# EryiXie/PlaneRecNet

Hardware: AMD Instinct MI355X
Metric: img/s fwd+bwd @480×640 ResNet101-DCN, 1/2/4/8 MI355X + roofline % (higher is better)
Workload: dtype f32 (tensors and accumulation fp32; plain GEMMs and the tap-walked 4x4/s2, 1x1/s2 and sub-pixel convolutions >= 300 tiles: 2xfp16-piece split MFMA, fp32 accumulate; fp32-only rate in fp32_only_run)

## Files before the change

include/prn.h:

```cpp
#ifndef PRN_H
#define PRN_H
#include <stdint.h>
#ifdef __cplusplus
extern "C" {
#endif

#define PRN_BN_SPLITS 32

int prn_version(void);
const char* prn_last_error(void);

enum { PRN_IN_ZERO = 0, PRN_IN_REFLECT = 1, PRN_IN_UP2_REFLECT = 2, PRN_IN_DILATED = 3, PRN_IN_UP2_PHASE = 4,
       PRN_IN_EMBED1 = 5  };
enum { PRN_EPI_NONE = 0, PRN_EPI_RELU = 1, PRN_EPI_SIGMOID = 2 };

enum { PRN_SPLIT_OFF = 0, PRN_SPLIT_PLAN = 1, PRN_SPLIT_ALWAYS = 2 };
enum { PRN_PIECES_BF16 = 0, PRN_PIECES_F16 = 16 };
typedef struct prn_gemm_opts {
  int32_t split_mode;
  int32_t split_kind;
  int32_t split_products;
  int32_t split_min_tiles;
  float split_min_gflop;
  int32_t wgrad_wgs;
// ... 161 lines not shown
                    const float* beta, float* dx, float* dres, float* dgamma, float* dbeta, double* ws,
                    int B, int C, int HW, int relu, int frozen, void* stream);

int prn_bn_train_fwd_partials(const float* parts, int nparts, int64_t part_stride, float* x_out, float* stats, const float* gamma, const float* beta,
                              const float* residual, float* y, float* running_mean, float* running_var, int B, int C, int HW, float eps, float momentum,
                              int relu, void* stream);
int prn_bn_bwd_partials(const float* dparts, int nparts, int64_t part_stride, const float* x, const float* y, const float* stats, const float* gamma,
                        const float* beta, float* dx, float* dres, float* dgamma, float* dbeta, int B, int C, int HW, int relu, int frozen, void* stream);
int prn_bn_train_fwd_winograd(const float* parts, int nparts, int64_t part_stride, float* x_out, float* stats, const float* gamma, const float* beta,
                              const float* residual, float* y, float* running_mean, float* running_var, float* V, int B, int C, int H, int W, float eps,
                              float momentum, int relu, void* stream);
int prn_bn_bwd_winograd(const float* dparts, int nparts, int64_t part_stride, const float* x, const float* y, const float* stats, const float* gamma,
                        const float* beta, float* dx, float* dres, float* dgamma, float* dbeta, float* V, int B, int C, int H, int W, int relu, int frozen,
                        void* stream);

int prn_gn_relu_fwd(const float* x, const float* gamma, const float* beta, float* y, float* stats ,
                    int B, int C, int HW, int G, float eps, void* stream);
int prn_gn_relu_bwd(const float* dy, const float* x, const float* beta, const float* stats, const float* gamma,
                    float* dx, float* dgamma_part , float* dbeta_part ,
                    int B, int C, int HW, int G, void* stream);
int prn_gn_relu_fwd_ragged(const float* x, const float* gamma, const float* beta, float* y, float* stats,
                           int B, int C, int nseg, const int* hw, int G, float eps, void* stream);
int prn_gn_relu_bwd_ragged(const float* dy, const float* x, const float* beta, const float* stats, const float* gamma,
                           float* dx, float* dgamma_part, float* dbeta_part, int B, int C, int nseg, const int* hw, int G,
                           void* stream);

int prn_sum_rows(const float* in, float* out, int nb, int R, int N, void* stream);

int prn_debug_skip_launches(int mask);

int prn_resize_bilinear_fwd(const float* x, float* y, int BC, int H, int W, int Ho, int Wo, void* stream);
int prn_resize_bilinear_bwd(const float* dy, float* dx, int BC, int H, int W, int Ho, int Wo, void* stream);
int prn_resize_bilinear_add_fwd(const float* x, const float* addend, float* y, int BC, int H, int W, int Ho, int Wo, void* stream);
int prn_resize_bilinear_bwd_add(const float* dy, const float* addend, float* dx, int BC, int H, int W, int Ho, int Wo, void* stream);
int prn_maxpool3s2_fwd(const float* x, float* y, unsigned char* arg, int BC, int H, int W, int Ho, int Wo, void* stream);
int prn_maxpool3s2_bwd(const unsigned char* arg, const float* dy, float* dx, int BC, int H, int W, int Ho, int Wo, void* stream);

int64_t prn_plane_prior_ws_bytes(int B, int E, int h, int w, int NK, int F, const prn_gemm_opts* opts);
int prn_plane_prior_fwd(const float* seg, const float* kernels, const float* w1, const float* b1, float* pooled, float* out, void* ws, int B, int E,
                        int h, int w, int NK, int F, const prn_gemm_opts* opts, void* stream);
int prn_plane_prior_fwd_phase(const float* seg, const float* kernels, const float* w1, const float* b1, float* pooled, float* out, void* ws, int B, int E,
                        int h, int w, int NK, int F, const prn_gemm_opts* opts, void* stream, int phase);
int64_t prn_plane_prior_wgrad_ws_bytes(int B, int h, int w, int NK, int F, const prn_gemm_opts* opts);
int prn_plane_prior_wgrad(const float* pooled, const float* d_out, float* dw1, void* ws, int B, int h, int w, int NK, int F, const prn_gemm_opts* opts,
                          void* stream);
int64_t prn_fpn_level_ws_bytes(int B, int C, int H, int W, int F, int relu, int has_prev, int have_u, const prn_gemm_opts* opts);
int prn_fpn_level_fwd(const float* x, const float* w_lat, const float* b_lat, const float* prev, int Hp, int Wp, const float* w_out, const float* u_out,
                      const float* b_out, float* lateral, float* p_out, void* ws, int B, int C, int H, int W, int F, int relu, const prn_gemm_opts* opts,
                      void* stream);

enum { PRN_BLK_WINOGRAD = 1,
       PRN_BLK_HANDOVER = 2,
       PRN_BLK_KEEP_V = 4,
       PRN_BLK_SCATTER_ACC = 8 };
enum { PRN_BLK_CONV2_DIRECT = 0, PRN_BLK_CONV2_WINOGRAD = 1, PRN_BLK_CONV2_DCN = 2 };
typedef struct prn_bottleneck_desc {
  int32_t B, C, H, W;
  int32_t planes;
  int32_t stride;
  int32_t dcn;
  int32_t downsample;
  int32_t flags;
  float eps[4], momentum[4];
  float max_offset;
  int32_t reserved;
  prn_gemm_opts opts;
} prn_bottleneck_desc;
typedef struct prn_bottleneck_params {
  const float *w1, *w2, *w3, *wd;
  const float *b2;
  const void *w1_img, *w3_img, *wd_img;
  const float* u2; const void* u2_img;
  const float *w1_t, *w2_t, *w3_t, *wd_t;
  const void *w1_t_img, *w3_t_img, *wd_t_img;
  const float* ut2; const void* ut2_img;
  const float *w27, *b27, *w27_t;
  const float* w2_cols_t; const void* w2_cols_t_img;
  const float *gamma[4], *beta[4];
  float *running_mean[4], *running_var[4];
} prn_bottleneck_params;
enum { PRN_BLK_SAVE_BYTES = 0, PRN_BLK_GSAVE_BYTES, PRN_BLK_FWD_WS_BYTES, PRN_BLK_BWD_WS_BYTES, PRN_BLK_HO, PRN_BLK_WO, PRN_BLK_CONV2_PATH, PRN_BLK_KEEPS_V,
       PRN_BLK_OFF_A1, PRN_BLK_OFF_V, PRN_BLK_OFF_A2, PRN_BLK_OFF_OM, PRN_BLK_OFF_TABLE,
       PRN_BLK_OFF_D1, PRN_BLK_OFF_D2, PRN_BLK_OFF_D3, PRN_BLK_OFF_DD, PRN_BLK_OFF_DOM,
       PRN_BLK_BN_GRAD_FLOATS,
       PRN_BLK_HANDOVERS,
       PRN_BLK_NEEDS_W1_IMG, PRN_BLK_NEEDS_W3_IMG, PRN_BLK_NEEDS_WD_IMG, PRN_BLK_NEEDS_W1T_IMG, PRN_BLK_NEEDS_W3T_IMG, PRN_BLK_NEEDS_WDT_IMG, PRN_BLK_NEEDS_U_IMG,
       PRN_BLK_NEEDS_COLT_IMG, PRN_BLK_INFO_COUNT };
int64_t prn_bottleneck_plan_bytes(void);
int64_t prn_bottleneck_params_bytes(void);
int prn_bottleneck_plan(const prn_bottleneck_desc* d, void* plan);
int prn_bottleneck_plan_info(const void* plan, int64_t* out, int n);
int prn_bottleneck_train_fwd(const void* plan, const prn_bottleneck_params* p, const float* x, float* y, void* save, void* ws, void* stream);
int prn_bottleneck_train_bwd(const void* plan, const prn_bottleneck_params* p, const float* x, const float* y, const float* dy, float* dx, int dx_accumulate,
                             const void* save, void* gsave, float* bn_grads, void* ws, void* stream);

int prn_frame_to_input(const unsigned char* src, int Hs, int Ws, int Hr, int Wr, int Hp, int Wp, const float* mean_bgr, const float* std_bgr, int mode,
                       float* dst, float* frame_bgr, void* stream);

int prn_mask_loss_ws_floats(int P);
int prn_mask_loss_fwd(const float* logits, const unsigned char* labels, const float* adj, const int64_t* img, const float* gsum, const float* npos,
                      float* out2, float* coef, float* ws, int P, int HW, int B, float w_ins, float w_lav, void* stream);
int prn_mask_loss_bwd(const float* logits, const unsigned char* labels, const float* adj, const int64_t* img, const float* coef, const float* g_ins,
                      const float* g_lav, float* dlogits, int P, int HW, void* stream);

int prn_lava_gt_weights(const float* gt, float* out, int B, int H, int W, float depth_resolution, void* stream);

int prn_vnl_triplets(const float* pred, const float* gt, const int* gid, const int64_t* seg, const unsigned char* seg_is_plane, const double* seg_normal,
// ... 123 lines not shown
```

planerecnet_amd/blocks.py:

```python
import ctypes
import os
import sys

import torch

from . import _lib, ops, profiling
from ._lib import lib, check

ENABLED = os.environ.get("PRN_BLOCKS", "1") == "1"
HANDOVER = os.environ.get("PRN_BLOCK_HANDOVER", "1") == "1"
SCATTER_ACCUMULATE = os.environ.get("PRN_SCATTER_ACC", "1") == "1"
STATS = {"fwd": 0, "bwd": 0, "resolved": 0, "vouched": 0, "scatter_acc": 0}

BLK_WINOGRAD, BLK_HANDOVER, BLK_KEEP_V, BLK_SCATTER_ACC = 1, 2, 4, 8
CONV2_DIRECT, CONV2_WINOGRAD, CONV2_DCN = 0, 1, 2
(I_SAVE, I_GSAVE, I_FWD_WS, I_BWD_WS, I_HO, I_WO, I_CONV2, I_KEEPS_V, I_A1, I_V, I_A2, I_OM, I_TABLE, I_D1, I_D2, I_D3, I_DD, I_DOM, I_BN_FLOATS, I_HANDOVERS,
 I_W1_IMG, I_W3_IMG, I_WD_IMG, I_W1T_IMG, I_W3T_IMG, I_WDT_IMG, I_U_IMG, I_COLT_IMG, INFO_COUNT) = range(29)

_SCRATCH = {}
_F32 = torch.float32
_empty = torch.empty


def scratch(nbytes, dev):
    key = (dev.index, ops._raw_stream(dev.index))
    t = _SCRATCH.get(key)
    if t is None or t.numel() * 4 < nbytes:
        t = _SCRATCH[key] = torch.empty((int(nbytes * 1.25) + 1023) // 4, device=dev, dtype=torch.float32)
    return t


class _Ref:
    __slots__ = ("ptr", "shape", "device")

    def __init__(self, ptr, shape, device):
        self.ptr, self.shape, self.device = ptr, shape, device

    def data_ptr(self):
        return self.ptr

    def numel(self):
        n = 1
        for s in self.shape:
            n *= s
        return n


class _State:
    __slots__ = ("plan", "plan_ref", "info", "params", "params_ref", "convw", "wver", "epoch", "batched", "keep", "hb", "bn_sizes", "out_shape", "Ho", "Wo", "conv2",
                 "dims", "wino_wgrad", "g_keys", "max_offset", "ps", "bns", "stat_bufs", "save_n", "gsave_n", "bn_n", "fwd_ws", "bwd_ws", "stride", "dcn", "ds",
                 "shapes")


def _flags():
    f = BLK_SCATTER_ACC if SCATTER_ACCUMULATE else 0
    if ops.WINOGRAD:
        f |= BLK_WINOGRAD
    if ops.WINOGRAD and ops.WINOGRAD_WGRAD:
        f |= BLK_KEEP_V
    if HANDOVER:
        f |= BLK_HANDOVER
    return f


def supported(blk):
    from .dcn import DeformableConv2d
    c2 = blk.conv2
    if blk.downsample is not None:
        dc = blk.downsample[0]
        if dc.kernel_size != (1, 1) or dc.stride[0] != blk.stride or dc.bias is not None:
            return False
    elif blk.stride != 1 or blk.conv1.weight.shape[1] != blk.conv3.weight.shape[0]:
        return False
    if isinstance(c2, DeformableConv2d):
        if c2.stride != blk.stride:
            return False
    elif c2.bias is not None or c2.kernel_size != (3, 3) or c2.padding != (1, 1) or c2.stride[0] != blk.stride:
        return False
    bns = [blk.bn1, blk.bn2, blk.bn3] + ([blk.downsample[1]] if blk.downsample is not None else [])
    return (blk.stride in (1, 2) and ops.WINOGRAD_MIN_TILES == 128 and blk.conv1.bias is None and blk.conv3.bias is None and blk.conv1.kernel_size == (1, 1)
            and blk.conv3.kernel_size == (1, 1) and all(isinstance(m, torch.nn.BatchNorm2d) and m.affine and m.track_running_stats and m.momentum is not None for m in bns))


def _param_list(blk):
    from .dcn import DeformableConv2d
    c2 = blk.conv2
    ps = [blk.conv1.weight, blk.bn1.weight, blk.bn1.bias]
    if isinstance(c2, DeformableConv2d):
        ps += [c2.offset_conv.weight, c2.modulator_conv.weight, c2.offset_conv.bias, c2.modulator_conv.bias, c2.regular_conv.weight, c2.regular_conv.bias]
    else:
        ps += [c2.weight]
    ps += [blk.bn2.weight, blk.bn2.bias, blk.conv3.weight, blk.bn3.weight, blk.bn3.bias]
    if blk.downsample is not None:
        ps += [blk.downsample[0].weight, blk.downsample[1].weight, blk.downsample[1].bias]
    return tuple(ps)


def _state(blk, x, key):
    from .dcn import DeformableConv2d
    oe = ops._opts_entry()
    B, C, H, W = x.shape
    dcn = isinstance(blk.conv2, DeformableConv2d)
    bns = (blk.bn1, blk.bn2, blk.bn3) + ((blk.downsample[1],) if blk.downsample is not None else ())
    eps = [float(m.eps) for m in bns] + [0.0] * (4 - len(bns))
    mom = [float(m.momentum) for m in bns] + [0.0] * (4 - len(bns))
    P = blk.conv1.weight.shape[0]
    d = _lib.BottleneckDesc(B, C, H, W, P, blk.stride, int(dcn), int(blk.downsample is not None), key[2], (ctypes.c_float * 4)(*eps), (ctypes.c_float * 4)(*mom),
                            max(H, W) / 4.0 if dcn else 0.0, 0, oe[0])
    st = _State()
    st.plan = ctypes.create_string_buffer(int(lib.prn_bottleneck_plan_bytes()) + 64)
    st.plan_ref = (ctypes.addressof(st.plan) + 63) & ~63
    check(lib.prn_bottleneck_plan(ctypes.byref(d), st.plan_ref), "prn_bottleneck_plan")
    info = (ctypes.c_int64 * INFO_COUNT)()
    check(lib.prn_bottleneck_plan_info(st.plan_ref, info, INFO_COUNT), "prn_bottleneck_plan_info")
# ... 276 lines not shown
```

planerecnet_amd/csrc/prn_bottleneck.hip:

```cpp
#include "prn_common.h"
#include <string.h>

namespace {

constexpr int32_t PLAN_MAGIC = 0x424c4b36;
constexpr int64_t WINOGRAD_MIN_TILES = 128;

inline int64_t up256(int64_t v) { return (v + 255) & ~255LL; }

struct Plan {
  int32_t magic, pad_;
  prn_bottleneck_desc d;
  int32_t Ho, Wo, P4, conv2_path;
  int32_t small1, small2;
  int32_t lazy1, parts1;
  int32_t v1, lazy2, keep_v;
  int32_t lazy3g, parts3g;
  int32_t v2g, lazy2g;
  int32_t pad2_;
  int64_t parts1_off, parts3g_off;
  prn_conv_desc c1, c2, c3, cd, c27, g1, g2, g3, gd, g27;
  prn_dcn_desc dcn;
  int64_t s_c1, s_a1, s_v, s_c2, s_a2, s_c3, s_cd, s_om, s_table, s_stats[4], save_bytes;
  int64_t q_d3, q_dd, q_d2, q_d1, q_dom, q_bn, gsave_bytes;
  int64_t f_c1, f_bn, f_v, f_yt, f_gemm, f_c2, f_c27, f_dcn, f_c3, f_cd, f_res, fwd_ws_bytes;
  int64_t b_bn, b_dres, b_g3, b_g3ws, b_v, b_yt, b_gemm, b_g2, b_g2ws, b_dcn, b_dx1, b_g27ws, b_g1ws, b_gdtmp, b_gdws, bwd_ws_bytes;
};

prn_conv_desc conv_desc(int B, int C, int H, int W, int M, int K, int stride, int pad, int Ho, int Wo, int mode, int dil, int ystride, int yH, int yW,
                        const prn_gemm_opts& o) {
  prn_conv_desc d;
  d.B = B; d.C = C; d.H = H; d.W = W; d.M = M; d.KH = d.KW = K; d.stride = stride; d.pad = pad; d.Ho = Ho; d.Wo = Wo;
  d.in_mode = mode; d.dil = dil; d.epilogue = PRN_EPI_NONE; d.ystride = ystride; d.yH = yH; d.yW = yW; d.reserved = 0;
  d.opts = o;
  return d;
}

bool winograd_ok(const prn_bottleneck_desc& d, int B, int C, int H, int W, int M) {
  return (d.flags & PRN_BLK_WINOGRAD) && (W % 4) == 0 && H >= 8 && C >= 64 && M >= 64 && (int64_t)B * ((H + 3) / 4) * (W / 4) >= WINOGRAD_MIN_TILES;
}

int make_plan(const prn_bottleneck_desc* dp, Plan& L) {
  PRN_REQUIRE(dp != nullptr, "prn_bottleneck_plan: null descriptor");
  const prn_bottleneck_desc& d = *dp;
  PRN_REQUIRE(d.B > 0 && d.C > 0 && d.H > 0 && d.W > 0 && d.planes > 0, "prn_bottleneck_plan: empty dimension");
  PRN_REQUIRE(d.stride == 1 || d.stride == 2, "prn_bottleneck_plan: stride %d (1 or 2)", d.stride);
  PRN_REQUIRE(d.downsample || (d.stride == 1 && d.C == 4 * d.planes), "prn_bottleneck_plan: without a downsample branch the block must keep its shape (C = 4 * planes, stride 1)");
  PRN_REQUIRE(!d.dcn || d.max_offset > 0.f, "prn_bottleneck_plan: the deformable variant needs max_offset (max(h, w) / 4)");
  memset(&L, 0, sizeof(L));
  L.magic = PLAN_MAGIC;
  L.d = d;
  const int B = d.B, C = d.C, H = d.H, W = d.W, P = d.planes, s = d.stride, Q = 4 * d.planes;
  const int Ho = (H + 2 - 3) / s + 1, Wo = (W + 2 - 3) / s + 1;
  L.Ho = Ho; L.Wo = Wo;
  const prn_gemm_opts& o = d.opts;
  const bool ho = (d.flags & PRN_BLK_HANDOVER) != 0;
  L.small1 = prn_bn_kernel_kind(B, H * W);
  L.small2 = prn_bn_kernel_kind(B, Ho * Wo);
  L.c1 = conv_desc(B, C, H, W, P, 1, 1, 0, H, W, PRN_IN_ZERO, 1, 0, 0, 0, o);
  L.c3 = conv_desc(B, P, Ho, Wo, Q, 1, 1, 0, Ho, Wo, PRN_IN_ZERO, 1, 0, 0, 0, o);
  if (d.downsample) L.cd = conv_desc(B, C, H, W, Q, 1, s, 0, Ho, Wo, PRN_IN_ZERO, 1, 0, 0, 0, o);
  const bool wino = !d.dcn && s == 1 && winograd_ok(d, B, P, H, W, P);
  L.conv2_path = d.dcn ? PRN_BLK_CONV2_DCN : (wino ? PRN_BLK_CONV2_WINOGRAD : PRN_BLK_CONV2_DIRECT);
  if (d.dcn) {
    L.c27 = conv_desc(B, P, H, W, 27, 3, s, 1, Ho, Wo, PRN_IN_ZERO, 1, 0, 0, 0, o);
    prn_dcn_desc& q = L.dcn;
    q.B = B; q.C = P; q.H = H; q.W = W; q.M = P; q.stride = s; q.pad = 1; q.Ho = Ho; q.Wo = Wo; q.raw = 1; q.max_offset = d.max_offset; q.epilogue = PRN_EPI_NONE;
    q.opts = o;
  } else if (!wino) {
    L.c2 = conv_desc(B, P, H, W, P, 3, s, 1, Ho, Wo, PRN_IN_ZERO, 1, 0, 0, 0, o);
  }
  if (wino) L.P4 = (int)prn_winograd_tiles(B, H, W);
  L.g3 = conv_desc(B, Q, Ho, Wo, P, 1, 1, 0, Ho, Wo, PRN_IN_ZERO, 1, 0, 0, 0, o);
  L.g1 = conv_desc(B, P, H, W, C, 1, 1, 0, H, W, PRN_IN_ZERO, 1, 0, 0, 0, o);
  if (!d.dcn && !wino)
    L.g2 = s == 1 ? conv_desc(B, P, Ho, Wo, P, 3, 1, 1, H, W, PRN_IN_ZERO, 1, 0, 0, 0, o) : conv_desc(B, P, Ho, Wo, P, 3, 1, 1, H, W, PRN_IN_DILATED, 2, 0, 0, 0, o);
  if (d.dcn)
    L.g27 = s == 1 ? conv_desc(B, 27, Ho, Wo, P, 3, 1, 1, H, W, PRN_IN_ZERO, 1, 0, 0, 0, o) : conv_desc(B, 27, Ho, Wo, P, 3, 1, 1, H, W, PRN_IN_DILATED, 2, 0, 0, 0, o);
  if (d.downsample)
    L.gd = s == 1 ? conv_desc(B, Q, Ho, Wo, C, 1, 1, 0, H, W, PRN_IN_ZERO, 1, 0, 0, 0, o) : conv_desc(B, Q, Ho, Wo, C, 1, 1, 0, Ho, Wo, PRN_IN_ZERO, 1, 2, H, W, o);
  int64_t off = 0;
  const int p1 = prn_conv2d_fwd_partials(&L.c1, &off);
  if (p1 < 0) return 2;
  L.lazy1 = ho && L.small1 && p1 > 1 && (((int64_t)B * P * H * W) & 3) == 0;
  L.parts1 = L.lazy1 ? p1 : 0; L.parts1_off = L.lazy1 ? off : 0;
  L.v1 = ho && wino && L.small1;
  L.lazy2 = ho && wino && L.small2 && L.P4 <= 768;
  L.keep_v = wino && (d.flags & PRN_BLK_KEEP_V) && 4LL * 36 * P * L.P4 <= (128LL << 20);
  const int p3 = prn_conv2d_fwd_partials(&L.g3, &off);
  if (p3 < 0) return 2;
  L.lazy3g = ho && L.small2 && p3 > 1 && (((int64_t)B * P * Ho * Wo) & 3) == 0;
  L.parts3g = L.lazy3g ? p3 : 0; L.parts3g_off = L.lazy3g ? off : 0;
  L.v2g = ho && wino && L.small2;
  L.lazy2g = ho && wino && L.small1 && L.P4 <= 768;
  const int64_t n1 = (int64_t)B * P * H * W * 4, n2 = (int64_t)B * P * Ho * Wo * 4, n3 = (int64_t)B * Q * Ho * Wo * 4, nx = (int64_t)B * C * H * W * 4;
  const int64_t nv = wino ? 4LL * 36 * P * L.P4 : 0, nom = (int64_t)B * 27 * Ho * Wo * 4;
  const int Cmax = Q > C ? Q : C;
  const int64_t bnws = 2LL * Cmax * PRN_BN_SPLITS * 8;
#define PRN_WS(expr_, name_) const int64_t name_ = (expr_); if (name_ < 0) return 2
  PRN_WS(prn_conv2d_fwd_ws_bytes(&L.c1), w_c1);
  PRN_WS(prn_conv2d_fwd_ws_bytes(&L.c3), w_c3);
  PRN_WS(d.downsample ? prn_conv2d_fwd_ws_bytes(&L.cd) : 0, w_cd);
  PRN_WS(L.conv2_path == PRN_BLK_CONV2_DIRECT ? prn_conv2d_fwd_ws_bytes(&L.c2) : 0, w_c2);
  PRN_WS(d.dcn ? prn_conv2d_fwd_ws_bytes(&L.c27) : 0, w_c27);
  PRN_WS(d.dcn ? prn_dcnv2_fwd_ws_bytes(&L.dcn) : 0, w_dcnf);
  PRN_WS(d.dcn ? prn_dcnv2_table_bytes(&L.dcn) : 0, n_table);
  PRN_WS(d.dcn ? prn_dcnv2_bwd_ws_bytes(&L.dcn) : 0, w_dcnb);
  PRN_WS(wino ? prn_gemm_batched_ws_bytes(P, P, L.P4, 36, &o) : 0, w_gemm);
  PRN_WS(prn_conv2d_fwd_ws_bytes(&L.g3), w_g3);
  PRN_WS(prn_conv2d_fwd_ws_bytes(&L.g1), w_g1);
  PRN_WS(L.conv2_path == PRN_BLK_CONV2_DIRECT ? prn_conv2d_fwd_ws_bytes(&L.g2) : 0, w_g2);
  PRN_WS(d.dcn ? prn_conv2d_fwd_ws_bytes(&L.g27) : 0, w_g27);
  PRN_WS(d.downsample ? prn_conv2d_fwd_ws_bytes(&L.gd) : 0, w_gd);
#undef PRN_WS
  int64_t at = 0;
  auto put = [&at](int64_t& slot, int64_t bytes) { slot = at; at += up256(bytes); };
  put(L.s_c1, n1); put(L.s_a1, n1);
  put(L.s_v, L.keep_v ? nv : 0);
  put(L.s_c2, n2); put(L.s_a2, n2); put(L.s_c3, n3);
  put(L.s_cd, d.downsample ? n3 : 0);
  put(L.s_om, d.dcn ? nom : 0); put(L.s_table, n_table);
  put(L.s_stats[0], 8LL * P); put(L.s_stats[1], 8LL * P); put(L.s_stats[2], 8LL * Q); put(L.s_stats[3], d.downsample ? 8LL * Q : 0);
  L.save_bytes = at;
  at = 0;
  put(L.q_d3, n3); put(L.q_dd, d.downsample ? n3 : 0); put(L.q_d2, n2); put(L.q_d1, n1); put(L.q_dom, d.dcn ? nom : 0);
  L.q_bn = 2 * P + 2 * P + 2 * Q + (d.downsample ? 2 * Q : 0);
  L.gsave_bytes = at;
  at = 0;
  put(L.f_c1, w_c1); put(L.f_bn, bnws);
  put(L.f_v, (wino && !L.keep_v) ? nv : 0); put(L.f_yt, nv); put(L.f_gemm, w_gemm);
  put(L.f_c2, w_c2); put(L.f_c27, w_c27); put(L.f_dcn, w_dcnf); put(L.f_c3, w_c3); put(L.f_cd, w_cd);
  put(L.f_res, d.downsample ? n3 : 0);
  L.fwd_ws_bytes = at;
  at = 0;
  put(L.b_bn, bnws); put(L.b_dres, n3);
  put(L.b_g3, n2); put(L.b_g3ws, w_g3);
  put(L.b_v, nv); put(L.b_yt, nv); put(L.b_gemm, w_gemm);
  put(L.b_g2, n1); put(L.b_g2ws, w_g2);
  put(L.b_dcn, w_dcnb); put(L.b_dx1, d.dcn ? n1 : 0); put(L.b_g27ws, w_g27);
  put(L.b_g1ws, w_g1);
  put(L.b_gdtmp, d.downsample ? nx : 0); put(L.b_gdws, w_gd);
  L.bwd_ws_bytes = at;
  return 0;
}

const Plan* plan_of(const void* plan, const char* who) {
  const Plan* L = (const Plan*)plan;
  if (L == nullptr || L->magic != PLAN_MAGIC) { prn_set_error("%s: not a plan filled by prn_bottleneck_plan", who); return nullptr; }
  return L;
}

inline float* f32(void* base, int64_t off) { return (float*)((char*)base + off); }
inline void* raw(void* base, int64_t off, int64_t used = 1) { return used ? (void*)((char*)base + off) : nullptr; }

#define PRN_TRY(call_) do { if (int e_ = (call_)) return e_; } while (0)

}

extern "C" int64_t prn_bottleneck_plan_bytes(void) { return (int64_t)sizeof(Plan); }
extern "C" int64_t prn_bottleneck_params_bytes(void) { return (int64_t)sizeof(prn_bottleneck_params); }

extern "C" int prn_bottleneck_plan(const prn_bottleneck_desc* d, void* plan) {
  PRN_REQUIRE(plan != nullptr, "prn_bottleneck_plan: null plan buffer (prn_bottleneck_plan_bytes() bytes, caller-owned)");
  Plan L;
  if (int e = make_plan(d, L)) { memset(plan, 0, sizeof(int32_t)); return e; }
  memcpy(plan, &L, sizeof(L));
  return 0;
}

extern "C" int prn_bottleneck_plan_info(const void* plan, int64_t* out, int n) {
  const Plan* L = plan_of(plan, "prn_bottleneck_plan_info");
  if (!L) return 2;
  PRN_REQUIRE(out != nullptr && n >= PRN_BLK_INFO_COUNT, "prn_bottleneck_plan_info: out must hold PRN_BLK_INFO_COUNT (%d) values", PRN_BLK_INFO_COUNT);
  out[PRN_BLK_SAVE_BYTES] = L->save_bytes; out[PRN_BLK_GSAVE_BYTES] = L->gsave_bytes;
  out[PRN_BLK_FWD_WS_BYTES] = L->fwd_ws_bytes; out[PRN_BLK_BWD_WS_BYTES] = L->bwd_ws_bytes;
  out[PRN_BLK_HO] = L->Ho; out[PRN_BLK_WO] = L->Wo; out[PRN_BLK_CONV2_PATH] = L->conv2_path; out[PRN_BLK_KEEPS_V] = L->keep_v;
  out[PRN_BLK_OFF_A1] = L->s_a1; out[PRN_BLK_OFF_V] = L->s_v; out[PRN_BLK_OFF_A2] = L->s_a2; out[PRN_BLK_OFF_OM] = L->s_om; out[PRN_BLK_OFF_TABLE] = L->s_table;
  out[PRN_BLK_OFF_D1] = L->q_d1; out[PRN_BLK_OFF_D2] = L->q_d2; out[PRN_BLK_OFF_D3] = L->q_d3; out[PRN_BLK_OFF_DD] = L->q_dd; out[PRN_BLK_OFF_DOM] = L->q_dom;
  out[PRN_BLK_BN_GRAD_FLOATS] = L->q_bn;
  out[PRN_BLK_HANDOVERS] = L->lazy1 | (L->v1 << 1) | (L->lazy2 << 2) | (L->lazy3g << 3) | (L->v2g << 4) | (L->lazy2g << 5);
  out[PRN_BLK_NEEDS_W1_IMG] = prn_conv2d_kernel_kind(&L->c1) >= 2; out[PRN_BLK_NEEDS_W3_IMG] = prn_conv2d_kernel_kind(&L->c3) >= 2;
  out[PRN_BLK_NEEDS_WD_IMG] = (L->d.downsample && L->d.stride == 1 && prn_conv2d_kernel_kind(&L->cd) >= 2) ? 1 : 0;
  out[PRN_BLK_NEEDS_W1T_IMG] = prn_conv2d_kernel_kind(&L->g1) >= 2; out[PRN_BLK_NEEDS_W3T_IMG] = prn_conv2d_kernel_kind(&L->g3) >= 2;
  out[PRN_BLK_NEEDS_WDT_IMG] = (L->d.downsample && L->d.stride == 1 && prn_conv2d_kernel_kind(&L->gd) >= 2) ? 1 : 0;
  out[PRN_BLK_NEEDS_U_IMG] = (L->conv2_path == PRN_BLK_CONV2_WINOGRAD && prn_gemm_pipe(L->d.planes, L->d.planes, 1, L->P4, 36, &L->d.opts) >= 1) ? 1 : 0;
  out[PRN_BLK_NEEDS_COLT_IMG] = (L->d.dcn && prn_gemm_pipe(9 * L->d.planes, L->d.planes, L->d.B, L->Ho * L->Wo, 1, &L->d.opts) >= 1) ? 1 : 0;
  return 0;
}

extern "C" int prn_bottleneck_train_fwd(const void* plan, const prn_bottleneck_params* p, const float* x, float* y, void* save, void* ws, void* stream) {
  const Plan* Lp = plan_of(plan, "prn_bottleneck_train_fwd");
  if (!Lp) return 2;
  const Plan& L = *Lp;
  const prn_bottleneck_desc& d = L.d;
  PRN_REQUIRE(p && x && y && save && (ws || L.fwd_ws_bytes == 0), "prn_bottleneck_train_fwd: null tensor / buffer");
  PRN_REQUIRE(p->w1 && p->w3 && (p->w2 || L.conv2_path == PRN_BLK_CONV2_WINOGRAD) && (p->u2 || L.conv2_path != PRN_BLK_CONV2_WINOGRAD) && (!d.downsample || p->wd),
              "prn_bottleneck_train_fwd: a weight operand the plan reads is null");
  PRN_REQUIRE(!d.dcn || (p->w27 && p->b27), "prn_bottleneck_train_fwd: the deformable variant needs the merged offset | modulator weights");
  for (int i = 0; i < (d.downsample ? 4 : 3); ++i)
    PRN_REQUIRE(p->gamma[i] && p->beta[i] && p->running_mean[i] && p->running_var[i], "prn_bottleneck_train_fwd: null BatchNorm parameter (layer %d)", i);
  PRN_REQUIRE(((reinterpret_cast<uintptr_t>(save) | reinterpret_cast<uintptr_t>(ws)) & 255) == 0, "prn_bottleneck_train_fwd: save / ws must be 256-byte aligned");
  const int B = d.B, H = d.H, W = d.W, P = d.planes, Q = 4 * P, Ho = L.Ho, Wo = L.Wo;
  float* c1 = f32(save, L.s_c1); float* a1 = f32(save, L.s_a1); float* c2 = f32(save, L.s_c2); float* a2 = f32(save, L.s_a2); float* c3 = f32(save, L.s_c3);
  float* st1 = f32(save, L.s_stats[0]); float* st2 = f32(save, L.s_stats[1]); float* st3 = f32(save, L.s_stats[2]); float* std_ = f32(save, L.s_stats[3]);
  double* bnws = (double*)raw(ws, L.f_bn);
  const int64_t n1 = (int64_t)B * P * H * W;
  const prn_gemm_opts* o = &d.opts;
  PRN_TRY(prn_conv2d_fwd_counted(&L.c1, x, p->w1, p->w1_img, nullptr, nullptr, c1, raw(ws, L.f_c1, L.f_bn - L.f_c1), nullptr, stream, L.lazy1 ? 1 : 0));
  float* V = L.conv2_path == PRN_BLK_CONV2_WINOGRAD ? (L.keep_v ? f32(save, L.s_v) : f32(ws, L.f_v)) : nullptr;
  const float* in1 = L.lazy1 ? f32(ws, L.f_c1 + L.parts1_off) : c1;
  if (L.v1)
    PRN_TRY(prn_bn_train_fwd_winograd(in1, L.lazy1 ? L.parts1 : 1, L.lazy1 ? n1 : 0, L.lazy1 ? c1 : nullptr, st1, p->gamma[0], p->beta[0], nullptr, a1, p->running_mean[0],
                                      p->running_var[0], V, B, P, H, W, d.eps[0], d.momentum[0], 1, stream));
  else if (L.lazy1)
    PRN_TRY(prn_bn_train_fwd_partials(in1, L.parts1, n1, c1, st1, p->gamma[0], p->beta[0], nullptr, a1, p->running_mean[0], p->running_var[0], B, P, H * W, d.eps[0],
                                      d.momentum[0], 1, stream));
  else
    PRN_TRY(prn_bn_train_fwd(c1, st1, p->gamma[0], p->beta[0], nullptr, a1, p->running_mean[0], p->running_var[0], L.small1 ? nullptr : bnws, B, P, H * W, d.eps[0],
                             d.momentum[0], 1, stream));
  float* Yt = f32(ws, L.f_yt);
  if (L.conv2_path == PRN_BLK_CONV2_WINOGRAD) {
    if (!L.v1) PRN_TRY(prn_winograd_input(a1, V, B, P, H, W, PRN_IN_ZERO, stream));
    PRN_TRY(prn_gemm_batched(P, P, L.P4, 36, p->u2, p->u2_img, V, Yt, raw(ws, L.f_gemm, L.f_c2 - L.f_gemm), o, stream));
    if (!L.lazy2) PRN_TRY(prn_winograd_output(Yt, nullptr, nullptr, c2, B, P, H, W, PRN_EPI_NONE, stream));
  } else if (L.conv2_path == PRN_BLK_CONV2_DCN) {
    float* om = f32(save, L.s_om);
    void* table = raw(save, L.s_table);
    PRN_TRY(prn_conv2d_fwd_counted(&L.c27, a1, p->w27, nullptr, p->b27, nullptr, om, raw(ws, L.f_c27, L.f_dcn - L.f_c27), nullptr, stream, 0));
    PRN_TRY(prn_dcnv2_table(&L.dcn, om, nullptr, table, stream));
    PRN_TRY(prn_dcnv2_fwd(&L.dcn, a1, table, p->w2, p->b2, c2, raw(ws, L.f_dcn, L.f_c3 - L.f_dcn), stream));
  } else {
    PRN_TRY(prn_conv2d_fwd_counted(&L.c2, a1, p->w2, nullptr, nullptr, nullptr, c2, raw(ws, L.f_c2, L.f_c27 - L.f_c2), nullptr, stream, 0));
  }
  if (L.conv2_path == PRN_BLK_CONV2_WINOGRAD && L.lazy2)
    PRN_TRY(prn_winograd_output_bn_fwd(Yt, c2, st2, p->gamma[1], p->beta[1], a2, p->running_mean[1], p->running_var[1], B, P, Ho, Wo, d.eps[1], d.momentum[1], 1, stream));
  else
    PRN_TRY(prn_bn_train_fwd(c2, st2, p->gamma[1], p->beta[1], nullptr, a2, p->running_mean[1], p->running_var[1], L.small2 ? nullptr : bnws, B, P, Ho * Wo, d.eps[1],
                             d.momentum[1], 1, stream));
  PRN_TRY(prn_conv2d_fwd_counted(&L.c3, a2, p->w3, p->w3_img, nullptr, nullptr, c3, raw(ws, L.f_c3, L.f_cd - L.f_c3), nullptr, stream, 0));
  const float* res = x;
  if (d.downsample) {
    float* cd = f32(save, L.s_cd);
    float* rd = f32(ws, L.f_res);
    PRN_TRY(prn_conv2d_fwd_counted(&L.cd, x, p->wd, d.stride == 1 ? p->wd_img : nullptr, nullptr, nullptr, cd, raw(ws, L.f_cd, L.f_res - L.f_cd), nullptr, stream, 0));
    PRN_TRY(prn_bn_train_fwd(cd, std_, p->gamma[3], p->beta[3], nullptr, rd, p->running_mean[3], p->running_var[3], L.small2 ? nullptr : bnws, B, Q, Ho * Wo, d.eps[3],
                             d.momentum[3], 0, stream));
    res = rd;
  }
  return prn_bn_train_fwd(c3, st3, p->gamma[2], p->beta[2], res, y, p->running_mean[2], p->running_var[2], L.small2 ? nullptr : bnws, B, Q, Ho * Wo, d.eps[2], d.momentum[2],
                          1, stream);
}

extern "C" int prn_bottleneck_train_bwd(const void* plan, const prn_bottleneck_params* p, const float* x, const float* y, const float* dy, float* dx,
                                        int dx_accumulate, const void* save_, void* gsave, float* bn_grads, void* ws, void* stream) {
  const Plan* Lp = plan_of(plan, "prn_bottleneck_train_bwd");
  if (!Lp) return 2;
  const Plan& L = *Lp;
  const prn_bottleneck_desc& d = L.d;
  PRN_REQUIRE(p && x && y && dy && dx && save_ && gsave && bn_grads && ws, "prn_bottleneck_train_bwd: null tensor / buffer");
  PRN_REQUIRE(p->w1_t && p->w3_t && (!d.downsample || p->wd_t), "prn_bottleneck_train_bwd: an input-gradient weight layout the plan reads is null");
  PRN_REQUIRE(L.conv2_path != PRN_BLK_CONV2_WINOGRAD || p->ut2, "prn_bottleneck_train_bwd: conv2's Winograd-domain input-gradient operand is null");
  PRN_REQUIRE(L.conv2_path != PRN_BLK_CONV2_DIRECT || p->w2_t, "prn_bottleneck_train_bwd: conv2's input-gradient layout is null");
  PRN_REQUIRE(!d.dcn || (p->w27_t && p->w2_cols_t), "prn_bottleneck_train_bwd: the deformable variant needs the input-gradient layouts of both convolutions");
  PRN_REQUIRE(!dx_accumulate || (d.downsample && d.stride == 2 && (d.flags & PRN_BLK_SCATTER_ACC)),
              "prn_bottleneck_train_bwd: dx_accumulate only for stride-2 downsample blocks planned with PRN_BLK_SCATTER_ACC");
  PRN_REQUIRE(((reinterpret_cast<uintptr_t>(save_) | reinterpret_cast<uintptr_t>(gsave) | reinterpret_cast<uintptr_t>(ws)) & 255) == 0,
              "prn_bottleneck_train_bwd: save / gsave / ws must be 256-byte aligned");
  void* save = const_cast<void*>(save_);
  const int B = d.B, C = d.C, H = d.H, W = d.W, P = d.planes, Q = 4 * P, Ho = L.Ho, Wo = L.Wo;
  const float* c1 = f32(save, L.s_c1); const float* a1 = f32(save, L.s_a1); const float* c2 = f32(save, L.s_c2); const float* c3 = f32(save, L.s_c3);
  const float* st1 = f32(save, L.s_stats[0]); const float* st2 = f32(save, L.s_stats[1]); const float* st3 = f32(save, L.s_stats[2]); const float* std_ = f32(save, L.s_stats[3]);
  float* d3 = f32(gsave, L.q_d3); float* d2 = f32(gsave, L.q_d2); float* d1 = f32(gsave, L.q_d1);
  float* dg1 = bn_grads; float* db1 = dg1 + P; float* dg2 = db1 + P; float* db2 = dg2 + P; float* dg3 = db2 + P; float* db3 = dg3 + Q; float* dgd = db3 + Q; float* dbd = dgd + Q;
  double* bnws = (double*)raw(ws, L.b_bn);
  float* dres = f32(ws, L.b_dres);
  const prn_gemm_opts* o = &d.opts;
  hipStream_t st = (hipStream_t)stream;
  PRN_TRY(prn_bn_bwd(dy, c3, y, st3, p->gamma[2], p->beta[2], d3, dres, dg3, db3, L.small2 ? nullptr : bnws, B, Q, Ho * Wo, 1, 0, stream));
  const float* addx = dres;
  if (d.downsample) {
    float* dd = f32(gsave, L.q_dd);
    PRN_TRY(prn_bn_bwd(dres, f32(save, L.s_cd), nullptr, std_, p->gamma[3], p->beta[3], dd, nullptr, dgd, dbd, L.small2 ? nullptr : bnws, B, Q, Ho * Wo, 0, 0, stream));
    void* gws = raw(ws, L.b_gdws, L.bwd_ws_bytes - L.b_gdws);
    if (d.stride == 1) {
      float* tmp = f32(ws, L.b_gdtmp);
      PRN_TRY(prn_conv2d_fwd_counted(&L.gd, dd, p->wd_t, p->wd_t_img, nullptr, nullptr, tmp, gws, nullptr, stream, 0));
      addx = tmp;
    } else if (dx_accumulate) {
      PRN_TRY(prn_conv2d_fwd_counted(&L.gd, dd, p->wd_t, nullptr, nullptr, dx, dx, gws, nullptr, stream, 0));
      addx = dx;
    } else {
      float* tmp = f32(ws, L.b_gdtmp);
      const hipError_t e = hipMemsetAsync(tmp, 0, (size_t)B * C * H * W * 4, st);
      PRN_REQUIRE(e == hipSuccess, "prn_bottleneck_train_bwd: clearing the strided input gradient failed: %s", hipGetErrorString(e));
      PRN_TRY(prn_conv2d_fwd_counted(&L.gd, dd, p->wd_t, nullptr, nullptr, nullptr, tmp, gws, nullptr, stream, 0));
      addx = tmp;
    }
  }
  float* g3 = f32(ws, L.b_g3);
  PRN_TRY(prn_conv2d_fwd_counted(&L.g3, d3, p->w3_t, p->w3_t_img, nullptr, nullptr, g3, raw(ws, L.b_g3ws, L.b_v - L.b_g3ws), nullptr, stream, L.lazy3g ? 1 : 0));
  const float* in2 = L.lazy3g ? f32(ws, L.b_g3ws + L.parts3g_off) : g3;
  const int64_t n2 = (int64_t)B * P * Ho * Wo;
  float* Vg = f32(ws, L.b_v);
  if (L.v2g)
    PRN_TRY(prn_bn_bwd_winograd(in2, L.lazy3g ? L.parts3g : 1, L.lazy3g ? n2 : 0, c2, nullptr, st2, p->gamma[1], p->beta[1], d2, nullptr, dg2, db2, Vg, B, P, Ho, Wo, 1, 0, stream));
  else if (L.lazy3g)
    PRN_TRY(prn_bn_bwd_partials(in2, L.parts3g, n2, c2, nullptr, st2, p->gamma[1], p->beta[1], d2, nullptr, dg2, db2, B, P, Ho * Wo, 1, 0, stream));
  else
    PRN_TRY(prn_bn_bwd(g3, c2, nullptr, st2, p->gamma[1], p->beta[1], d2, nullptr, dg2, db2, L.small2 ? nullptr : bnws, B, P, Ho * Wo, 1, 0, stream));
  float* g2 = f32(ws, L.b_g2);
  float* Ytg = f32(ws, L.b_yt);
  if (L.conv2_path == PRN_BLK_CONV2_WINOGRAD) {
    if (!L.v2g) PRN_TRY(prn_winograd_input(d2, Vg, B, P, H, W, PRN_IN_ZERO, stream));
    PRN_TRY(prn_gemm_batched(P, P, L.P4, 36, p->ut2, p->ut2_img, Vg, Ytg, raw(ws, L.b_gemm, L.b_g2 - L.b_gemm), o, stream));
    if (!L.lazy2g) PRN_TRY(prn_winograd_output(Ytg, nullptr, nullptr, g2, B, P, H, W, PRN_EPI_NONE, stream));
  } else if (L.conv2_path == PRN_BLK_CONV2_DCN) {
    const float* om = f32(save, L.s_om);
    float* dom = f32(gsave, L.q_dom);
    float* dx1 = f32(ws, L.b_dx1);
    void* cws = raw(ws, L.b_dcn);
    PRN_TRY(prn_dcnv2_bwd_input(&L.dcn, d2, p->w2_cols_t, p->w2_cols_t_img, om, nullptr, dx1, cws, stream));
    PRN_TRY(prn_dcnv2_bwd_offset_mask(&L.dcn, a1, om, nullptr, dom, nullptr, cws, stream));
    PRN_TRY(prn_conv2d_fwd_counted(&L.g27, dom, p->w27_t, nullptr, nullptr, dx1, g2, raw(ws, L.b_g27ws, L.b_g1ws - L.b_g27ws), nullptr, stream, 0));
  } else {
    PRN_TRY(prn_conv2d_fwd_counted(&L.g2, d2, p->w2_t, nullptr, nullptr, nullptr, g2, raw(ws, L.b_g2ws, L.b_dcn - L.b_g2ws), nullptr, stream, 0));
  }
  if (L.conv2_path == PRN_BLK_CONV2_WINOGRAD && L.lazy2g)
    PRN_TRY(prn_winograd_output_bn_bwd(Ytg, c1, st1, p->gamma[0], p->beta[0], d1, dg1, db1, B, P, H, W, 1, stream));
  else
    PRN_TRY(prn_bn_bwd(g2, c1, nullptr, st1, p->gamma[0], p->beta[0], d1, nullptr, dg1, db1, L.small1 ? nullptr : bnws, B, P, H * W, 1, 0, stream));
  return prn_conv2d_fwd_counted(&L.g1, d1, p->w1_t, p->w1_t_img, nullptr, addx, dx, raw(ws, L.b_g1ws, L.b_gdtmp - L.b_g1ws), nullptr, stream, 0);
}
```

planerecnet_amd/csrc/prn_common.h:

```cpp
#pragma once
#include <hip/hip_runtime.h>
#include <stdint.h>
#include <stdio.h>
#include "../../include/prn.h"

#define PRN_WAVE 64

void prn_set_error(const char* fmt, ...);

#include <stdlib.h>
static inline int prn_env_int(const char* name, int dflt) {
  const char* e = getenv(name);
  return e ? atoi(e) : dflt;
}
struct prn_env4 { int v[4]; };
static inline prn_env4 prn_env_ints(const char* name) {
  prn_env4 r = {{0, 0, 0, 0}};
  if (const char* e = getenv(name)) sscanf(e, "%d,%d,%d,%d", &r.v[0], &r.v[1], &r.v[2], &r.v[3]);
  return r;
}

extern int prn_skip_mask;
#define PRN_SKIPPED(bit) (__builtin_expect(prn_skip_mask & (bit), 0))
#define PRN_REPS(bit) (__builtin_expect(prn_skip_mask & ((bit) | ((bit) << 8)), 0) ? ((prn_skip_mask & (bit)) ? 0 : 2) : 1)
// ... 37 lines not shown
  const int64_t T_ = (int64_t)gridDim.x * 256, i0_ = (int64_t)blockIdx.x * 256 + threadIdx.x; \
  float v_[PRN_EPT]; \
  _Pragma("unroll") for (int k_ = 0; k_ < PRN_EPT; ++k_) { \
    const int64_t i = (i0_ + k_ * T_ < (total_)) ? i0_ + k_ * T_ : (total_) - 1;
#define PRN_EPT_END(total_, out_) \
  } \
  _Pragma("unroll") for (int k_ = 0; k_ < PRN_EPT; ++k_) if (i0_ + k_ * T_ < (total_)) (out_)[i0_ + k_ * T_] = v_[k_];


__device__ __forceinline__ float wave_sum(float v) {
#pragma unroll
  for (int o = 32; o > 0; o >>= 1) v += __shfl_xor(v, o, 64);
  return v;
}
__device__ __forceinline__ double wave_sum_d(double v) {
#pragma unroll
  for (int o = 32; o > 0; o >>= 1) v += __shfl_xor(v, o, 64);
  return v;
}
__device__ __forceinline__ int wave_sum_i(int v) {
#pragma unroll
  for (int o = 32; o > 0; o >>= 1) v += __shfl_xor(v, o, 64);
  return v;
}

__device__ __forceinline__ void block_sum2(double& a, double& b, double* sm) {
  a = wave_sum_d(a);
  b = wave_sum_d(b);
  const int w = threadIdx.x >> 6, nw = blockDim.x >> 6;
  __syncthreads();
  if ((threadIdx.x & 63) == 0) { sm[w] = a; sm[nw + w] = b; }
  __syncthreads();
  double ra = 0.0, rb = 0.0;
  for (int i = 0; i < nw; ++i) { ra += sm[i]; rb += sm[nw + i]; }
  a = ra; b = rb;
}

__device__ __forceinline__ void bt6(const float* v, float* o) {
  o[0] = 4.f * v[0] - 5.f * v[2] + v[4];
  o[1] = -4.f * (v[1] + v[2]) + v[3] + v[4];
  o[2] = 4.f * (v[1] - v[2]) - v[3] + v[4];
  o[3] = -2.f * v[1] - v[2] + 2.f * v[3] + v[4];
  o[4] = 2.f * v[1] - v[2] - 2.f * v[3] + v[4];
  o[5] = 4.f * v[1] - 5.f * v[3] + v[5];
}
__device__ __forceinline__ void at6(const float* m, float* o) {
  const float s12 = m[1] + m[2], d12 = m[1] - m[2], s34 = m[3] + m[4], d34 = m[3] - m[4];
  o[0] = m[0] + s12 + s34;
  o[1] = d12 + 2.f * d34;
  o[2] = s12 + 4.f * s34;
  o[3] = d12 + 8.f * d34 + m[5];
}

static inline int cdiv(int64_t a, int64_t b) { return (int)((a + b - 1) / b); }
__host__ __device__ inline size_t prn_align256(size_t v) { return (v + 255) & ~(size_t)255; }

int prn_launch_reduce_epilogue(const float* ws, const float* bias, const float* addend, float* y, int64_t total, int M, int HoWo, int splits,
                               int epi, hipStream_t st);
int prn_launch_reduce_splits(const float* ws, float* out, int64_t n, int splits, hipStream_t st);
int prn_quantise_splits(int64_t tiles, int splits);
int prn_gemm_batched_epi(int M, int C, int P, int nb, const float* U, const void* u_images, const float* V, float* Y, void* ws, const prn_gemm_opts* opts, int epi,
                         void* stream);

int prn_split_gemm_plan(int M, int K, int B, int HW, int nz, const prn_gemm_opts* opts);
int64_t prn_split_gemm_image_bytes(int M, int K, int nz);
int64_t prn_split_gemm_partial_bytes(int M, int B, int HW, int nz, int splits);
int prn_split_gemm(const float* w, const void* w_images, const float* x, const float* bias, const float* addend, float* y, void* images_ws, float* partial, int M,
                   int K, int B, int HW, int nz, int64_t zw, int64_t zx, int64_t zy, int epi, int splits, const prn_gemm_opts* opts, hipStream_t st, int phase);
int prn_split_conv_taps(const float* w, const float* x, const float* bias, const float* addend, float* y, void* images_ws, float* partial, int M, int C, int B, int XH,
                        int XW, int Ho, int Wo, int KH, int KW, int stride, int pad, int epi, int splits, const prn_gemm_opts* o, hipStream_t st, int phase);
int prn_split_conv_up2(const float* wp, const float* x, const float* bias, float* y, void* images_ws, int M, int C, int B, int H, int W, int epi, const prn_gemm_opts* o,
                       hipStream_t st);
static inline prn_gemm_opts prn_opts_or_zero(const prn_gemm_opts* o) {
  prn_gemm_opts z;
  if (o) return *o;
  z.split_mode = 0; z.split_kind = 0; z.split_products = 0; z.split_min_tiles = 0; z.split_min_gflop = 0.f; z.wgrad_wgs = 0; z.wgrad_target = 0; z.wgrad_split = 0;
  return z;
}

int prn_wgrad16_plan(int M, int C, int64_t N, int HW, int nz, const prn_gemm_opts* opts);
int prn_wgrad16_launch(const float* dy, const float* x, const float* const* gdy, const float* const* gx, int ngroup, float* out, int M, int C, int B, int HW, int nz,
                       int64_t zdy, int64_t zx, int splits, const prn_gemm_opts* opts, hipStream_t st);
```

planerecnet_amd/csrc/prn_conv.hip:

```cpp
#include <stddef.h>
#include <stdlib.h>
#include <type_traits>
#include "prn_common.h"

typedef float f32x16 __attribute__((ext_vector_type(16)));

namespace {

constexpr int MAX_SEG = 6;
struct Seg {
  int nseg;
  int n0[MAX_SEG + 1];
  int H[MAX_SEG], W[MAX_SEG];
  int x0[MAX_SEG], y0[MAX_SEG];
};
__device__ __forceinline__ int seg_find(const Seg& g, int n) {
  int s = 0;
#pragma unroll
  for (int t = 1; t < MAX_SEG; ++t)
    if (t < g.nseg && n >= g.n0[t]) s = t;
  return s;
}
template <class Args>
__device__ __forceinline__ int seg_read(size_t member_offset, int s) {
// ... 839 lines not shown
#pragma unroll
  for (int t = 0; t < 9; ++t) {
    const int o = tap_offset<PRN_IN_ZERO>(oh - pad + t / 3, ow - pad + t % 3, true, H, W);
    v[t] = o >= 0 ? xb[o] : 0.f;
  }
  for (int m = 0; m < M; ++m) {
    float r = 0.f;
#pragma unroll
    for (int t = 0; t < 9; ++t) r += w[(size_t)m * 9 + t] * v[t];
    const size_t idx = ((size_t)b * M + m) * HoWo + p;
    if (bias) r += bias[m];
    if (addend) r += addend[idx];
    if (epi == PRN_EPI_RELU) r = fmaxf(r, 0.f);
    else if (epi == PRN_EPI_SIGMOID) r = 1.f / (1.f + __expf(-r));
    y[idx] = r;
  }
}

template <int MODE>
__global__ __launch_bounds__(256) void conv3x3_small_m_wgrad_kernel(const float* __restrict__ x, const float* __restrict__ dy, float* __restrict__ out,
                                                                    int B, int C, int H, int W, int M, int pad) {
  const int c = blockIdx.x % C, m = blockIdx.x / C, sp = blockIdx.y, S = gridDim.y;
  const int HW = H * W;
  const int64_t N = (int64_t)B * HW, beg = N * sp / S, end = N * (sp + 1) / S;
  float acc[9];
#pragma unroll
  for (int t = 0; t < 9; ++t) acc[t] = 0.f;
  for (int64_t n = beg + threadIdx.x; n < end; n += 256) {
    const int b = (int)(n / HW), p = (int)(n - (int64_t)b * HW), oh = p / W, ow = p - oh * W;
    const float g = dy[((size_t)b * M + m) * HW + p];
    const float* xc = x + ((size_t)b * C + c) * HW;
#pragma unroll
    for (int t = 0; t < 9; ++t) {
      const int o = tap_offset<MODE>(oh - pad + t / 3, ow - pad + t % 3, true, H, W);
      acc[t] += g * (o >= 0 ? xc[o] : 0.f);
    }
  }
  __shared__ float sm[4][9];
#pragma unroll
  for (int t = 0; t < 9; ++t) {
    float v = acc[t];
    for (int o = 32; o > 0; o >>= 1) v += __shfl_down(v, o);
    if ((threadIdx.x & 63) == 0) sm[threadIdx.x >> 6][t] = v;
  }
  __syncthreads();
  if (threadIdx.x < 9) {
    const int t = threadIdx.x;
    out[((size_t)sp * M + m) * C * 9 + (size_t)c * 9 + t] = (sm[0][t] + sm[1][t]) + (sm[2][t] + sm[3][t]);
  }
}

__global__ __launch_bounds__(256) void reduce_epilogue_kernel(const float* __restrict__ ws, const float* __restrict__ bias,
                                                               const float* __restrict__ addend, float* __restrict__ y, int64_t total,
                                                               int M, int HoWo, int splits, int epi) {
  const int64_t i = ((int64_t)blockIdx.x * 256 + threadIdx.x) * 4;
  if (i >= total) return;
  if (i + 3 < total && (HoWo & 3) == 0) {
    float4 v = *reinterpret_cast<const float4*>(ws + i);
    for (int s = 1; s < splits; ++s) {
      const float4 t = *reinterpret_cast<const float4*>(ws + (size_t)s * total + i);
      v.x += t.x; v.y += t.y; v.z += t.z; v.w += t.w;
    }
    const int m = (int)((i / HoWo) % M);
    if (bias) { const float bm = bias[m]; v.x += bm; v.y += bm; v.z += bm; v.w += bm; }
    if (addend) { const float4 t = *reinterpret_cast<const float4*>(addend + i); v.x += t.x; v.y += t.y; v.z += t.z; v.w += t.w; }
    if (epi == PRN_EPI_RELU) { v.x = fmaxf(v.x, 0.f); v.y = fmaxf(v.y, 0.f); v.z = fmaxf(v.z, 0.f); v.w = fmaxf(v.w, 0.f); }
    else if (epi == PRN_EPI_SIGMOID) { v.x = 1.f / (1.f + __expf(-v.x)); v.y = 1.f / (1.f + __expf(-v.y)); v.z = 1.f / (1.f + __expf(-v.z)); v.w = 1.f / (1.f + __expf(-v.w)); }
    *reinterpret_cast<float4*>(y + i) = v;
  } else {
    for (int64_t q = i; q < total && q < i + 4; ++q) {
      float v = ws[q];
      for (int s = 1; s < splits; ++s) v += ws[(size_t)s * total + q];
      if (bias) v += bias[(q / HoWo) % M];
      if (addend) v += addend[q];
      if (epi == PRN_EPI_RELU) v = fmaxf(v, 0.f);
      else if (epi == PRN_EPI_SIGMOID) v = 1.f / (1.f + __expf(-v));
      y[q] = v;
    }
  }
}

__global__ __launch_bounds__(256) void reduce_tail_kernel(const float* __restrict__ ws, const float* __restrict__ bias, const float* __restrict__ addend,
                                                          float* __restrict__ y, int64_t total, int M, int HoWo, int n_start, int ntail4, int splits,
                                                          int epi) {
  const int64_t t = (int64_t)blockIdx.x * 256 + threadIdx.x;
  if (t >= (int64_t)M * ntail4) return;
  const int m = (int)(t / ntail4), q = (int)(t - (int64_t)m * ntail4);
  const int n = n_start + q * 4, b = n / HoWo, p = n - b * HoWo;
  const int64_t i = ((int64_t)b * M + m) * HoWo + p;
  float4 v = *reinterpret_cast<const float4*>(ws + i);
  for (int s = 1; s < splits; ++s) {
    const float4 u = *reinterpret_cast<const float4*>(ws + (size_t)s * total + i);
    v.x += u.x; v.y += u.y; v.z += u.z; v.w += u.w;
  }
  if (bias) { const float bm = bias[m]; v.x += bm; v.y += bm; v.z += bm; v.w += bm; }
  if (addend) { const float4 u = *reinterpret_cast<const float4*>(addend + i); v.x += u.x; v.y += u.y; v.z += u.z; v.w += u.w; }
  if (epi == PRN_EPI_RELU) { v.x = fmaxf(v.x, 0.f); v.y = fmaxf(v.y, 0.f); v.z = fmaxf(v.z, 0.f); v.w = fmaxf(v.w, 0.f); }
  else if (epi == PRN_EPI_SIGMOID) { v.x = 1.f / (1.f + __expf(-v.x)); v.y = 1.f / (1.f + __expf(-v.y)); v.z = 1.f / (1.f + __expf(-v.z)); v.w = 1.f / (1.f + __expf(-v.w)); }
  *reinterpret_cast<float4*>(y + i) = v;
}

__global__ __launch_bounds__(256) void reduce_splits_kernel(const float* __restrict__ ws, float* __restrict__ out, int64_t n, int splits) {
  __shared__ float sm[4][64];
  const int e = threadIdx.x & 63, g = threadIdx.x >> 6;
  const int64_t i = (int64_t)blockIdx.x * 64 + e;
  float acc = 0.f;
  if (i < n) {
    float a0 = 0.f, a1 = 0.f, a2 = 0.f, a3 = 0.f;
    int k = g;
    for (; k + 12 < splits; k += 16) {
      a0 += ws[(size_t)k * n + i];
      a1 += ws[(size_t)(k + 4) * n + i];
      a2 += ws[(size_t)(k + 8) * n + i];
      a3 += ws[(size_t)(k + 12) * n + i];
    }
    for (; k < splits; k += 4) a0 += ws[(size_t)k * n + i];
    acc = (a0 + a1) + (a2 + a3);
  }
// ... 371 lines not shown
int direct_wgrad_splits(const prn_conv_desc* d) {
  int s = 2048 / (d->C * d->M);
  return s < 1 ? 1 : (s > 64 ? 64 : s);
}

struct Geo { int gH, gW, phases; bool nosplit; };
Geo geo_of(const prn_conv_desc* d) {
  Geo g;
  g.phases = d->in_mode == PRN_IN_UP2_PHASE ? 4 : 1;
  g.gH = g.phases == 4 ? d->H : d->Ho;
  g.gW = g.phases == 4 ? d->W : d->Wo;
  g.nosplit = g.phases == 4 || d->ystride == 2;
  return g;
}

int tail_of(const prn_conv_desc* d, const Geo& g, const FwdPlan& p, int* pieces) {
  *pieces = 0;
  if (g.phases != 1 || g.nosplit || d->ystride > 1) return 0;
  const int64_t N = (int64_t)d->B * g.gH * g.gW;
  const int tilesM = cdiv(d->M, 32 * p.wm * p.tm);
  return plan_tail(p, (int64_t)tilesM * cdiv(N, 32 * p.wn * p.tn), tilesM, d->C * d->KH * d->KW, N, g.gH * g.gW, pieces);
}

int split_plan_of(const prn_conv_desc* d) {
  if (!(d->KH == 1 && d->in_mode == PRN_IN_ZERO && d->stride == 1 && d->pad == 0 && d->ystride <= 1 && d->Ho == d->H && d->Wo == d->W)) return 0;
  return prn_split_gemm_plan(d->M, d->C, d->B, d->H * d->W, 1, &d->opts);
}
int wgrad16_plan_of(const prn_conv_desc* d, int G) {
  if (!(d->KH == 1 && d->in_mode == PRN_IN_ZERO && d->stride == 1 && d->pad == 0 && d->ystride <= 1 && d->Ho == d->H && d->Wo == d->W)) return 0;
  return prn_wgrad16_plan(d->M, d->C, (int64_t)d->B * d->H * d->W, d->H * d->W, G, &d->opts);
}
int taps_plan_of(const prn_conv_desc* d) {
  static const int on = prn_env_int("PRN_SPLIT_TAPS", 1);
  const bool shape = (d->KH == 4 && d->stride == 2) || (d->KH == 1 && d->stride == 2 && d->pad == 0);
  if (!on || !(shape && d->in_mode == PRN_IN_ZERO && d->ystride <= 1 && (d->C & 31) == 0 && d->opts.split_kind == PRN_PIECES_F16)) return 0;
  return prn_split_gemm_plan(d->M, d->C * d->KH * d->KW, d->B, d->Ho * d->Wo, 1, &d->opts);
}
int up2_plan_of(const prn_conv_desc* d) {
  static const int on = prn_env_int("PRN_SPLIT_UP2", 1);
  if (!on || !(d->KH == 2 && d->in_mode == PRN_IN_UP2_PHASE && (d->C & 31) == 0 && (d->W & 3) == 0 && d->opts.split_kind == PRN_PIECES_F16 && d->ystride <= 1)) return 0;
  if (!(d->epilogue == PRN_EPI_NONE || d->epilogue == PRN_EPI_RELU)) return 0;
  return prn_split_gemm_plan(d->M, d->C * 4, d->B, d->H * d->W, 4, &d->opts) == 1 ? 1 : 0;
}
int64_t taps_ws_bytes(const prn_conv_desc* d, int splits) {
  return ((prn_split_gemm_image_bytes(d->M, d->C * d->KH * d->KW, 1) + 255) & ~255LL) + prn_split_gemm_partial_bytes(d->M, d->B, d->Ho * d->Wo, 1, splits);
}
int64_t split_ws_bytes(const prn_conv_desc* d, int splits) {
  return ((prn_split_gemm_image_bytes(d->M, d->C, 1) + 255) & ~255LL) + prn_split_gemm_partial_bytes(d->M, d->B, d->H * d->W, 1, splits);
}

}

int prn_launch_reduce_epilogue(const float* ws, const float* bias, const float* addend, float* y, int64_t total, int M, int HoWo, int splits,
                               int epi, hipStream_t st) {
  hipLaunchKernelGGL(reduce_epilogue_kernel, dim3(cdiv(total, 1024)), dim3(256), 0, st, ws, bias, addend, y, total, M, HoWo, splits, epi);
  PRN_CHECK_LAUNCH("reduce_epilogue");
  return 0;
}
int prn_launch_reduce_splits(const float* ws, float* out, int64_t n, int splits, hipStream_t st) {
  for (int r = PRN_REPS(4); r > 0; --r) hipLaunchKernelGGL(reduce_splits_kernel, dim3(cdiv(n, 64)), dim3(256), 0, st, ws, out, n, splits);
  PRN_CHECK_LAUNCH("reduce_splits");
  return 0;
}
int prn_quantise_splits(int64_t tiles, int splits) { return quantise_splits(tiles, splits); }

extern "C" int64_t prn_conv2d_fwd_ws_bytes(const prn_conv_desc* d) {
  if (check_desc(d, "prn_conv2d_fwd_ws_bytes")) return -1;
  if (direct_small_m(d) || direct_one_c(d)) return 0;
  if (const int ss = split_plan_of(d)) return split_ws_bytes(d, ss);
  if (const int st = taps_plan_of(d)) return taps_ws_bytes(d, st);
  if (up2_plan_of(d)) return (prn_split_gemm_image_bytes(d->M, d->C * 4, 4) + 255) & ~255LL;
  const Geo g = geo_of(d);
  const FwdPlan p = plan_fwd(d->M, (int64_t)d->B * g.gH * g.gW, d->C * d->KH * d->KW, narrow_available(d->KH, d->in_mode), g.phases, g.nosplit,
                             wide_ks(d->KH, d->in_mode));
  if (p.splits > 1) return (int64_t)p.splits * d->B * d->M * d->Ho * d->Wo * 4;
  int pieces = 0;
  tail_of(d, g, p, &pieces);
  return pieces > 1 ? (int64_t)pieces * d->B * d->M * d->Ho * d->Wo * 4 : 0;
}

extern "C" int prn_conv2d_fwd(const prn_conv_desc* d, const float* x, const float* w, const float* bias,
                              const float* addend, float* y, void* ws, void* stream) {
  return prn_conv2d_fwd_phase(d, x, w, bias, addend, y, ws, stream, 0);
}

namespace {
int fill_seg(Seg& sg, const prn_ragged* rg, const prn_conv_desc* d, int align, const char* who) {
  sg.nseg = 0;
  if (rg == nullptr) return 0;
  PRN_REQUIRE(rg->nseg >= 1 && rg->nseg <= MAX_SEG, "%s: 1..%d segments", who, MAX_SEG);
  PRN_REQUIRE(d->in_mode == PRN_IN_ZERO && d->stride == 1 && (d->KH == 1 || d->KH == 3) && d->pad == (d->KH - 1) / 2 && d->ystride <= 1,
              "%s: ragged batches take stride-1 'same' 1x1 / 3x3 convolutions with zero padding", who);
  int64_t n = 0, xo = 0, yo = 0;
  for (int s = 0; s < rg->nseg; ++s) {
    const int H = rg->H[s], W = rg->W[s];
    PRN_REQUIRE(H > 0 && W > 0, "%s: empty segment", who);
    PRN_REQUIRE(n % align == 0, "%s: segment %d starts at pixel %lld, not a multiple of %d", who, s, (long long)n, align);
    sg.n0[s] = (int)n; sg.H[s] = H; sg.W[s] = W; sg.x0[s] = (int)xo; sg.y0[s] = (int)yo;
    n += (int64_t)d->B * H * W;
    xo += (int64_t)d->B * d->C * H * W;
    yo += (int64_t)d->B * d->M * H * W;
  }
  PRN_REQUIRE(n % align == 0 && n < (1LL << 31) && xo < (1LL << 29) && yo < (1LL << 29), "%s: ragged batch too large or unaligned", who);
  for (int s = rg->nseg; s <= MAX_SEG; ++s) sg.n0[s] = (int)n;
  sg.nseg = rg->nseg;
  return 0;
}
int64_t seg_pixels(const prn_ragged* rg, int B) {
  int64_t n = 0;
  for (int s = 0; s < rg->nseg; ++s) n += (int64_t)B * rg->H[s] * rg->W[s];
  return n;
}
int conv_fwd_impl(const prn_conv_desc* d, const prn_ragged* rg, const float* x, const float* w, const float* bias, const float* addend, float* y,
                  void* ws, void* stream, int phase, unsigned* counters = nullptr, const void* w_images = nullptr);
int conv_wgrad_impl(const prn_conv_desc* d, const prn_ragged* rg, const float* x, const float* dy, float* dw, void* ws, void* stream, int phase);
}

extern "C" int prn_conv2d_kernel_kind(const prn_conv_desc* d) {
  if (check_desc(d, "prn_conv2d_kernel_kind")) return -1;
  if (direct_small_m(d) || direct_one_c(d)) return 1;
  int ss = split_plan_of(d);
  if (ss == 0) ss = taps_plan_of(d);
  if (ss == 0) ss = up2_plan_of(d);
  return ss == 0 ? 0 : (ss == 1 ? 2 : 3);
}

extern "C" int prn_conv2d_fwd_partials(const prn_conv_desc* d, int64_t* offset_bytes) {
  if (check_desc(d, "prn_conv2d_fwd_partials")) return -1;
  PRN_REQUIRE(offset_bytes != nullptr, "prn_conv2d_fwd_partials: null offset");
  *offset_bytes = 0;
  if (direct_small_m(d) || direct_one_c(d)) return 0;
  if (const int ss = split_plan_of(d)) {
    *offset_bytes = (prn_split_gemm_image_bytes(d->M, d->C, 1) + 255) & ~255LL;
    return ss > 1 ? ss : 0;
  }
  if (taps_plan_of(d) || up2_plan_of(d)) return 0;
  const Geo g = geo_of(d);
  const FwdPlan p = plan_fwd(d->M, (int64_t)d->B * g.gH * g.gW, d->C * d->KH * d->KW, narrow_available(d->KH, d->in_mode), g.phases, g.nosplit,
                             wide_ks(d->KH, d->in_mode));
  return p.splits > 1 ? p.splits : 0;
}

extern "C" int prn_conv2d_fwd_phase(const prn_conv_desc* d, const float* x, const float* w, const float* bias,
                                    const float* addend, float* y, void* ws, void* stream, int phase) {
  return conv_fwd_impl(d, nullptr, x, w, bias, addend, y, ws, stream, phase);
}

extern "C" int prn_conv2d_fwd_counted(const prn_conv_desc* d, const float* x, const float* w, const void* w_images, const float* bias, const float* addend,
                                      float* y, void* ws, unsigned* counters, void* stream, int phase) {
  return conv_fwd_impl(d, nullptr, x, w, bias, addend, y, ws, stream, phase, counters, w_images);
}

extern "C" int prn_conv2d_fwd_ragged(const prn_conv_desc* d, const prn_ragged* rg, const float* x, const float* w, const float* bias,
                                     const float* addend, float* y, void* stream) {
  PRN_REQUIRE(rg != nullptr, "prn_conv2d_fwd_ragged: null segment list");
  return conv_fwd_impl(d, rg, x, w, bias, addend, y, nullptr, stream, 0);
}

namespace {
int conv_fwd_impl(const prn_conv_desc* d0, const prn_ragged* rg, const float* x, const float* w, const float* bias, const float* addend, float* y,
                  void* ws, void* stream, int phase, unsigned* counters, const void* w_images) {
  prn_conv_desc dd;
  const prn_conv_desc* d = d0;
  if (rg && d0) {
    dd = *d0; dd.H = dd.Ho = rg->H[0]; dd.W = dd.Wo = rg->W[0]; d = &dd;
  }
  if (int e = check_desc(d, "prn_conv2d_fwd")) return e;
  PRN_REQUIRE(x && w && y, "prn_conv2d_fwd: null tensor");
  if (rg == nullptr && (direct_small_m(d) || direct_one_c(d))) {
    if (phase == 2) return 0;
    hipStream_t sd = (hipStream_t)stream;
    if (direct_small_m(d)) {
      const dim3 grid(cdiv((int64_t)d->B * d->H * d->W, 256)), block(256);
#define PRN_SMALL_M(MODE_, MM_) hipLaunchKernelGGL((conv3x3_small_m_kernel<MODE_, MM_>), grid, block, 0, sd, x, w, bias, addend, y, d->B, d->C, d->H, d->W, \
                                                   d->pad, d->epilogue)
      if (d->in_mode == PRN_IN_ZERO) { if (d->M == 1) PRN_SMALL_M(PRN_IN_ZERO, 1); else PRN_SMALL_M(PRN_IN_ZERO, 2); }
      else { if (d->M == 1) PRN_SMALL_M(PRN_IN_REFLECT, 1); else PRN_SMALL_M(PRN_IN_REFLECT, 2); }
#undef PRN_SMALL_M
    } else {
      hipLaunchKernelGGL(conv3x3_one_c_kernel, dim3(cdiv((int64_t)d->B * d->Ho * d->Wo, 256)), dim3(256), 0, sd, x, w, bias, addend, y, d->B, d->H, d->W,
                         d->M, d->pad, d->Ho, d->Wo, d->epilogue);
    }
    PRN_CHECK_LAUNCH("prn_conv2d_fwd/direct");
    return 0;
  }
  if (rg == nullptr && ws != nullptr) {
    if (const int ss = split_plan_of(d)) {
      const int64_t ib = (prn_split_gemm_image_bytes(d->M, d->C, 1) + 255) & ~255LL;
      return prn_split_gemm(w, w_images, x, bias, addend, y, ws, (float*)((char*)ws + ib), d->M, d->C, d->B, d->H * d->W, 1, 0, 0, 0, d->epilogue, ss, &d->opts,
                            (hipStream_t)stream, phase);
    }
    if (up2_plan_of(d) && addend == nullptr && (reinterpret_cast<uintptr_t>(y) & 15) == 0) {
      if (phase == 2) return 0;
      return prn_split_conv_up2(w, x, bias, y, ws, d->M, d->C, d->B, d->H, d->W, d->epilogue, &d->opts, (hipStream_t)stream);
    }
    if (const int st = taps_plan_of(d)) {
      const int64_t ib = (prn_split_gemm_image_bytes(d->M, d->C * d->KH * d->KW, 1) + 255) & ~255LL;
      return prn_split_conv_taps(w, x, bias, addend, y, ws, (float*)((char*)ws + ib), d->M, d->C, d->B, d->H, d->W, d->Ho, d->Wo, d->KH, d->KW, d->stride, d->pad, d->epilogue,
                                 st, &d->opts, (hipStream_t)stream, phase);
    }
  }
  ConvArgs a;
  a.x = x; a.w = w; a.bias = bias; a.addend = addend; a.y = y; a.ws = (float*)ws;
  a.B = d->B; a.C = d->C; a.H = d->H; a.W = d->W; a.M = d->M; a.stride = d->stride; a.pad = d->pad;
  const Geo g = geo_of(d);
  a.Ho = g.gH; a.Wo = g.gW; a.epi = d->epilogue;
  a.K = d->C * d->KH * d->KW; a.N = d->B * g.gH * g.gW; a.HoWo = g.gH * g.gW; a.HW = d->H * d->W;
  a.xbytes = d->B * d->C * d->H * d->W * 4; a.wbytes = d->M * a.K * 4;
  a.ystride = 1; a.yW = g.gW; a.yHW = a.HoWo;
  a.zx = a.zw = a.zy = 0;
  if (g.phases == 4) { a.ystride = 2; a.yW = d->Wo; a.yHW = d->Ho * d->Wo; }
  else if (d->ystride == 2) { a.ystride = 2; a.yW = d->yW; a.yHW = d->yH * d->yW; }
  if (rg) a.N = (int)seg_pixels(rg, d->B);
  FwdPlan p = plan_fwd(a.M, a.N, a.K, narrow_available(d->KH, d->in_mode), g.phases, g.nosplit || rg != nullptr, wide_ks(d->KH, d->in_mode));
  if (rg) {
    int bn = 32 * p.wn * p.tn;
    bool ok = true;
    int64_t n = 0;
    for (int sI = 0; sI < rg->nseg; ++sI) { ok = ok && n % bn == 0; n += (int64_t)d->B * rg->H[sI] * rg->W[sI]; }
    if (!(ok && n % bn == 0) && !(p.tm == 1 && p.tn == 1 && p.wm == 2)) { p.tm = 1; p.tn = 1; p.wm = 2; p.wn = 2; }
    if (int e = fill_seg(a.seg, rg, d, 32 * p.wn * p.tn, "prn_conv2d_fwd_ragged")) return e;
  } else {
    a.seg.nseg = 0;
  }
  PRN_REQUIRE(p.splits == 1 || ws != nullptr, "prn_conv2d_fwd: workspace required (%d K-splits, see prn_conv2d_fwd_ws_bytes)", p.splits);
  hipStream_t st = (hipStream_t)stream;
  const int mode = d->in_mode;
  int tail_pieces = 0;
  const int tail_tiles = (rg == nullptr && ws != nullptr) ? tail_of(d, g, p, &tail_pieces) : 0;
  if (phase == 2) goto reduce_only;
  if (d->KH == 1) {
    PRN_REQUIRE(mode == PRN_IN_ZERO || mode == PRN_IN_DILATED, "prn_conv2d_fwd: 1x1 kernels take zero or dilated input mode");
    if (mode == PRN_IN_ZERO) launch_fwd<1, PRN_IN_ZERO>(a, p, st, 1, tail_tiles, tail_pieces, counters); else launch_fwd<1, PRN_IN_DILATED>(a, p, st, 1, 0, 0, counters);
  } else if (d->KH == 2) {
    launch_fwd<2, PRN_IN_UP2_PHASE>(a, p, st, 4);
  } else if (d->KH == 3) {
    if (mode == PRN_IN_ZERO) launch_fwd<3, PRN_IN_ZERO>(a, p, st, 1, tail_tiles, tail_pieces, counters);
    else if (mode == PRN_IN_REFLECT) launch_fwd<3, PRN_IN_REFLECT>(a, p, st, 1, tail_tiles, tail_pieces, counters);
    else if (mode == PRN_IN_UP2_REFLECT) launch_fwd<3, PRN_IN_UP2_REFLECT>(a, p, st, 1, 0, 0, counters);
    else launch_fwd<3, PRN_IN_DILATED>(a, p, st, 1, 0, 0, counters);
  } else if (d->KH == 4) {
    launch_fwd<4, PRN_IN_ZERO>(a, p, st, 1, 0, 0, counters);
  } else {
    if (mode == PRN_IN_ZERO) launch_fwd<7, PRN_IN_ZERO>(a, p, st, 1, 0, 0, counters); else launch_fwd<7, PRN_IN_DILATED>(a, p, st, 1, 0, 0, counters);
  }
  PRN_CHECK_LAUNCH("prn_conv2d_fwd");
  if (phase == 1) return 0;
reduce_only:
  {
    const bool tail_launch = tail_pieces > 1 && (mode == PRN_IN_ZERO || mode == PRN_IN_REFLECT) && (d->KH == 1 || d->KH == 3);
    if (fused_reduce_ok(a, p, g.phases, tail_launch ? tail_pieces : 0, counters)) return 0;
  }
  if (p.splits > 1) {
    const int64_t total = (int64_t)a.B * a.M * a.HoWo;
    hipLaunchKernelGGL(reduce_epilogue_kernel, dim3(cdiv(total, 1024)), dim3(256), 0, st, (const float*)ws, bias, addend, y, total, a.M, a.HoWo,
                       p.splits, a.epi);
    PRN_CHECK_LAUNCH("prn_conv2d_fwd/reduce");
  } else if (tail_pieces > 1 && (mode == PRN_IN_ZERO || mode == PRN_IN_REFLECT) && (d->KH == 1 || d->KH == 3)) {
    const int64_t total = (int64_t)a.B * a.M * a.HoWo;
    const int bn = 32 * p.wn * p.tn, tilesM = cdiv(a.M, 32 * p.wm * p.tm);
    const int n_start = (int)(((int64_t)tilesM * cdiv(a.N, bn) - tail_tiles) / tilesM) * bn;
    const int ntail4 = (a.N - n_start) / 4;
    hipLaunchKernelGGL(reduce_tail_kernel, dim3(cdiv((int64_t)a.M * ntail4, 256)), dim3(256), 0, st, (const float*)ws, bias, addend, y, total, a.M, a.HoWo,
                       n_start, ntail4, tail_pieces, a.epi);
    PRN_CHECK_LAUNCH("prn_conv2d_fwd/tail reduce");
  }
  return 0;
}
}

extern "C" int64_t prn_conv2d_wgrad_ws_bytes(const prn_conv_desc* d) {
  if (check_desc(d, "prn_conv2d_wgrad_ws_bytes")) return -1;
  const int K = d->C * d->KH * d->KW;
  if (direct_small_m(d)) return (int64_t)direct_wgrad_splits(d) * d->M * K * 4;
  if (const int s16 = wgrad16_plan_of(d, 1)) return s16 > 1 ? (int64_t)s16 * d->M * K * 4 : 0;
  const Geo g = geo_of(d);
  WgPlan p = plan_wgrad(d->opts, d->M, K, (int64_t)d->B * g.gH * g.gW, g.phases);
  return p.splits > 1 ? (int64_t)p.splits * g.phases * d->M * K * 4 : 0;
}

extern "C" int prn_conv2d_wgrad_kernel_kind(const prn_conv_desc* d, int G) {
  if (check_desc(d, "prn_conv2d_wgrad_kernel_kind")) return -1;
  if (direct_small_m(d)) return 1;
  return wgrad16_plan_of(d, G < 1 ? 1 : G) ? 2 : 0;
}
extern "C" int prn_conv2d_wgrad(const prn_conv_desc* d, const float* x, const float* dy, float* dw, void* ws, void* stream) {
  return prn_conv2d_wgrad_phase(d, x, dy, dw, ws, stream, 0);
}

extern "C" int prn_conv2d_wgrad_phase(const prn_conv_desc* d, const float* x, const float* dy, float* dw, void* ws, void* stream, int phase) {
  return conv_wgrad_impl(d, nullptr, x, dy, dw, ws, stream, phase);
}

extern "C" int64_t prn_conv2d_wgrad_grouped_ws_bytes(const prn_conv_desc* d, int G) {
  if (check_desc(d, "prn_conv2d_wgrad_grouped_ws_bytes")) return -1;
  if (G < 1 || G > PRN_WGRAD_GROUP_MAX || geo_of(d).phases != 1 || direct_small_m(d)) { prn_set_error("prn_conv2d_wgrad_grouped_ws_bytes: unsupported group"); return -1; }
  const int K = d->C * d->KH * d->KW;
  if (const int s16 = wgrad16_plan_of(d, G)) return s16 > 1 ? (int64_t)s16 * G * d->M * K * 4 : 0;
  const WgPlan p = plan_wgrad(d->opts, d->M, K, (int64_t)d->B * d->Ho * d->Wo, G);
  return p.splits > 1 ? (int64_t)p.splits * G * d->M * K * 4 : 0;
}

extern "C" int prn_conv2d_wgrad_grouped(const prn_conv_desc* d, int G, const float* const* x, const float* const* dy, float* dw, void* ws, void* stream) {
  if (int e = check_desc(d, "prn_conv2d_wgrad_grouped")) return e;
  PRN_REQUIRE(G >= 1 && G <= PRN_WGRAD_GROUP_MAX, "prn_conv2d_wgrad_grouped: 1 <= G <= %d", PRN_WGRAD_GROUP_MAX);
  PRN_REQUIRE(x && dy && dw, "prn_conv2d_wgrad_grouped: null argument");
  const Geo g = geo_of(d);
  PRN_REQUIRE(g.phases == 1 && !direct_small_m(d) && d->in_mode != PRN_IN_DILATED && d->KH != 4 && d->KH != 2 && d->ystride <= 1,
              "prn_conv2d_wgrad_grouped: dense 1x1 / 3x3 / 7x7 weight gradients only");
// ... 266 lines not shown
```

planerecnet_amd/csrc/prn_gemm_split.hip:

```cpp
#include "prn_common.h"
#include <stdlib.h>

namespace {

typedef __attribute__((ext_vector_type(8))) __bf16 bf16x8_t;
typedef __attribute__((ext_vector_type(16))) float f32x16_t;
typedef int i32x4_t __attribute__((ext_vector_type(4)));
typedef float f32x4_t __attribute__((ext_vector_type(4)));

constexpr int BM = 128, BK = 32;
constexpr int IMG_U4 = 1536;

__device__ __forceinline__ void split2(float x0, float x1, unsigned& h, unsigned& m, unsigned& l) {
  const unsigned u0 = __float_as_uint(x0), u1 = __float_as_uint(x1);
  const float r0 = x0 - __uint_as_float(u0 & 0xffff0000u), r1 = x1 - __uint_as_float(u1 & 0xffff0000u);
  const unsigned v0 = __float_as_uint(r0), v1 = __float_as_uint(r1);
  const float s0 = r0 - __uint_as_float(v0 & 0xffff0000u), s1 = r1 - __uint_as_float(v1 & 0xffff0000u);
  h = __builtin_amdgcn_perm(u1, u0, 0x07060302u);
  m = __builtin_amdgcn_perm(v1, v0, 0x07060302u);
  l = __builtin_amdgcn_perm(__float_as_uint(s1), __float_as_uint(s0), 0x07060302u);
}

__global__ void split_prepare_kernel(const float* __restrict__ w, uint4* __restrict__ img, int M, int K, long long zw, int mtiles, int kslices, long long total) {
  const long long i = (long long)blockIdx.x * 256 + threadIdx.x;
// ... 177 lines not shown

__global__ void split16_prepare_kernel(const float* __restrict__ w, uint4* __restrict__ img, const int* __restrict__ ex, int M, int K, long long zw, int mtiles, int kslices,
                                       long long total, int taps = 1) {
  const long long i = (long long)blockIdx.x * 256 + threadIdx.x;
  if (i >= total) return;
  const int g = i % 4; const int r = (i / 4) % 128; const long long t = i / 512;
  const int ks = t % kslices; const long long zm = t / kslices; const int mt = zm % mtiles; const long long z = zm / mtiles;
  const int m = mt * 128 + r, k0 = ks * 32 + g * 8;
  const int sh = 14 - ex[z * (mtiles * 128) + m];
  float v[8];
  const int C = K / taps;
#pragma unroll
  for (int j = 0; j < 8; ++j) {
    const int kp = k0 + j;
    const int ksrc = taps > 1 ? (kp % C) * taps + kp / C : kp;
    v[j] = (m < M && kp < K) ? ldexpf(w[z * zw + (long long)m * K + ksrc], sh) : 0.f;
  }
  uint4 h, l;
  split2_f16(v[0], v[1], h.x, l.x); split2_f16(v[2], v[3], h.y, l.y); split2_f16(v[4], v[5], h.z, l.z); split2_f16(v[6], v[7], h.w, l.w);
  uint4* o = img + t * IMG16_U4;
  o[g * 128 + r] = h; o[(4 + g) * 128 + r] = l;
}

#ifdef PRN_S16_TIMING
__device__ long long prn_s16_dbg[8192 * 6];
#define S16_T(slot_) do { if (t == 0 && blockIdx.x + gridDim.x * blockIdx.y < 8192) prn_s16_dbg[(blockIdx.x + gridDim.x * blockIdx.y) * 6 + (slot_)] = (long long)wall_clock64(); } while (0)
__device__ long long prn_s16_it[64 * 4 * 4];
#define S16_IT(slot_) do { if (t == 0 && (blockIdx.x == 0 || blockIdx.x == gridDim.x / 2) && blockIdx.y == 0 && ks - ks0 < 64) { \
    if ((slot_) == 2) asm volatile("s_waitcnt vmcnt(0)" ::: "memory"); \
    prn_s16_it[((blockIdx.x ? 1 : 0) * 64 + (ks - ks0)) * 4 + (slot_)] = (long long)wall_clock64(); } } while (0)
extern "C" int prn_debug_s16_iter(long long* host, int n) { return (int)hipMemcpyFromSymbol(host, HIP_SYMBOL(prn_s16_it), sizeof(long long) * (size_t)n); }
extern "C" int prn_debug_s16_timing(long long* host, int n) { return (int)hipMemcpyFromSymbol(host, HIP_SYMBOL(prn_s16_dbg), sizeof(long long) * (size_t)n); }
#else
#define S16_T(slot_) do { } while (0)
#define S16_IT(slot_) do { } while (0)
#endif

__device__ __forceinline__ void store4_policy(float* p, float4 v, int pol) {
  const f32x4_t q = {v.x, v.y, v.z, v.w};
  if (pol == 0) *reinterpret_cast<float4*>(p) = v;
  else if (pol == 1) asm volatile("global_store_dwordx4 %0, %1, off sc1" ::"v"(p), "v"(q) : "memory");
  else if (pol == 2) asm volatile("global_store_dwordx4 %0, %1, off nt" ::"v"(p), "v"(q) : "memory");
  else if (pol == 3) asm volatile("global_store_dwordx4 %0, %1, off sc0 sc1" ::"v"(p), "v"(q) : "memory");
  else asm volatile("global_store_dwordx4 %0, %1, off sc1 nt" ::"v"(p), "v"(q) : "memory");
}

struct Split16Args {
  const uint4* img; const int* ex; const float* x; const float* bias; const float* addend; float* y; float* partial;
  int M, K, B, HW, epi, mtiles, kslices, ptiles, total, splits;
  int wide;
  int store_policy;
  long long zx, zy, slice;
  int C, XH, XW, Wo, KW, stride, pad;
};

template <int NP, int TAPS = 0>
__global__ __launch_bounds__(256) __attribute__((amdgpu_waves_per_eu(3, 3))) void split16_gemm_kernel(const Split16Args a) {
  __shared__ uint4 lds[2 * IMG16_U4];
  const int t = threadIdx.x, lane = t & 63, wave = __builtin_amdgcn_readfirstlane(t >> 6);
  const int id = prn_xcd_remap(blockIdx.x, a.total);
  const int mt = id % a.mtiles; const int rest = id / a.mtiles;
  const int pt = rest % a.ptiles; const int zb = rest / a.ptiles; const int b = zb % a.B, z = zb / a.B;
  const int sp = blockIdx.y;
  const int ks0 = (int)((long long)a.kslices * sp / a.splits), ks1 = (int)((long long)a.kslices * (sp + 1) / a.splits);
  const int HW = a.HW, M = a.M;
  const int r = lane & 31, gs = lane >> 5;
  S16_T(0);
#ifdef PRN_S16_TIMING
  if (t == 0 && blockIdx.x + gridDim.x * blockIdx.y < 8192) {
    unsigned hw, xcc; asm volatile("s_getreg_b32 %0, hwreg(HW_REG_HW_ID)" : "=s"(hw)); asm volatile("s_getreg_b32 %0, hwreg(HW_REG_XCC_ID)" : "=s"(xcc));
    prn_s16_dbg[(blockIdx.x + gridDim.x * blockIdx.y) * 6 + 4] = ((long long)(xcc & 15) << 32) | hw;
  }
#endif
  const int px = pt * 128 + wave * 32 + r;
  const int pxc = px < HW ? px : HW - 1;
  const int XHW = TAPS ? a.XH * a.XW : HW;
  const int XK = TAPS ? a.C : a.K;
  const float* xb = a.x + (long long)z * a.zx + (long long)b * XK * XHW;
  const __amdgpu_buffer_rsrc_t xrs = __builtin_amdgcn_make_buffer_rsrc(const_cast<float*>(xb), 0, XK * XHW * 4, 0x00020000);
  const int xoff = (pxc + gs * 8 * HW) * 4;
  int choff[16];
#pragma unroll
  for (int j = 0; j < 16; ++j) choff[j] = __builtin_amdgcn_readfirstlane(min(((j >> 3) * 16 + (j & 7)) * XHW * 4, XK * XHW * 4));
  const int t_oi = TAPS ? pxc / a.Wo : 0, t_oj = TAPS ? pxc - t_oi * a.Wo : 0;
  const int t_iy0 = t_oi * a.stride - a.pad, t_ix0 = t_oj * a.stride - a.pad;
  auto tap_vo = [&](int ks_) -> int {
    const int k0 = ks_ * BK, tp = __builtin_amdgcn_readfirstlane(k0 / a.C), c0 = __builtin_amdgcn_readfirstlane(k0 - tp * a.C);
    const int ty = __builtin_amdgcn_readfirstlane(tp / a.KW), tx = __builtin_amdgcn_readfirstlane(tp - ty * a.KW);
    int iy = t_iy0 + ty, ix = t_ix0 + tx;
    bool ok = (unsigned)iy < (unsigned)a.XH && (unsigned)ix < (unsigned)a.XW && k0 < a.K;
    if (TAPS == 2) {
      iy = min(max(t_oi + (z >> 1) - 1 + ty, 0), a.XH - 1); ix = min(max(t_oj + (z & 1) - 1 + tx, 0), a.XW - 1);
      ok = k0 < a.K;
    }
    return ok ? (iy * a.XW + ix + (c0 + gs * 8) * XHW) * 4 : (int)0x80000000u;
  };
  const uint4* ag = a.img + ((long long)(z * a.mtiles + mt) * a.kslices) * IMG16_U4;
  const i32x4_t adesc = make_desc(ag, (unsigned)a.kslices * IMG16_U4 * 16u);
  const unsigned lds0 = (unsigned)(unsigned long long)(void*)lds;
  float rn[16];
  f16x8_t bp[2][2];
  int erun = -1000, de = 0;
  const unsigned podd = (unsigned)__builtin_popcount((unsigned)px) & 1u;
  const unsigned sflip16 = podd ? 0x80008000u : 0u, sflip32 = podd ? 0x80000000u : 0u;
#define S16_DMA(ks_, st_) do { \
    _Pragma("unroll") for (int i = 0; i < 4; ++i) \
// ... 73 lines not shown
    __builtin_amdgcn_sched_barrier(0);
    S16_STEP(1);
    S16_IT(1);
    S16_IT(2);
    if (more) S16_PIECES(); else de = 0;
    __builtin_amdgcn_sched_barrier(0);
    S16_LOADB(ks + 2);
    S16_IT(3);
  }
#undef S16_DMA
#undef S16_LOADB
#undef S16_PIECES
#undef S16_STEP
  S16_T(2);
  const bool cok = px < HW;
  const int* exm = a.ex + (long long)z * a.mtiles * 128 + mt * 128;
  float* yb = a.y + (long long)z * a.zy + (long long)b * M * HW;
  const float* ab = a.addend ? a.addend + (long long)z * a.zy + (long long)b * M * HW : nullptr;
  float* pb = a.splits > 1 ? a.partial + (long long)sp * a.slice + ((long long)z * a.B + b) * (long long)M * HW : nullptr;
  if (a.wide) {
    __syncthreads();
    float* cw = reinterpret_cast<float*>(lds) + wave * (32 * 36);
    int* exl = reinterpret_cast<int*>(lds) + 4 * (32 * 36);
    if (t < 128) exl[t] = exm[t];
    __syncthreads();
    const int crow = lane >> 3, ccol = (lane & 7) * 4;
    const int px4 = pt * 128 + wave * 32 + ccol;
    const bool pok = px4 < HW;
    const bool fin = a.splits == 1;
#pragma unroll
    for (int i = 0; i < 4; ++i) {
#pragma unroll
      for (int e = 0; e < 16; ++e) {
        const int ro = (e >> 2) * 8 + (e & 3) + gs * 4;
        cw[ro * 36 + r] = __uint_as_float(__float_as_uint(ldexpf(acc[i][e], erun + exl[i * 32 + ro] - 28)) ^ sflip32);
      }
      __builtin_amdgcn_wave_barrier();
#pragma unroll
      for (int q = 0; q < 4; ++q) {
        const int rl = crow + 8 * q, row = mt * BM + i * 32 + rl;
        float4 v = *reinterpret_cast<const float4*>(&cw[rl * 36 + ccol]);
        if (!pok || row >= M) continue;
        const long long idx = (long long)row * HW + px4;
        if (TAPS == 2) {
          if (a.bias) { const float bm = a.bias[row]; v.x += bm; v.y += bm; v.z += bm; v.w += bm; }
          if (a.epi == PRN_EPI_RELU) { v.x = fmaxf(v.x, 0.f); v.y = fmaxf(v.y, 0.f); v.z = fmaxf(v.z, 0.f); v.w = fmaxf(v.w, 0.f); }
          const int oi4 = px4 / a.Wo, oj4 = px4 - oi4 * a.Wo;
          float* yp = a.y + (((long long)b * M + row) * (2 * a.XH) + 2 * oi4 + (z >> 1)) * (2 * a.XW) + 2 * oj4 + (z & 1);
          yp[0] = v.x; yp[2] = v.y; yp[4] = v.z; yp[6] = v.w;
          continue;
        }
        if (fin) {
          if (a.bias) { const float bm = a.bias[row]; v.x += bm; v.y += bm; v.z += bm; v.w += bm; }
          if (ab) { const float4 t4 = *reinterpret_cast<const float4*>(ab + idx); v.x += t4.x; v.y += t4.y; v.z += t4.z; v.w += t4.w; }
          if (a.epi == PRN_EPI_RELU) { v.x = fmaxf(v.x, 0.f); v.y = fmaxf(v.y, 0.f); v.z = fmaxf(v.z, 0.f); v.w = fmaxf(v.w, 0.f); }
          else if (a.epi == PRN_EPI_SIGMOID) { v.x = 1.f / (1.f + expf(-v.x)); v.y = 1.f / (1.f + expf(-v.y)); v.z = 1.f / (1.f + expf(-v.z)); v.w = 1.f / (1.f + expf(-v.w)); }
          store4_policy(yb + idx, v, a.store_policy);
        } else {
          store4_policy(pb + idx, v, a.store_policy);
        }
      }
      __builtin_amdgcn_wave_barrier();
    }
#ifdef PRN_S16_TIMING
    asm volatile("s_waitcnt vmcnt(0)" ::: "memory");
#endif
    S16_T(3);
    return;
  }
  if (a.splits > 1) {
#pragma unroll
    for (int i = 0; i < 4; ++i)
#pragma unroll
      for (int e = 0; e < 16; ++e) {
        const int rl = i * 32 + gs * 4 + (e >> 2) * 8 + (e & 3), row = mt * BM + rl;
        if (cok && row < M) pb[(long long)row * HW + px] = __uint_as_float(__float_as_uint(ldexpf(acc[i][e], erun + exm[rl] - 28)) ^ sflip32);
      }
    return;
  }
#pragma unroll
  for (int i = 0; i < 4; ++i) {
    const int rl0 = i * 32 + gs * 4, rbase = mt * BM + rl0;
    float bv[16], av[16]; int ev[16];
#pragma unroll
    for (int e = 0; e < 16; ++e) {
      const int ro = (e >> 2) * 8 + (e & 3), row = rbase + ro; const int rc = row < M ? row : M - 1;
      bv[e] = a.bias ? a.bias[rc] : 0.f; av[e] = ab ? ab[(long long)rc * HW + pxc] : 0.f; ev[e] = exm[rl0 + ro];
    }
#pragma unroll
    for (int e = 0; e < 16; ++e) {
      const int row = rbase + (e >> 2) * 8 + (e & 3);
      float v = __uint_as_float(__float_as_uint(ldexpf(acc[i][e], erun + ev[e] - 28)) ^ sflip32) + bv[e] + av[e];
      if (a.epi == PRN_EPI_RELU) v = fmaxf(v, 0.f);
      else if (a.epi == PRN_EPI_SIGMOID) v = 1.f / (1.f + expf(-v));
      if (cok && row < M) yb[(long long)row * HW + px] = v;
    }
  }
}

struct PrepItem { const float* src; uint4* dst; int M, K, nz, pad; long long zw; long long first; };
__global__ void split_prepare_batched_kernel(const PrepItem* __restrict__ items, int n) {
  int lo = 0, hi = n - 1;
  const long long blk = blockIdx.x;
  while (lo < hi) { const int mid = (lo + hi + 1) >> 1; if (items[mid].first <= blk) lo = mid; else hi = mid - 1; }
  const PrepItem it = items[lo];
  const int mtiles = (it.M + 127) / 128, kslices = (it.K + 31) / 32;
  const long long total = (long long)it.nz * mtiles * kslices * 512;
  const long long i = (blk - it.first) * 256 + threadIdx.x;
  if (i >= total) return;
  const int g = i % 4; const int r = (i / 4) % 128; const long long t = i / 512;
  const int ks = t % kslices; const long long zm = t / kslices; const int mt = zm % mtiles; const long long z = zm / mtiles;
  const int m = mt * 128 + r, k0 = ks * 32 + g * 8;
  float v[8];
#pragma unroll
  for (int j = 0; j < 8; ++j) v[j] = (m < it.M && k0 + j < it.K) ? it.src[z * (long long)it.M * it.K + (long long)m * it.K + k0 + j] : 0.f;
  uint4 h, mm, l;
  split2(v[0], v[1], h.x, mm.x, l.x); split2(v[2], v[3], h.y, mm.y, l.y); split2(v[4], v[5], h.z, mm.z, l.z); split2(v[6], v[7], h.w, mm.w, l.w);
  uint4* o = it.dst + t * IMG_U4;
  o[(0 * 4 + g) * 128 + r] = h; o[(1 * 4 + g) * 128 + r] = mm; o[(2 * 4 + g) * 128 + r] = l;
}

__device__ __forceinline__ PrepItem find_item(const PrepItem* items, int n, long long blk, bool rows) {
  int lo = 0, hi = n - 1;
  while (lo < hi) { const int mid = (lo + hi + 1) >> 1; if ((rows ? items[mid].zw : items[mid].first) <= blk) lo = mid; else hi = mid - 1; }
  return items[lo];
}
__global__ __launch_bounds__(256) void split16_rowmax_batched_kernel(const PrepItem* __restrict__ items, int n) {
  const PrepItem it = find_item(items, n, blockIdx.x, true);
  const int mtiles = (it.M + 127) / 128, Mpad = mtiles * 128;
  const long long rows = (long long)it.nz * Mpad;
  const long long row = ((long long)blockIdx.x - it.zw) * 4 + (threadIdx.x >> 6);
  if (row >= rows) return;
  const int kslices = (it.K + 31) / 32;
  int* ex = (int*)((char*)it.dst + (long long)it.nz * mtiles * kslices * IMG16_U4 * 16);
  const int lane = threadIdx.x & 63;
  const long long z = row / Mpad; const int m = (int)(row - z * Mpad);
  float mx = 0.f;
  if (m < it.M) {
    const float* wr = it.src + z * (long long)it.M * it.K + (long long)m * it.K;
    if ((it.K & 3) == 0 && (reinterpret_cast<uintptr_t>(it.src) & 15) == 0) {
// ... 59 lines not shown
  return splits;
}
extern "C" void prn_gemm_opts_default(prn_gemm_opts* o) {
  if (!o) return;
  o->split_mode = PRN_SPLIT_PLAN; o->split_kind = PRN_PIECES_F16; o->split_products = 3; o->split_min_tiles = 300; o->split_min_gflop = 4.0f;
  o->wgrad_wgs = 0; o->wgrad_target = 0; o->wgrad_split = PRN_SPLIT_PLAN;
}
extern "C" int64_t prn_split_images_bytes(int M, int K, int nz) {
  if (M <= 0 || K <= 0 || nz <= 0) return -1;
  return prn_split_gemm_image_bytes(M, K, nz);
}
extern "C" int prn_split_prepare_batched(const void* items_dev, int n_items, int64_t total_blocks, int64_t total_row_blocks, int kind, void* stream) {
  PRN_REQUIRE(items_dev && n_items > 0 && total_blocks > 0 && total_blocks < (1LL << 31), "prn_split_prepare_batched: bad arguments");
  PRN_REQUIRE(kind == PRN_PIECES_F16 || kind == PRN_PIECES_BF16, "prn_split_prepare_batched: kind is PRN_PIECES_F16 or PRN_PIECES_BF16");
  if (kind == PRN_PIECES_F16) {
    PRN_REQUIRE(total_row_blocks > 0 && total_row_blocks < (1LL << 31), "prn_split_prepare_batched: the fp16 piece format needs the row-block count");
    hipLaunchKernelGGL(split16_rowmax_batched_kernel, dim3((unsigned)total_row_blocks), dim3(256), 0, (hipStream_t)stream, (const PrepItem*)items_dev, n_items);
    hipLaunchKernelGGL(split16_prepare_batched_kernel, dim3((unsigned)total_blocks), dim3(256), 0, (hipStream_t)stream, (const PrepItem*)items_dev, n_items);
    PRN_CHECK_LAUNCH("prn_split_prepare_batched/f16");
    return 0;
  }
  hipLaunchKernelGGL(split_prepare_batched_kernel, dim3((unsigned)total_blocks), dim3(256), 0, (hipStream_t)stream, (const PrepItem*)items_dev, n_items);
  PRN_CHECK_LAUNCH("prn_split_prepare_batched");
  return 0;
}
namespace {
int cut_weight(const float* w, void* images, int M, int K, int nz, long long zw, int kind, hipStream_t st, const char* who, int taps = 1) {
  const int mtiles = cdiv(M, 128), kslices = cdiv(K, 32);
  const long long ptotal = (long long)nz * mtiles * kslices * 512;
  if (kind == PRN_PIECES_F16) {
    int* ex = (int*)((char*)images + (int64_t)nz * mtiles * kslices * IMG16_U4 * 16);
    const long long rows = (long long)nz * mtiles * 128;
    hipLaunchKernelGGL(split16_rowmax_kernel, dim3(cdiv(rows, 4)), dim3(256), 0, st, w, ex, M, K, zw, mtiles * 128, rows);
    hipLaunchKernelGGL(split16_prepare_kernel, dim3(cdiv(ptotal, 256)), dim3(256), 0, st, w, (uint4*)images, (const int*)ex, M, K, zw, mtiles, kslices, ptotal, taps);
  } else {
    hipLaunchKernelGGL(split_prepare_kernel, dim3(cdiv(ptotal, 256)), dim3(256), 0, st, w, (uint4*)images, M, K, zw, mtiles, kslices, ptotal);
  }
  PRN_CHECK_LAUNCH(who);
  return 0;
}
}
extern "C" int prn_split_prepare(const float* w, void* images, int M, int K, int nz, int kind, void* stream) {
  PRN_REQUIRE(w && images && M > 0 && K > 0 && nz > 0 && (reinterpret_cast<uintptr_t>(images) & 15) == 0, "prn_split_prepare: bad arguments");
  PRN_REQUIRE(kind == PRN_PIECES_F16 || kind == PRN_PIECES_BF16, "prn_split_prepare: kind is PRN_PIECES_F16 or PRN_PIECES_BF16");
  return cut_weight(w, images, M, K, nz, (long long)M * K, kind, (hipStream_t)stream, "prn_split_prepare");
}
extern "C" int prn_gemm_pipe(int M, int K, int B, int HW, int nz, const prn_gemm_opts* opts) {
  return prn_split_gemm_plan(M, K, B, HW, nz, opts);
}
int64_t prn_split_gemm_image_bytes(int M, int K, int nz) { return (int64_t)nz * cdiv(M, 128) * cdiv(K, 32) * IMG_U4 * 16 + (int64_t)nz * cdiv(M, 128) * 128 * 4; }
int64_t prn_split_gemm_partial_bytes(int M, int B, int HW, int nz, int splits) { return splits > 1 ? (int64_t)splits * nz * B * M * HW * 4 : 0; }

int prn_split_gemm(const float* w, const void* w_images, const float* x, const float* bias, const float* addend, float* y, void* images_ws, float* partial, int M,
                   int K, int B, int HW, int nz, int64_t zw, int64_t zx, int64_t zy, int epi, int splits, const prn_gemm_opts* o, hipStream_t st, int phase) {
  PRN_REQUIRE(o != nullptr && w && x && y && (splits == 1 || partial), "prn_split_gemm: null operand");
  const int mtiles = cdiv(M, 128), kslices = cdiv(K, 32), ptiles = cdiv(HW, 128);
  PRN_REQUIRE((int64_t)kslices * IMG_U4 * 16 < (1LL << 31) && (int64_t)K * HW < (1LL << 29), "prn_split_gemm: operand larger than a buffer descriptor");
  const int kind = o->split_kind;
  PRN_REQUIRE(kind == PRN_PIECES_F16 || kind == PRN_PIECES_BF16, "prn_split_gemm: unknown piece format %d", kind);
  {
    static const int dbg = prn_env_int("PRN_SPLIT_DEBUG", 0);
    if (dbg) fprintf(stderr, "prn_split_gemm M=%d K=%d B=%d HW=%d nz=%d splits=%d epi=%d addend=%d\n", M, K, B, HW, nz, splits, epi, addend != nullptr);
  }
  if (phase != 2) {
    const void* images = w_images;
    if (images == nullptr) {
      PRN_REQUIRE(images_ws != nullptr, "prn_split_gemm: no workspace for the weight images");
      if (int e = cut_weight(w, images_ws, M, K, nz, (long long)zw, kind, st, "prn_split_gemm/prepare")) return e;
      images = images_ws;
    }
    PRN_REQUIRE((reinterpret_cast<uintptr_t>(images) & 15) == 0, "prn_split_gemm: images must be 16-byte aligned");
    if (kind == PRN_PIECES_F16) {
      Split16Args a;
      a.img = (const uint4*)images; a.ex = (const int*)((const char*)images + (int64_t)nz * mtiles * kslices * IMG16_U4 * 16);
      a.x = x; a.bias = bias; a.addend = addend; a.y = y; a.partial = partial;
      a.M = M; a.K = K; a.B = B; a.HW = HW; a.epi = epi; a.mtiles = mtiles; a.kslices = kslices; a.ptiles = ptiles;
      a.total = mtiles * ptiles * B * nz; a.splits = splits; a.zx = zx; a.zy = zy; a.slice = (long long)nz * B * M * HW;
      a.C = K; a.XH = 1; a.XW = HW; a.Wo = HW; a.KW = 1; a.stride = 1; a.pad = 0;
      {
        auto al16 = [](const void* q) { return (reinterpret_cast<uintptr_t>(q) & 15) == 0; };
        static const int wide_on = prn_env_int("PRN_SPLIT_WIDE_STORE", 1);
        a.wide = wide_on && (HW & 3) == 0 && ((int64_t)M * HW & 3) == 0 && (zy & 3) == 0 && al16(y) && al16(addend) && al16(partial);
        static const int policy = prn_env_int("PRN_SPLIT_STORE_POLICY", 1);
        a.store_policy = policy;
      }
      if (o->split_products >= 4) hipLaunchKernelGGL(split16_gemm_kernel<4>, dim3(a.total, splits), dim3(256), 0, st, a);
      else hipLaunchKernelGGL(split16_gemm_kernel<3>, dim3(a.total, splits), dim3(256), 0, st, a);
      PRN_CHECK_LAUNCH("prn_split_gemm/f16");
    } else {
      SplitArgs a;
      a.img = (const uint4*)images; a.x = x; a.bias = bias; a.addend = addend; a.y = y; a.partial = partial;
      a.M = M; a.K = K; a.B = B; a.HW = HW; a.epi = epi; a.mtiles = mtiles; a.kslices = kslices; a.ptiles = ptiles;
      a.total = mtiles * ptiles * B * nz; a.splits = splits; a.zx = zx; a.zy = zy; a.slice = (long long)nz * B * M * HW;
      hipLaunchKernelGGL(split_gemm_kernel, dim3(a.total, splits), dim3(256), 0, st, a);
      PRN_CHECK_LAUNCH("prn_split_gemm");
    }
  }
  if (splits > 1 && phase != 1) {
    PRN_REQUIRE(nz == 1 || (zy == (int64_t)B * M * HW), "prn_split_gemm: K splits need a dense output");
    return prn_launch_reduce_epilogue(partial, bias, addend, y, (int64_t)nz * B * M * HW, M, HW, splits, epi, st);
  }
  return 0;
}

int prn_split_conv_taps(const float* w, const float* x, const float* bias, const float* addend, float* y, void* images_ws, float* partial, int M, int C, int B, int XH,
                        int XW, int Ho, int Wo, int KH, int KW, int stride, int pad, int epi, int splits, const prn_gemm_opts* o, hipStream_t st, int phase) {
  PRN_REQUIRE(o != nullptr && w && x && y && images_ws && (splits == 1 || partial), "prn_split_conv_taps: null operand");
  PRN_REQUIRE(o->split_kind == PRN_PIECES_F16 && (C & 31) == 0 && KH > 0 && KW > 0, "prn_split_conv_taps: fp16 pieces and C %% 32 == 0 only");
  const int K = KH * KW * C, HW = Ho * Wo;
  const int mtiles = cdiv(M, 128), kslices = K / 32, ptiles = cdiv(HW, 128);
  PRN_REQUIRE((int64_t)kslices * IMG_U4 * 16 < (1LL << 31) && (int64_t)C * XH * XW < (1LL << 29) && (int64_t)M * HW < (1LL << 29),
              "prn_split_conv_taps: operand larger than a buffer descriptor");
  if (phase != 2) {
    if (int e = cut_weight(w, images_ws, M, K, 1, (long long)M * K, PRN_PIECES_F16, st, "prn_split_conv_taps/prepare", KH * KW)) return e;
    Split16Args a;
    a.img = (const uint4*)images_ws; a.ex = (const int*)((const char*)images_ws + (int64_t)mtiles * kslices * IMG16_U4 * 16);
    a.x = x; a.bias = bias; a.addend = addend; a.y = y; a.partial = partial;
    a.M = M; a.K = K; a.B = B; a.HW = HW; a.epi = epi; a.mtiles = mtiles; a.kslices = kslices; a.ptiles = ptiles;
    a.total = mtiles * ptiles * B; a.splits = splits; a.zx = 0; a.zy = 0; a.slice = (long long)B * M * HW;
    a.C = C; a.XH = XH; a.XW = XW; a.Wo = Wo; a.KW = KW; a.stride = stride; a.pad = pad;
    auto al16 = [](const void* q) { return (reinterpret_cast<uintptr_t>(q) & 15) == 0; };
    a.wide = (HW & 3) == 0 && ((int64_t)M * HW & 3) == 0 && al16(y) && al16(addend) && al16(partial);
    a.store_policy = 1;
    if (o->split_products >= 4) hipLaunchKernelGGL((split16_gemm_kernel<4, 1>), dim3(a.total, splits), dim3(256), 0, st, a);
    else hipLaunchKernelGGL((split16_gemm_kernel<3, 1>), dim3(a.total, splits), dim3(256), 0, st, a);
    PRN_CHECK_LAUNCH("prn_split_conv_taps");
  }
  if (splits > 1 && phase != 1) return prn_launch_reduce_epilogue(partial, bias, addend, y, (int64_t)B * M * HW, M, HW, splits, epi, st);
  return 0;
}

int prn_split_conv_up2(const float* wp, const float* x, const float* bias, float* y, void* images_ws, int M, int C, int B, int H, int W, int epi, const prn_gemm_opts* o,
                       hipStream_t st) {
  PRN_REQUIRE(o != nullptr && wp && x && y && images_ws, "prn_split_conv_up2: null operand");
  PRN_REQUIRE(o->split_kind == PRN_PIECES_F16 && (C & 31) == 0 && (W & 3) == 0 && (reinterpret_cast<uintptr_t>(y) & 15) == 0, "prn_split_conv_up2: fp16 pieces, C %% 32 == 0, W %% 4 == 0");
  const int K = 4 * C, HW = H * W;
  const int mtiles = cdiv(M, 128), kslices = K / 32, ptiles = cdiv(HW, 128);
  PRN_REQUIRE((int64_t)kslices * IMG_U4 * 16 < (1LL << 31) && (int64_t)C * HW < (1LL << 29) && (int64_t)B * M * HW * 4 < (1LL << 31), "prn_split_conv_up2: operand too large");
  if (int e = cut_weight(wp, images_ws, M, K, 4, (long long)M * K, PRN_PIECES_F16, st, "prn_split_conv_up2/prepare", 4)) return e;
  Split16Args a;
  a.img = (const uint4*)images_ws; a.ex = (const int*)((const char*)images_ws + (int64_t)4 * mtiles * kslices * IMG16_U4 * 16);
  a.x = x; a.bias = bias; a.addend = nullptr; a.y = y; a.partial = nullptr;
  a.M = M; a.K = K; a.B = B; a.HW = HW; a.epi = epi; a.mtiles = mtiles; a.kslices = kslices; a.ptiles = ptiles;
  a.total = mtiles * ptiles * B * 4; a.splits = 1; a.zx = 0; a.zy = 0; a.slice = 0;
  a.C = C; a.XH = H; a.XW = W; a.Wo = W; a.KW = 2; a.stride = 1; a.pad = 0;
  a.wide = 1; a.store_policy = 1;
  if (o->split_products >= 4) hipLaunchKernelGGL((split16_gemm_kernel<4, 2>), dim3(a.total, 1), dim3(256), 0, st, a);
  else hipLaunchKernelGGL((split16_gemm_kernel<3, 2>), dim3(a.total, 1), dim3(256), 0, st, a);
  PRN_CHECK_LAUNCH("prn_split_conv_up2");
  return 0;
}
```

planerecnet_amd/csrc/prn_norm.hip:

```cpp
#include <stdlib.h>
#include "prn_common.h"

namespace {


__device__ __forceinline__ void slice_bounds(int HW, int s, int S, bool vec, int& beg, int& end) {
  if (vec) {
    const int n4 = HW >> 2;
    beg = (int)((int64_t)n4 * s / S) * 4;
    end = (int)((int64_t)n4 * (s + 1) / S) * 4;
  } else {
    beg = (int)((int64_t)HW * s / S);
    end = (int)((int64_t)HW * (s + 1) / S);
  }
}

__global__ __launch_bounds__(256) void bn_partial_kernel(const float* __restrict__ x, double* __restrict__ ws, int B, int C, int HW) {
  const int c = blockIdx.x, s = blockIdx.y, S = gridDim.y;
  const bool vec = (HW & 3) == 0;
  int beg, end;
  slice_bounds(HW, s, S, vec, beg, end);
  float s1 = 0.f, s2 = 0.f;
  for (int b = 0; b < B; ++b) {
    const float* xp = x + ((size_t)b * C + c) * HW;
    if (vec) {
      for (int p = beg + threadIdx.x * 4; p < end; p += 1024) {
        const float4 v = *reinterpret_cast<const float4*>(xp + p);
        s1 += (v.x + v.y) + (v.z + v.w);
        s2 += (v.x * v.x + v.y * v.y) + (v.z * v.z + v.w * v.w);
      }
    } else {
      for (int p = beg + threadIdx.x; p < end; p += 256) {
        const float v = xp[p];
        s1 += v; s2 += v * v;
      }
    }
  }
  __shared__ double sm[16];
  double d1 = s1, d2 = s2;
  block_sum2(d1, d2, sm);
  if (threadIdx.x == 0) { ws[((size_t)c * S + s) * 2] = d1; ws[((size_t)c * S + s) * 2 + 1] = d2; }
}

__global__ void bn_finalize_kernel(const double* __restrict__ ws, float* __restrict__ stats, float* __restrict__ rmean,
                                   float* __restrict__ rvar, int C, int S, double count, float eps, float momentum) {
  const int c = blockIdx.x * blockDim.x + threadIdx.x;
  if (c >= C) return;
  double s1 = 0.0, s2 = 0.0;
  for (int s = 0; s < S; ++s) { s1 += ws[((size_t)c * S + s) * 2]; s2 += ws[((size_t)c * S + s) * 2 + 1]; }
  const double mean = s1 / count;
  double var = s2 / count - mean * mean;
  if (var < 0.0) var = 0.0;
  stats[c] = (float)mean;
  stats[C + c] = (float)(1.0 / sqrt(var + (double)eps));
  if (rmean) {
    const double unbiased = count > 1.0 ? var * count / (count - 1.0) : var;
    rmean[c] = (1.f - momentum) * rmean[c] + momentum * (float)mean;
    rvar[c] = (1.f - momentum) * rvar[c] + momentum * (float)unbiased;
  }
}

template <bool FIN>
__global__ __launch_bounds__(256) void bn_apply_kernel(const float* __restrict__ x, float* __restrict__ stats,
                                                       const float* __restrict__ gamma, const float* __restrict__ beta,
                                                       const float* __restrict__ res, float* __restrict__ y, int C, int HW, int relu,
                                                       const double* __restrict__ ws, float* __restrict__ rmean, float* __restrict__ rvar,
                                                       int S, double count, float eps, float momentum, int64_t ybs) {
  const int bc = blockIdx.y, c = bc % C;
  float mean_f, istd_f;
  if (FIN) {
    double s1 = 0.0, s2 = 0.0;
    for (int s = 0; s < S; ++s) { s1 += ws[((size_t)c * S + s) * 2]; s2 += ws[((size_t)c * S + s) * 2 + 1]; }
    const double mean = s1 / count;
    double var = s2 / count - mean * mean;
    if (var < 0.0) var = 0.0;
    mean_f = (float)mean;
    istd_f = (float)(1.0 / sqrt(var + (double)eps));
    if (blockIdx.x == 0 && bc == c && threadIdx.x == 0) {
      stats[c] = mean_f;
      stats[C + c] = istd_f;
      if (rmean) {
        const double unbiased = count > 1.0 ? var * count / (count - 1.0) : var;
        rmean[c] = (1.f - momentum) * rmean[c] + momentum * mean_f;
        rvar[c] = (1.f - momentum) * rvar[c] + momentum * (float)unbiased;
      }
    }
  } else {
    mean_f = stats[c];
    istd_f = stats[C + c];
  }
  const float sc = istd_f * gamma[c], sh = beta[c] - mean_f * sc;
  const size_t base = (size_t)bc * HW;
  y += (size_t)(bc / C) * ybs + (size_t)c * HW - base;
  if ((HW & 3) == 0) {
    const int n4 = HW >> 2;
    const float4* xp = reinterpret_cast<const float4*>(x + base);
    const float4* rp = res ? reinterpret_cast<const float4*>(res + base) : nullptr;
    float4* yp = reinterpret_cast<float4*>(y + base);
    for (int i = blockIdx.x * 256 + threadIdx.x; i < n4; i += gridDim.x * 256) {
      float4 v = xp[i];
      v.x = fmaf(v.x, sc, sh); v.y = fmaf(v.y, sc, sh); v.z = fmaf(v.z, sc, sh); v.w = fmaf(v.w, sc, sh);
      if (rp) { const float4 r = rp[i]; v.x += r.x; v.y += r.y; v.z += r.z; v.w += r.w; }
      if (relu) { v.x = fmaxf(v.x, 0.f); v.y = fmaxf(v.y, 0.f); v.z = fmaxf(v.z, 0.f); v.w = fmaxf(v.w, 0.f); }
      yp[i] = v;
    }
  } else {
    for (int i = blockIdx.x * 256 + threadIdx.x; i < HW; i += gridDim.x * 256) {
      float v = fmaf(x[base + i], sc, sh);
      if (res) v += res[base + i];
      if (relu) v = fmaxf(v, 0.f);
      y[base + i] = v;
    }
  }
}

__global__ __launch_bounds__(256) void bn_bwd_partial_kernel(const float* __restrict__ dy, const float* __restrict__ x,
                                                             const float* __restrict__ y, const float* __restrict__ stats,
                                                             double* __restrict__ ws, int B, int C, int HW, int relu, const float* __restrict__ gamma,
                                                             const float* __restrict__ beta, int64_t dbs) {
  const int c = blockIdx.x, s = blockIdx.y, S = gridDim.y;
  const bool vec = (HW & 3) == 0;
  int beg, end;
  slice_bounds(HW, s, S, vec, beg, end);
  const float mean = stats[c], istd = stats[C + c];
  const float sc = relu == 2 ? istd * gamma[c] : 0.f, sh = relu == 2 ? beta[c] - mean * sc : 0.f;
  float s1 = 0.f, s2 = 0.f;
  for (int b = 0; b < B; ++b) {
    const size_t base = ((size_t)b * C + c) * HW;
    const float* dyb = dy + (size_t)b * dbs + (size_t)c * HW;
    if (vec) {
      for (int p = beg + threadIdx.x * 4; p < end; p += 1024) {
        float4 g = *reinterpret_cast<const float4*>(dyb + p);
        const float4 xv = *reinterpret_cast<const float4*>(x + base + p);
        if (relu == 1) {
          const float4 yv = *reinterpret_cast<const float4*>(y + base + p);
          g.x = yv.x > 0.f ? g.x : 0.f; g.y = yv.y > 0.f ? g.y : 0.f; g.z = yv.z > 0.f ? g.z : 0.f; g.w = yv.w > 0.f ? g.w : 0.f;
        } else if (relu == 2) {
          g.x = fmaf(xv.x, sc, sh) > 0.f ? g.x : 0.f; g.y = fmaf(xv.y, sc, sh) > 0.f ? g.y : 0.f;
          g.z = fmaf(xv.z, sc, sh) > 0.f ? g.z : 0.f; g.w = fmaf(xv.w, sc, sh) > 0.f ? g.w : 0.f;
        }
        s1 += (g.x + g.y) + (g.z + g.w);
        s2 += (g.x * (xv.x - mean) + g.y * (xv.y - mean)) + (g.z * (xv.z - mean) + g.w * (xv.w - mean));
      }
    } else {
      for (int p = beg + threadIdx.x; p < end; p += 256) {
        float g = dyb[p];
        if (relu == 1 && !(y[base + p] > 0.f)) g = 0.f;
        if (relu == 2 && !(fmaf(x[base + p], sc, sh) > 0.f)) g = 0.f;
        s1 += g; s2 += g * (x[base + p] - mean);
      }
    }
  }
  s2 *= istd;
  __shared__ double sm[16];
  double d1 = s1, d2 = s2;
  block_sum2(d1, d2, sm);
  if (threadIdx.x == 0) { ws[((size_t)c * S + s) * 2] = d1; ws[((size_t)c * S + s) * 2 + 1] = d2; }
}

__global__ __launch_bounds__(256) void bn_bwd_apply_kernel(const float* __restrict__ dy, const float* __restrict__ x,
                                                           const float* __restrict__ y, const float* __restrict__ stats,
                                                           const float* __restrict__ gamma, const double* __restrict__ ws,
                                                           float* __restrict__ dx, float* __restrict__ dres, int C, int HW,
                                                           int S, float inv_count, int relu, int frozen, int have_partials,
                                                           float* __restrict__ dgamma, float* __restrict__ dbeta,
                                                           const float* __restrict__ beta, int64_t dbs) {
  const int bc = blockIdx.y, c = bc % C;
  const float mean = stats[c], istd = stats[C + c], gi = gamma[c] * istd;
  const float sc = relu == 2 ? gi : 0.f, sh = relu == 2 ? beta[c] - mean * sc : 0.f;
  double t1 = 0.0, t2 = 0.0;
  if (have_partials)
    for (int s = 0; s < S; ++s) { t1 += ws[((size_t)c * S + s) * 2]; t2 += ws[((size_t)c * S + s) * 2 + 1]; }
  if (have_partials && blockIdx.x == 0 && bc == c && threadIdx.x == 0) {
    if (dbeta) dbeta[c] = (float)t1;
    if (dgamma) dgamma[c] = (float)t2;
  }
  const float m1 = frozen ? 0.f : (float)t1 * inv_count;
  const float m2 = frozen ? 0.f : (float)t2 * inv_count;
  const size_t base = (size_t)bc * HW;
  dy += (size_t)(bc / C) * dbs + (size_t)c * HW - base;
  if ((HW & 3) == 0) {
    const int n4 = HW >> 2;
    for (int i = blockIdx.x * 256 + threadIdx.x; i < n4; i += gridDim.x * 256) {
      float4 g = reinterpret_cast<const float4*>(dy + base)[i];
      const float4 xv = reinterpret_cast<const float4*>(x + base)[i];
      if (relu == 1) {
        const float4 yv = reinterpret_cast<const float4*>(y + base)[i];
        g.x = yv.x > 0.f ? g.x : 0.f; g.y = yv.y > 0.f ? g.y : 0.f; g.z = yv.z > 0.f ? g.z : 0.f; g.w = yv.w > 0.f ? g.w : 0.f;
      } else if (relu == 2) {
        g.x = fmaf(xv.x, sc, sh) > 0.f ? g.x : 0.f; g.y = fmaf(xv.y, sc, sh) > 0.f ? g.y : 0.f;
        g.z = fmaf(xv.z, sc, sh) > 0.f ? g.z : 0.f; g.w = fmaf(xv.w, sc, sh) > 0.f ? g.w : 0.f;
      }
      if (dres) reinterpret_cast<float4*>(dres + base)[i] = g;
      float4 o;
      o.x = gi * (g.x - m1 - (xv.x - mean) * istd * m2); o.y = gi * (g.y - m1 - (xv.y - mean) * istd * m2);
      o.z = gi * (g.z - m1 - (xv.z - mean) * istd * m2); o.w = gi * (g.w - m1 - (xv.w - mean) * istd * m2);
      reinterpret_cast<float4*>(dx + base)[i] = o;
    }
    return;
  }
  for (int i = blockIdx.x * 256 + threadIdx.x; i < HW; i += gridDim.x * 256) {
    float g = dy[base + i];
    if (relu == 1 && !(y[base + i] > 0.f)) g = 0.f;
    if (relu == 2 && !(fmaf(x[base + i], sc, sh) > 0.f)) g = 0.f;
    if (dres) dres[base + i] = g;
    const float xh = (x[base + i] - mean) * istd;
    dx[base + i] = gi * (g - m1 - xh * m2);
  }
}

constexpr int BN_SMALL_MAX = 12288;

__device__ __forceinline__ void plane_to_winograd_v(const float* __restrict__ plane, float* __restrict__ V, int c, int C, int B, int H, int W) {
  const int TW = W >> 2, TH = (H + 3) >> 2, P = B * TH * TW, P4 = (P + 3) & ~3, HW = H * W;
  const size_t zs = (size_t)C * P4;
  for (int p = threadIdx.x; p < P; p += 256) {
    const int tx = p % TW, ty = (p / TW) % TH, b = p / (TW * TH);
    const float* pb = plane + b * HW;
    const int w0 = 4 * tx;
    float d[6][6];
#pragma unroll
    for (int i = 0; i < 6; ++i) {
      const int ih = 4 * ty - 1 + i;
      const bool ok = (unsigned)ih < (unsigned)H;
      const float* row = pb + (ok ? ih : 0) * W;
      const float4 q = *reinterpret_cast<const float4*>(row + w0);
      const bool okl = w0 > 0, okr = w0 + 4 < W;
      const float l = row[okl ? w0 - 1 : 0], r = row[okr ? w0 + 4 : 0];
      d[i][0] = (ok && okl) ? l : 0.f;
      d[i][1] = ok ? q.x : 0.f; d[i][2] = ok ? q.y : 0.f; d[i][3] = ok ? q.z : 0.f; d[i][4] = ok ? q.w : 0.f;
      d[i][5] = (ok && okr) ? r : 0.f;
    }
    float t[6][6];
#pragma unroll
    for (int j = 0; j < 6; ++j) {
      float v[6], o[6];
#pragma unroll
      for (int i = 0; i < 6; ++i) v[i] = d[i][j];
      bt6(v, o);
#pragma unroll
      for (int i = 0; i < 6; ++i) t[i][j] = o[i];
    }
    float* out = V + (size_t)c * P4 + p;
#pragma unroll
    for (int i = 0; i < 6; ++i) {
      float o[6];
      bt6(t[i], o);
#pragma unroll
      for (int j = 0; j < 6; ++j) out[(size_t)(i * 6 + j) * zs] = o[j];
    }
  }
}

template <int NV, bool WINO = false>
__global__ __launch_bounds__(256) void bn_small_fwd_kernel(const float* __restrict__ x, float* __restrict__ stats, const float* __restrict__ gamma,
                                                           const float* __restrict__ beta, const float* __restrict__ res, float* __restrict__ y,
                                                           float* __restrict__ rmean, float* __restrict__ rvar, int B, int C, int HW, float eps,
                                                           float momentum, int relu, int64_t ybs, int nparts, int64_t pstride, float* __restrict__ xsum,
                                                           float* __restrict__ V = nullptr, int H = 0, int W = 0) {
  __shared__ float wino_plane[WINO ? BN_SMALL_MAX : 4];
  const int c = blockIdx.x, n4 = (B * HW) >> 2;
  const int64_t ydelta = ybs - (int64_t)C * HW;
  float4 v[NV];
  size_t off[NV];
  float s1 = 0.f, s2 = 0.f;
#pragma unroll
  for (int i = 0; i < NV; ++i) {
    const int q = threadIdx.x + i * 256;
    const int e = q < n4 ? q * 4 : 0, b = e / HW, p = e - b * HW;
    off[i] = ((size_t)b * C + c) * HW + p;
  }
#pragma unroll
  for (int i = 0; i < NV; ++i) v[i] = *reinterpret_cast<const float4*>(x + off[i]);
  __builtin_amdgcn_sched_barrier(0);
  for (int s = 1; s < nparts; ++s) {
    float4 t[NV];
#pragma unroll
    for (int i = 0; i < NV; ++i) t[i] = *reinterpret_cast<const float4*>(x + (size_t)s * pstride + off[i]);
    __builtin_amdgcn_sched_barrier(0);
#pragma unroll
    for (int i = 0; i < NV; ++i) { v[i].x += t[i].x; v[i].y += t[i].y; v[i].z += t[i].z; v[i].w += t[i].w; }
  }
  if (xsum) {
#pragma unroll
    for (int i = 0; i < NV; ++i)
      if (threadIdx.x + i * 256 < n4) *reinterpret_cast<float4*>(xsum + off[i]) = v[i];
  }
#pragma unroll
  for (int i = 0; i < NV; ++i) {
    if (threadIdx.x + i * 256 >= n4) v[i] = make_float4(0.f, 0.f, 0.f, 0.f);
    s1 += (v[i].x + v[i].y) + (v[i].z + v[i].w);
    s2 += (v[i].x * v[i].x + v[i].y * v[i].y) + (v[i].z * v[i].z + v[i].w * v[i].w);
  }
  __shared__ double sm[16];
  double d1 = s1, d2 = s2;
  block_sum2(d1, d2, sm);
  const double count = (double)B * HW, mean = d1 / count;
  double var = d2 / count - mean * mean;
  if (var < 0.0) var = 0.0;
  const float mean_f = (float)mean, istd_f = (float)(1.0 / sqrt(var + (double)eps));
  if (threadIdx.x == 0) {
    stats[c] = mean_f;
    stats[C + c] = istd_f;
    if (rmean) {
      const double unbiased = count > 1.0 ? var * count / (count - 1.0) : var;
      rmean[c] = (1.f - momentum) * rmean[c] + momentum * mean_f;
      rvar[c] = (1.f - momentum) * rvar[c] + momentum * (float)unbiased;
    }
  }
  const float sc = istd_f * gamma[c], sh = beta[c] - mean_f * sc;
  float4 r[NV];
  if (res) {
#pragma unroll
    for (int i = 0; i < NV; ++i) r[i] = *reinterpret_cast<const float4*>(res + off[i]);
    __builtin_amdgcn_sched_barrier(0);
  } else {
#pragma unroll
    for (int i = 0; i < NV; ++i) r[i] = make_float4(0.f, 0.f, 0.f, 0.f);
  }
#pragma unroll
  for (int i = 0; i < NV; ++i) {
    if (threadIdx.x + i * 256 >= n4) continue;
    float4 o = v[i];
    o.x = fmaf(o.x, sc, sh) + r[i].x; o.y = fmaf(o.y, sc, sh) + r[i].y; o.z = fmaf(o.z, sc, sh) + r[i].z; o.w = fmaf(o.w, sc, sh) + r[i].w;
    if (relu) { o.x = fmaxf(o.x, 0.f); o.y = fmaxf(o.y, 0.f); o.z = fmaxf(o.z, 0.f); o.w = fmaxf(o.w, 0.f); }
    size_t oy = off[i];
    if (ydelta) oy += (size_t)(((threadIdx.x + i * 256) * 4) / HW) * ydelta;
    *reinterpret_cast<float4*>(y + oy) = o;
    if constexpr (WINO) *reinterpret_cast<float4*>(&wino_plane[(threadIdx.x + i * 256) * 4]) = o;
  }
  if constexpr (WINO) {
    __syncthreads();
    plane_to_winograd_v(wino_plane, V, c, C, B, H, W);
  }
}

template <int NV, bool WINO = false>
__global__ __launch_bounds__(256) void bn_small_bwd_kernel(const float* __restrict__ dy, const float* __restrict__ x, const float* __restrict__ y,
                                                           const float* __restrict__ stats, const float* __restrict__ gamma,
                                                           const float* __restrict__ beta, float* __restrict__ dx, float* __restrict__ dres,
                                                           float* __restrict__ dgamma, float* __restrict__ dbeta, int B, int C, int HW, int relu,
                                                           int frozen, int64_t dbs, int nparts, int64_t pstride, float* __restrict__ V = nullptr, int H = 0,
                                                           int W = 0) {
  __shared__ float wino_plane[WINO ? BN_SMALL_MAX : 4];
  const int c = blockIdx.x, n4 = (B * HW) >> 2;
  const int64_t ddelta = dbs - (int64_t)C * HW;
  const float mean = stats[c], istd = stats[C + c], gi = gamma[c] * istd;
  const float sc = relu == 2 ? gi : 0.f, sh = relu == 2 ? beta[c] - mean * sc : 0.f;
  float4 g[NV], xv[NV];
  size_t off[NV];
  float s1 = 0.f, s2 = 0.f;
#pragma unroll
  for (int i = 0; i < NV; ++i) {
    const int q = threadIdx.x + i * 256;
    const int e = q < n4 ? q * 4 : 0, b = e / HW, p = e - b * HW;
    off[i] = ((size_t)b * C + c) * HW + p;
  }
#pragma unroll
  for (int i = 0; i < NV; ++i) {
    const int q = threadIdx.x + i * 256;
    g[i] = *reinterpret_cast<const float4*>(dy + off[i] + (ddelta ? (size_t)((q < n4 ? q * 4 : 0) / HW) * ddelta : 0));
    xv[i] = *reinterpret_cast<const float4*>(x + off[i]);
  }
  __builtin_amdgcn_sched_barrier(0);
  for (int s = 1; s < nparts; ++s) {
    float4 t[NV];
#pragma unroll
    for (int i = 0; i < NV; ++i) t[i] = *reinterpret_cast<const float4*>(dy + (size_t)s * pstride + off[i]);
    __builtin_amdgcn_sched_barrier(0);
#pragma unroll
    for (int i = 0; i < NV; ++i) { g[i].x += t[i].x; g[i].y += t[i].y; g[i].z += t[i].z; g[i].w += t[i].w; }
  }
  if (relu == 1) {
    float4 yv[NV];
#pragma unroll
    for (int i = 0; i < NV; ++i) yv[i] = *reinterpret_cast<const float4*>(y + off[i]);
    __builtin_amdgcn_sched_barrier(0);
#pragma unroll
    for (int i = 0; i < NV; ++i) {
      g[i].x = yv[i].x > 0.f ? g[i].x : 0.f; g[i].y = yv[i].y > 0.f ? g[i].y : 0.f;
      g[i].z = yv[i].z > 0.f ? g[i].z : 0.f; g[i].w = yv[i].w > 0.f ? g[i].w : 0.f;
    }
  } else if (relu == 2) {
#pragma unroll
    for (int i = 0; i < NV; ++i) {
      g[i].x = fmaf(xv[i].x, sc, sh) > 0.f ? g[i].x : 0.f; g[i].y = fmaf(xv[i].y, sc, sh) > 0.f ? g[i].y : 0.f;
      g[i].z = fmaf(xv[i].z, sc, sh) > 0.f ? g[i].z : 0.f; g[i].w = fmaf(xv[i].w, sc, sh) > 0.f ? g[i].w : 0.f;
    }
  }
#pragma unroll
  for (int i = 0; i < NV; ++i) {
    if (threadIdx.x + i * 256 >= n4) { g[i] = make_float4(0.f, 0.f, 0.f, 0.f); xv[i] = g[i]; }
    s1 += (g[i].x + g[i].y) + (g[i].z + g[i].w);
    s2 += (g[i].x * (xv[i].x - mean) + g[i].y * (xv[i].y - mean)) + (g[i].z * (xv[i].z - mean) + g[i].w * (xv[i].w - mean));
  }
  s2 *= istd;
  __shared__ double sm[16];
  double t1 = s1, t2 = s2;
  block_sum2(t1, t2, sm);
  if (threadIdx.x == 0) {
    if (dbeta) dbeta[c] = (float)t1;
    if (dgamma) dgamma[c] = (float)t2;
  }
  const float inv_count = 1.f / ((float)B * HW);
  const float m1 = frozen ? 0.f : (float)t1 * inv_count, m2 = frozen ? 0.f : (float)t2 * inv_count;
#pragma unroll
  for (int i = 0; i < NV; ++i) {
    if (threadIdx.x + i * 256 >= n4) continue;
    if (dres) *reinterpret_cast<float4*>(dres + off[i]) = g[i];
    float4 o;
    o.x = gi * (g[i].x - m1 - (xv[i].x - mean) * istd * m2); o.y = gi * (g[i].y - m1 - (xv[i].y - mean) * istd * m2);
    o.z = gi * (g[i].z - m1 - (xv[i].z - mean) * istd * m2); o.w = gi * (g[i].w - m1 - (xv[i].w - mean) * istd * m2);
    *reinterpret_cast<float4*>(dx + off[i]) = o;
    if constexpr (WINO) *reinterpret_cast<float4*>(&wino_plane[(threadIdx.x + i * 256) * 4]) = o;
  }
  if constexpr (WINO) {
    __syncthreads();
    plane_to_winograd_v(wino_plane, V, c, C, B, H, W);
  }
}

bool bn_small_ok(int B, int HW) {
  static const int on = prn_env_int("PRN_BN_SMALL", 1);
  return on && (HW & 3) == 0 && (int64_t)B * HW <= BN_SMALL_MAX;
}
}

extern "C" int prn_bn_kernel_kind(int B, int HW) { return bn_small_ok(B, HW) ? 1 : 0; }

namespace {

struct GnSeg { int nseg; int hw[6]; int off[6]; };
__device__ __forceinline__ int gn_seg_get(const int (&v)[6], int s) {
  int r = v[0];
#pragma unroll
// ... 119 lines not shown
      const float4 xv = *reinterpret_cast<const float4*>(x + base + i);
      const float h0 = (xv.x - mu) * istd, h1 = (xv.y - mu) * istd, h2 = (xv.z - mu) * istd, h3 = (xv.w - mu) * istd;
      if (!(h0 * gc + bc > 0.f)) gg.x = 0.f;
      if (!(h1 * gc + bc > 0.f)) gg.y = 0.f;
      if (!(h2 * gc + bc > 0.f)) gg.z = 0.f;
      if (!(h3 * gc + bc > 0.f)) gg.w = 0.f;
      float4 o;
      o.x = istd * (gc * gg.x - m1 - h0 * m2); o.y = istd * (gc * gg.y - m1 - h1 * m2);
      o.z = istd * (gc * gg.z - m1 - h2 * m2); o.w = istd * (gc * gg.w - m1 - h3 * m2);
      *reinterpret_cast<float4*>(dx + base + i) = o;
    }
    return;
  }
  for (int i = threadIdx.x; i < n; i += blockDim.x) {
    const int c = g * cpg + i / HW;
    float gg = dy[base + i];
    const float xh = (x[base + i] - mu) * istd;
    if (!(xh * gamma[c] + beta[c] > 0.f)) gg = 0.f;
    dx[base + i] = istd * (gamma[c] * gg - m1 - xh * m2);
  }
  (void)tot;
}

int bn_splits(int B, int HW) {
  int s = (int)(((int64_t)B * HW + 8191) / 8192);
  if (s > PRN_BN_SPLITS) s = PRN_BN_SPLITS;
  if (s < 1) s = 1;
  if (s > HW / 4 && HW >= 4) s = HW / 4;
  return s < 1 ? 1 : s;
}

}

extern "C" int prn_bn_stats(const float* x, float* stats, float* running_mean, float* running_var, double* ws,
                            int B, int C, int HW, float eps, float momentum, void* stream) {
  PRN_REQUIRE(x && stats && ws && B > 0 && C > 0 && HW > 0, "prn_bn_stats: bad arguments");
  hipStream_t st = (hipStream_t)stream;
  const int S = bn_splits(B, HW);
  hipLaunchKernelGGL(bn_partial_kernel, dim3(C, S), dim3(256), 0, st, x, ws, B, C, HW);
  PRN_CHECK_LAUNCH("prn_bn_stats/partial");
  hipLaunchKernelGGL(bn_finalize_kernel, dim3(cdiv(C, 128)), dim3(128), 0, st, (const double*)ws, stats, running_mean, running_var, C,
                     S, (double)B * HW, eps, momentum);
  PRN_CHECK_LAUNCH("prn_bn_stats/finalize");
  return 0;
}

extern "C" int prn_bn_apply(const float* x, const float* stats, const float* gamma, const float* beta, const float* residual,
                            float* y, int B, int C, int HW, int relu, void* stream) {
  PRN_REQUIRE(x && stats && gamma && beta && y && B > 0 && C > 0 && HW > 0, "prn_bn_apply: bad arguments");
  int gx = cdiv(HW, 256 * 8);
  if (gx < 1) gx = 1;
  PRN_REQUIRE((int64_t)B * C <= 65535, "prn_bn_apply: B*C too large for grid.y");
  hipLaunchKernelGGL((bn_apply_kernel<false>), dim3(gx, B * C), dim3(256), 0, (hipStream_t)stream, x, const_cast<float*>(stats), gamma, beta,
                     residual, y, C, HW, relu, (const double*)nullptr, (float*)nullptr, (float*)nullptr, 0, 0.0, 0.f, 0.f, (int64_t)C * HW);
  PRN_CHECK_LAUNCH("prn_bn_apply");
  return 0;
}

extern "C" int prn_bn_train_fwd(const float* x, float* stats, const float* gamma, const float* beta, const float* residual, float* y,
                                float* running_mean, float* running_var, double* ws, int B, int C, int HW, float eps, float momentum,
                                int relu, void* stream) {
  return prn_bn_train_fwd_into(x, stats, gamma, beta, residual, y, (int64_t)C * HW, running_mean, running_var, ws, B, C, HW, eps, momentum, relu, stream);
}

extern "C" int prn_bn_train_fwd_into(const float* x, float* stats, const float* gamma, const float* beta, const float* residual, float* y,
                                     int64_t y_batch_stride, float* running_mean, float* running_var, double* ws, int B, int C, int HW, float eps,
                                     float momentum, int relu, void* stream) {
  PRN_REQUIRE(x && stats && gamma && beta && y && B > 0 && C > 0 && HW > 0, "prn_bn_train_fwd: bad arguments");
  PRN_REQUIRE(ws || bn_small_ok(B, HW), "prn_bn_train_fwd: the two-launch path needs its workspace (prn_bn_kernel_kind(B, HW) == 0)");
  PRN_REQUIRE(y_batch_stride >= (int64_t)C * HW && ((HW & 3) || ((y_batch_stride & 3) == 0 && (reinterpret_cast<uintptr_t>(y) & 15) == 0)),
              "prn_bn_train_fwd_into: bad output batch stride / alignment");
  const int64_t ybs = y_batch_stride;
  PRN_REQUIRE((int64_t)B * C <= 65535, "prn_bn_train_fwd: B*C too large for grid.y");
  hipStream_t st = (hipStream_t)stream;
  if (bn_small_ok(B, HW)) {
    const int nv = cdiv(B * HW / 4, 256);
#define PRN_BN_SMALL_FWD(NV_) hipLaunchKernelGGL((bn_small_fwd_kernel<NV_>), dim3(C), dim3(256), 0, st, x, stats, gamma, beta, residual, y, \
                                                 running_mean, running_var, B, C, HW, eps, momentum, relu, ybs, 1, (int64_t)0, (float*)nullptr)
    if (nv <= 3) PRN_BN_SMALL_FWD(3); else if (nv <= 6) PRN_BN_SMALL_FWD(6); else if (nv <= 10) PRN_BN_SMALL_FWD(10); else PRN_BN_SMALL_FWD(12);
#undef PRN_BN_SMALL_FWD
    PRN_CHECK_LAUNCH("prn_bn_train_fwd/small");
    return 0;
  }
  const int S = bn_splits(B, HW);
  for (int r = PRN_REPS(1); r > 0; --r) hipLaunchKernelGGL(bn_partial_kernel, dim3(C, S), dim3(256), 0, st, x, ws, B, C, HW);
  PRN_CHECK_LAUNCH("prn_bn_train_fwd/partial");
  int gx = cdiv(HW, 256 * 8);
  if (gx < 1) gx = 1;
  hipLaunchKernelGGL((bn_apply_kernel<true>), dim3(gx, B * C), dim3(256), 0, st, x, stats, gamma, beta, residual, y, C, HW, relu,
                     (const double*)ws, running_mean, running_var, S, (double)B * HW, eps, momentum, ybs);
  PRN_CHECK_LAUNCH("prn_bn_train_fwd/apply");
  return 0;
}

extern "C" int prn_bn_bwd(const float* dy, const float* x, const float* y, const float* stats, const float* gamma, const float* beta,
                          float* dx, float* dres, float* dgamma, float* dbeta, double* ws,
                          int B, int C, int HW, int relu, int frozen, void* stream) {
  return prn_bn_bwd_from(dy, (int64_t)C * HW, x, y, stats, gamma, beta, dx, dres, dgamma, dbeta, ws, B, C, HW, relu, frozen, stream);
}

extern "C" int prn_bn_bwd_from(const float* dy, int64_t dy_batch_stride, const float* x, const float* y, const float* stats, const float* gamma,
                               const float* beta, float* dx, float* dres, float* dgamma, float* dbeta, double* ws,
                               int B, int C, int HW, int relu, int frozen, void* stream) {
  PRN_REQUIRE(dy && x && stats && gamma && dx && B > 0 && C > 0 && HW > 0, "prn_bn_bwd: bad arguments");
  PRN_REQUIRE(ws || bn_small_ok(B, HW), "prn_bn_bwd: the two-launch path needs its workspace (prn_bn_kernel_kind(B, HW) == 0)");
  PRN_REQUIRE(dy_batch_stride >= (int64_t)C * HW && ((HW & 3) || ((dy_batch_stride & 3) == 0 && (reinterpret_cast<uintptr_t>(dy) & 15) == 0)),
              "prn_bn_bwd_from: bad gradient batch stride / alignment");
  const int64_t dbs = dy_batch_stride;
  PRN_REQUIRE(!relu || y || (beta && !dres), "prn_bn_bwd: relu needs the forward output, or beta (and no residual) to recompute its sign");
  if (relu) relu = y ? 1 : 2;
  PRN_REQUIRE((int64_t)B * C <= 65535, "prn_bn_bwd: B*C too large for grid.y");
  hipStream_t st = (hipStream_t)stream;
  if (bn_small_ok(B, HW)) {
    const int nv = cdiv(B * HW / 4, 256);
#define PRN_BN_SMALL_BWD(NV_) hipLaunchKernelGGL((bn_small_bwd_kernel<NV_>), dim3(C), dim3(256), 0, st, dy, x, y, stats, gamma, beta, dx, dres, dgamma, \
                                                 dbeta, B, C, HW, relu, frozen, dbs, 1, (int64_t)0)
    if (nv <= 3) PRN_BN_SMALL_BWD(3); else if (nv <= 6) PRN_BN_SMALL_BWD(6); else if (nv <= 10) PRN_BN_SMALL_BWD(10); else PRN_BN_SMALL_BWD(12);
#undef PRN_BN_SMALL_BWD
    PRN_CHECK_LAUNCH("prn_bn_bwd/small");
    return 0;
  }
  const int S = bn_splits(B, HW);
  const int have = (!frozen || dgamma || dbeta) ? 1 : 0;
  if (have) {
    for (int r = PRN_REPS(2); r > 0; --r) hipLaunchKernelGGL(bn_bwd_partial_kernel, dim3(C, S), dim3(256), 0, st, dy, x, y, stats, ws, B, C, HW, relu, gamma, beta, dbs);
    PRN_CHECK_LAUNCH("prn_bn_bwd/partial");
  }
  int gx = cdiv(HW, 256 * 8);
  if (gx < 1) gx = 1;
  hipLaunchKernelGGL(bn_bwd_apply_kernel, dim3(gx, B * C), dim3(256), 0, st, dy, x, y, stats, gamma, (const double*)ws, dx, dres, C, HW,
                     S, 1.f / ((float)B * HW), relu, frozen, have, dgamma, dbeta, beta, dbs);
  PRN_CHECK_LAUNCH("prn_bn_bwd/apply");
  return 0;
}

extern "C" int prn_bn_train_fwd_partials(const float* parts, int nparts, int64_t part_stride, float* x_out, float* stats, const float* gamma, const float* beta,
                                         const float* residual, float* y, float* running_mean, float* running_var, int B, int C, int HW, float eps,
                                         float momentum, int relu, void* stream) {
  PRN_REQUIRE(parts && x_out && stats && gamma && beta && y && B > 0 && C > 0 && HW > 0, "prn_bn_train_fwd_partials: bad arguments");
  PRN_REQUIRE(nparts >= 1 && nparts <= 64 && (nparts == 1 || part_stride >= (int64_t)B * C * HW) && (part_stride & 3) == 0,
              "prn_bn_train_fwd_partials: 1..64 partial sums, a multiple of four elements and at least B*C*HW apart");
  PRN_REQUIRE(bn_small_ok(B, HW), "prn_bn_train_fwd_partials: only for maps the one-pass kernel takes (prn_bn_kernel_kind(B, HW) == 1)");
  PRN_REQUIRE(((reinterpret_cast<uintptr_t>(parts) | reinterpret_cast<uintptr_t>(x_out) | reinterpret_cast<uintptr_t>(y)) & 15) == 0,
              "prn_bn_train_fwd_partials: tensors must be 16-byte aligned");
  hipStream_t st = (hipStream_t)stream;
  const int nv = cdiv(B * HW / 4, 256);
  const int64_t ybs = (int64_t)C * HW;
#define PRN_BN_SMALL_FWD(NV_) hipLaunchKernelGGL((bn_small_fwd_kernel<NV_>), dim3(C), dim3(256), 0, st, parts, stats, gamma, beta, residual, y, \
                                                 running_mean, running_var, B, C, HW, eps, momentum, relu, ybs, nparts, part_stride, x_out)
  if (nv <= 3) PRN_BN_SMALL_FWD(3); else if (nv <= 6) PRN_BN_SMALL_FWD(6); else if (nv <= 10) PRN_BN_SMALL_FWD(10); else PRN_BN_SMALL_FWD(12);
#undef PRN_BN_SMALL_FWD
  PRN_CHECK_LAUNCH("prn_bn_train_fwd_partials");
  return 0;
}

extern "C" int prn_bn_bwd_partials(const float* dparts, int nparts, int64_t part_stride, const float* x, const float* y, const float* stats, const float* gamma,
                                   const float* beta, float* dx, float* dres, float* dgamma, float* dbeta, int B, int C, int HW, int relu, int frozen,
                                   void* stream) {
  PRN_REQUIRE(dparts && x && stats && gamma && dx && B > 0 && C > 0 && HW > 0, "prn_bn_bwd_partials: bad arguments");
  PRN_REQUIRE(nparts >= 1 && nparts <= 64 && (nparts == 1 || part_stride >= (int64_t)B * C * HW) && (part_stride & 3) == 0,
              "prn_bn_bwd_partials: 1..64 partial sums, a multiple of four elements and at least B*C*HW apart");
  PRN_REQUIRE(bn_small_ok(B, HW), "prn_bn_bwd_partials: only for maps the one-pass kernel takes (prn_bn_kernel_kind(B, HW) == 1)");
  PRN_REQUIRE((reinterpret_cast<uintptr_t>(dparts) & 15) == 0, "prn_bn_bwd_partials: partial sums must be 16-byte aligned");
  PRN_REQUIRE(!relu || y || (beta && !dres), "prn_bn_bwd_partials: relu needs the forward output, or beta (and no residual) to recompute its sign");
  if (relu) relu = y ? 1 : 2;
  hipStream_t st = (hipStream_t)stream;
  const int nv = cdiv(B * HW / 4, 256);
  const int64_t dbs = (int64_t)C * HW;
#define PRN_BN_SMALL_BWD(NV_) hipLaunchKernelGGL((bn_small_bwd_kernel<NV_>), dim3(C), dim3(256), 0, st, dparts, x, y, stats, gamma, beta, dx, dres, dgamma, \
                                                 dbeta, B, C, HW, relu, frozen, dbs, nparts, part_stride)
  if (nv <= 3) PRN_BN_SMALL_BWD(3); else if (nv <= 6) PRN_BN_SMALL_BWD(6); else if (nv <= 10) PRN_BN_SMALL_BWD(10); else PRN_BN_SMALL_BWD(12);
#undef PRN_BN_SMALL_BWD
  PRN_CHECK_LAUNCH("prn_bn_bwd_partials");
  return 0;
}

extern "C" int prn_bn_train_fwd_winograd(const float* parts, int nparts, int64_t part_stride, float* x_out, float* stats, const float* gamma, const float* beta,
                                         const float* residual, float* y, float* running_mean, float* running_var, float* V, int B, int C, int H, int W,
                                         float eps, float momentum, int relu, void* stream) {
  const int HW = H * W;
  PRN_REQUIRE(parts && stats && gamma && beta && y && V && B > 0 && C > 0 && H >= 5 && W >= 4 && (W & 3) == 0, "prn_bn_train_fwd_winograd: bad arguments");
  PRN_REQUIRE(nparts >= 1 && nparts <= 64 && (nparts == 1 || (x_out && part_stride >= (int64_t)B * C * HW)) && (part_stride & 3) == 0,
              "prn_bn_train_fwd_winograd: 1..64 partial sums (x_out required beyond one), a multiple of four elements and at least B*C*HW apart");
  PRN_REQUIRE(bn_small_ok(B, HW), "prn_bn_train_fwd_winograd: only for maps the one-pass kernel takes (prn_bn_kernel_kind(B, HW) == 1)");
// ... 110 lines not shown
```

Before: 190.2.

## Save ReLU sign bitmask in bottleneck forward and gate residual gradient in backward

The final BN+residual+ReLU of each bottleneck now also writes a 1-bit-per-element ReLU gate mask (a nibble per float4, stored as one byte). Backward BN reads this mask instead of the full output tensor y. For identity blocks, the residual-gradient tensor is never materialised: the mask is applied to dy directly in the split-GEMM epilogue of the conv1 data-gradient. This removes a full fp32 read of y and a write and read of dres per block, at the cost of a small extra mask write in forward and more plumbing through the GEMM and BN kernels.

```diff
diff --git a/include/prn.h b/include/prn.h
--- a/include/prn.h
+++ b/include/prn.h
@@ -237,7 +237,8 @@
 enum { PRN_BLK_WINOGRAD = 1,
        PRN_BLK_HANDOVER = 2,
        PRN_BLK_KEEP_V = 4,
-       PRN_BLK_SCATTER_ACC = 8 };
+       PRN_BLK_SCATTER_ACC = 8,
+       PRN_BLK_GATE = 16 };
 enum { PRN_BLK_CONV2_DIRECT = 0, PRN_BLK_CONV2_WINOGRAD = 1, PRN_BLK_CONV2_DCN = 2 };
 typedef struct prn_bottleneck_desc {
   int32_t B, C, H, W;
diff --git a/planerecnet_amd/blocks.py b/planerecnet_amd/blocks.py
--- a/planerecnet_amd/blocks.py
+++ b/planerecnet_amd/blocks.py
@@ -12,7 +12,7 @@
 SCATTER_ACCUMULATE = os.environ.get("PRN_SCATTER_ACC", "1") == "1"
 STATS = {"fwd": 0, "bwd": 0, "resolved": 0, "vouched": 0, "scatter_acc": 0}
 
-BLK_WINOGRAD, BLK_HANDOVER, BLK_KEEP_V, BLK_SCATTER_ACC = 1, 2, 4, 8
+BLK_WINOGRAD, BLK_HANDOVER, BLK_KEEP_V, BLK_SCATTER_ACC, BLK_GATE = 1, 2, 4, 8, 16
 CONV2_DIRECT, CONV2_WINOGRAD, CONV2_DCN = 0, 1, 2
 (I_SAVE, I_GSAVE, I_FWD_WS, I_BWD_WS, I_HO, I_WO, I_CONV2, I_KEEPS_V, I_A1, I_V, I_A2, I_OM, I_TABLE, I_D1, I_D2, I_D3, I_DD, I_DOM, I_BN_FLOATS, I_HANDOVERS,
  I_W1_IMG, I_W3_IMG, I_WD_IMG, I_W1T_IMG, I_W3T_IMG, I_WDT_IMG, I_U_IMG, I_COLT_IMG, INFO_COUNT) = range(29)
@@ -59,7 +59,7 @@
     if ops.WINOGRAD and ops.WINOGRAD_WGRAD:
         f |= BLK_KEEP_V
     if HANDOVER:
-        f |= BLK_HANDOVER
+        f |= BLK_HANDOVER | BLK_GATE
     return f
 
 
diff --git a/planerecnet_amd/csrc/prn_bottleneck.hip b/planerecnet_amd/csrc/prn_bottleneck.hip
--- a/planerecnet_amd/csrc/prn_bottleneck.hip
+++ b/planerecnet_amd/csrc/prn_bottleneck.hip
@@ -3,7 +3,7 @@
 
 namespace {
 
-constexpr int32_t PLAN_MAGIC = 0x424c4b36;
+constexpr int32_t PLAN_MAGIC = 0x424c4b37;
 constexpr int64_t WINOGRAD_MIN_TILES = 128;
 
 inline int64_t up256(int64_t v) { return (v + 255) & ~255LL; }
@@ -17,11 +17,11 @@
   int32_t v1, lazy2, keep_v;
   int32_t lazy3g, parts3g;
   int32_t v2g, lazy2g;
-  int32_t pad2_;
+  int32_t gate, gadd;
   int64_t parts1_off, parts3g_off;
   prn_conv_desc c1, c2, c3, cd, c27, g1, g2, g3, gd, g27;
   prn_dcn_desc dcn;
-  int64_t s_c1, s_a1, s_v, s_c2, s_a2, s_c3, s_cd, s_om, s_table, s_stats[4], save_bytes;
+  int64_t s_c1, s_a1, s_v, s_c2, s_a2, s_c3, s_cd, s_om, s_table, s_stats[4], s_gate, save_bytes;
   int64_t q_d3, q_dd, q_d2, q_d1, q_dom, q_bn, gsave_bytes;
   int64_t f_c1, f_bn, f_v, f_yt, f_gemm, f_c2, f_c27, f_dcn, f_c3, f_cd, f_res, fwd_ws_bytes;
   int64_t b_bn, b_dres, b_g3, b_g3ws, b_v, b_yt, b_gemm, b_g2, b_g2ws, b_dcn, b_dx1, b_g27ws, b_g1ws, b_gdtmp, b_gdws, bwd_ws_bytes;
@@ -93,6 +93,10 @@
   L.parts3g = L.lazy3g ? p3 : 0; L.parts3g_off = L.lazy3g ? off : 0;
   L.v2g = ho && wino && L.small2;
   L.lazy2g = ho && wino && L.small1 && L.P4 <= 768;
+  static const int gate_on = prn_env_int("PRN_BLK_GATE", 1);
+  L.gate = ho && (d.flags & PRN_BLK_GATE) && gate_on && ((Ho * Wo) & 3) == 0;
+  L.gadd = L.gate && !d.downsample && prn_conv2d_gated_addend_ok(&L.g1);
+  const bool need_dres = !L.gate || (!d.downsample && !L.gadd);
   const int64_t n1 = (int64_t)B * P * H * W * 4, n2 = (int64_t)B * P * Ho * Wo * 4, n3 = (int64_t)B * Q * Ho * Wo * 4, nx = (int64_t)B * C * H * W * 4;
   const int64_t nv = wino ? 4LL * 36 * P * L.P4 : 0, nom = (int64_t)B * 27 * Ho * Wo * 4;
   const int Cmax = Q > C ? Q : C;
@@ -121,6 +125,7 @@
   put(L.s_cd, d.downsample ? n3 : 0);
   put(L.s_om, d.dcn ? nom : 0); put(L.s_table, n_table);
   put(L.s_stats[0], 8LL * P); put(L.s_stats[1], 8LL * P); put(L.s_stats[2], 8LL * Q); put(L.s_stats[3], d.downsample ? 8LL * Q : 0);
+  put(L.s_gate, L.gate ? n3 / 16 : 0);
   L.save_bytes = at;
   at = 0;
   put(L.q_d3, n3); put(L.q_dd, d.downsample ? n3 : 0); put(L.q_d2, n2); put(L.q_d1, n1); put(L.q_dom, d.dcn ? nom : 0);
@@ -133,7 +138,7 @@
   put(L.f_res, d.downsample ? n3 : 0);
   L.fwd_ws_bytes = at;
   at = 0;
-  put(L.b_bn, bnws); put(L.b_dres, n3);
+  put(L.b_bn, bnws); put(L.b_dres, need_dres ? n3 : 0);
   put(L.b_g3, n2); put(L.b_g3ws, w_g3);
   put(L.b_v, nv); put(L.b_yt, nv); put(L.b_gemm, w_gemm);
   put(L.b_g2, n1); put(L.b_g2ws, w_g2);
@@ -178,7 +183,8 @@
   out[PRN_BLK_OFF_A1] = L->s_a1; out[PRN_BLK_OFF_V] = L->s_v; out[PRN_BLK_OFF_A2] = L->s_a2; out[PRN_BLK_OFF_OM] = L->s_om; out[PRN_BLK_OFF_TABLE] = L->s_table;
   out[PRN_BLK_OFF_D1] = L->q_d1; out[PRN_BLK_OFF_D2] = L->q_d2; out[PRN_BLK_OFF_D3] = L->q_d3; out[PRN_BLK_OFF_DD] = L->q_dd; out[PRN_BLK_OFF_DOM] = L->q_dom;
   out[PRN_BLK_BN_GRAD_FLOATS] = L->q_bn;
-  out[PRN_BLK_HANDOVERS] = L->lazy1 | (L->v1 << 1) | (L->lazy2 << 2) | (L->lazy3g << 3) | (L->v2g << 4) | (L->lazy2g << 5);
+  out[PRN_BLK_HANDOVERS] = L->lazy1 | (L->v1 << 1) | (L->lazy2 << 2) | (L->lazy3g << 3) | (L->v2g << 4) | (L->lazy2g << 5) | (L->gate << 6) |
+                           (L->gadd << 7);
   out[PRN_BLK_NEEDS_W1_IMG] = prn_conv2d_kernel_kind(&L->c1) >= 2; out[PRN_BLK_NEEDS_W3_IMG] = prn_conv2d_kernel_kind(&L->c3) >= 2;
   out[PRN_BLK_NEEDS_WD_IMG] = (L->d.downsample && L->d.stride == 1 && prn_conv2d_kernel_kind(&L->cd) >= 2) ? 1 : 0;
   out[PRN_BLK_NEEDS_W1T_IMG] = prn_conv2d_kernel_kind(&L->g1) >= 2; out[PRN_BLK_NEEDS_W3T_IMG] = prn_conv2d_kernel_kind(&L->g3) >= 2;
@@ -247,6 +253,9 @@
                              d.momentum[3], 0, stream));
     res = rd;
   }
+  if (L.gate)
+    return prn_bn_train_fwd_gate(c3, st3, p->gamma[2], p->beta[2], res, y, (unsigned char*)save + L.s_gate, p->running_mean[2], p->running_var[2],
+                                 L.small2 ? nullptr : bnws, B, Q, Ho * Wo, d.eps[2], d.momentum[2], 1, stream);
   return prn_bn_train_fwd(c3, st3, p->gamma[2], p->beta[2], res, y, p->running_mean[2], p->running_var[2], L.small2 ? nullptr : bnws, B, Q, Ho * Wo, d.eps[2], d.momentum[2],
                           1, stream);
 }
@@ -273,14 +282,21 @@
   float* d3 = f32(gsave, L.q_d3); float* d2 = f32(gsave, L.q_d2); float* d1 = f32(gsave, L.q_d1);
   float* dg1 = bn_grads; float* db1 = dg1 + P; float* dg2 = db1 + P; float* db2 = dg2 + P; float* dg3 = db2 + P; float* db3 = dg3 + Q; float* dgd = db3 + Q; float* dbd = dgd + Q;
   double* bnws = (double*)raw(ws, L.b_bn);
-  float* dres = f32(ws, L.b_dres);
+  const unsigned char* gate = L.gate ? (const unsigned char*)save + L.s_gate : nullptr;
+  float* dres = (!L.gate || (!d.downsample && !L.gadd)) ? f32(ws, L.b_dres) : nullptr;
   const prn_gemm_opts* o = &d.opts;
   hipStream_t st = (hipStream_t)stream;
-  PRN_TRY(prn_bn_bwd(dy, c3, y, st3, p->gamma[2], p->beta[2], d3, dres, dg3, db3, L.small2 ? nullptr : bnws, B, Q, Ho * Wo, 1, 0, stream));
+  if (gate)
+    PRN_TRY(prn_bn_bwd_gate(dy, c3, gate, st3, p->gamma[2], p->beta[2], d3, dres, dg3, db3, L.small2 ? nullptr : bnws, B, Q, Ho * Wo, 0, stream));
+  else
+    PRN_TRY(prn_bn_bwd(dy, c3, y, st3, p->gamma[2], p->beta[2], d3, dres, dg3, db3, L.small2 ? nullptr : bnws, B, Q, Ho * Wo, 1, 0, stream));
   const float* addx = dres;
   if (d.downsample) {
     float* dd = f32(gsave, L.q_dd);
-    PRN_TRY(prn_bn_bwd(dres, f32(save, L.s_cd), nullptr, std_, p->gamma[3], p->beta[3], dd, nullptr, dgd, dbd, L.small2 ? nullptr : bnws, B, Q, Ho * Wo, 0, 0, stream));
+    if (gate)
+      PRN_TRY(prn_bn_bwd_gate(dy, f32(save, L.s_cd), gate, std_, p->gamma[3], p->beta[3], dd, nullptr, dgd, dbd, L.small2 ? nullptr : bnws, B, Q, Ho * Wo, 0, stream));
+    else
+      PRN_TRY(prn_bn_bwd(dres, f32(save, L.s_cd), nullptr, std_, p->gamma[3], p->beta[3], dd, nullptr, dgd, dbd, L.small2 ? nullptr : bnws, B, Q, Ho * Wo, 0, 0, stream));
     void* gws = raw(ws, L.b_gdws, L.bwd_ws_bytes - L.b_gdws);
     if (d.stride == 1) {
       float* tmp = f32(ws, L.b_gdtmp);
@@ -329,5 +345,6 @@
     PRN_TRY(prn_winograd_output_bn_bwd(Ytg, c1, st1, p->gamma[0], p->beta[0], d1, dg1, db1, B, P, H, W, 1, stream));
   else
     PRN_TRY(prn_bn_bwd(g2, c1, nullptr, st1, p->gamma[0], p->beta[0], d1, nullptr, dg1, db1, L.small1 ? nullptr : bnws, B, P, H * W, 1, 0, stream));
+  if (L.gadd) return prn_conv2d_fwd_gated(&L.g1, d1, p->w1_t, p->w1_t_img, dy, gate, dx, raw(ws, L.b_g1ws, L.b_gdtmp - L.b_g1ws), stream);
   return prn_conv2d_fwd_counted(&L.g1, d1, p->w1_t, p->w1_t_img, nullptr, addx, dx, raw(ws, L.b_g1ws, L.b_gdtmp - L.b_g1ws), nullptr, stream, 0);
 }
diff --git a/planerecnet_amd/csrc/prn_common.h b/planerecnet_amd/csrc/prn_common.h
--- a/planerecnet_amd/csrc/prn_common.h
+++ b/planerecnet_amd/csrc/prn_common.h
@@ -113,11 +113,18 @@
   o[3] = d12 + 8.f * d34 + m[5];
 }
 
+__device__ __forceinline__ unsigned prn_gate_bits(const float4& o) {
+  return (o.x > 0.f ? 1u : 0u) | (o.y > 0.f ? 2u : 0u) | (o.z > 0.f ? 4u : 0u) | (o.w > 0.f ? 8u : 0u);
+}
+__device__ __forceinline__ void prn_gate_apply(float4& g, unsigned bits) {
+  g.x = (bits & 1u) ? g.x : 0.f; g.y = (bits & 2u) ? g.y : 0.f; g.z = (bits & 4u) ? g.z : 0.f; g.w = (bits & 8u) ? g.w : 0.f;
+}
+
 static inline int cdiv(int64_t a, int64_t b) { return (int)((a + b - 1) / b); }
 __host__ __device__ inline size_t prn_align256(size_t v) { return (v + 255) & ~(size_t)255; }
 
 int prn_launch_reduce_epilogue(const float* ws, const float* bias, const float* addend, float* y, int64_t total, int M, int HoWo, int splits,
-                               int epi, hipStream_t st);
+                               int epi, hipStream_t st, const unsigned char* gate = nullptr);
 int prn_launch_reduce_splits(const float* ws, float* out, int64_t n, int splits, hipStream_t st);
 int prn_quantise_splits(int64_t tiles, int splits);
 int prn_gemm_batched_epi(int M, int C, int P, int nb, const float* U, const void* u_images, const float* V, float* Y, void* ws, const prn_gemm_opts* opts, int epi,
@@ -127,7 +134,8 @@
 int64_t prn_split_gemm_image_bytes(int M, int K, int nz);
 int64_t prn_split_gemm_partial_bytes(int M, int B, int HW, int nz, int splits);
 int prn_split_gemm(const float* w, const void* w_images, const float* x, const float* bias, const float* addend, float* y, void* images_ws, float* partial, int M,
-                   int K, int B, int HW, int nz, int64_t zw, int64_t zx, int64_t zy, int epi, int splits, const prn_gemm_opts* opts, hipStream_t st, int phase);
+                   int K, int B, int HW, int nz, int64_t zw, int64_t zx, int64_t zy, int epi, int splits, const prn_gemm_opts* opts, hipStream_t st, int phase,
+                   const unsigned char* gate = nullptr);
 int prn_split_conv_taps(const float* w, const float* x, const float* bias, const float* addend, float* y, void* images_ws, float* partial, int M, int C, int B, int XH,
                         int XW, int Ho, int Wo, int KH, int KW, int stride, int pad, int epi, int splits, const prn_gemm_opts* o, hipStream_t st, int phase);
 int prn_split_conv_up2(const float* wp, const float* x, const float* bias, float* y, void* images_ws, int M, int C, int B, int H, int W, int epi, const prn_gemm_opts* o,
@@ -139,6 +147,14 @@
   return z;
 }
 
+int prn_bn_train_fwd_gate(const float* x, float* stats, const float* gamma, const float* beta, const float* residual, float* y, unsigned char* gate,
+                          float* running_mean, float* running_var, double* ws, int B, int C, int HW, float eps, float momentum, int relu, void* stream);
+int prn_bn_bwd_gate(const float* dy, const float* x, const unsigned char* gate, const float* stats, const float* gamma, const float* beta, float* dx, float* dres,
+                    float* dgamma, float* dbeta, double* ws, int B, int C, int HW, int frozen, void* stream);
+int prn_conv2d_gated_addend_ok(const prn_conv_desc* d);
+int prn_conv2d_fwd_gated(const prn_conv_desc* d, const float* x, const float* w, const void* w_images, const float* addend, const unsigned char* gate, float* y,
+                         void* ws, void* stream);
+
 int prn_wgrad16_plan(int M, int C, int64_t N, int HW, int nz, const prn_gemm_opts* opts);
 int prn_wgrad16_launch(const float* dy, const float* x, const float* const* gdy, const float* const* gx, int ngroup, float* out, int M, int C, int B, int HW, int nz,
                        int64_t zdy, int64_t zx, int splits, const prn_gemm_opts* opts, hipStream_t st);
diff --git a/planerecnet_amd/csrc/prn_conv.hip b/planerecnet_amd/csrc/prn_conv.hip
--- a/planerecnet_amd/csrc/prn_conv.hip
+++ b/planerecnet_amd/csrc/prn_conv.hip
@@ -915,7 +915,7 @@
 
 __global__ __launch_bounds__(256) void reduce_epilogue_kernel(const float* __restrict__ ws, const float* __restrict__ bias,
                                                                const float* __restrict__ addend, float* __restrict__ y, int64_t total,
-                                                               int M, int HoWo, int splits, int epi) {
+                                                               int M, int HoWo, int splits, int epi, const unsigned char* __restrict__ gate) {
   const int64_t i = ((int64_t)blockIdx.x * 256 + threadIdx.x) * 4;
   if (i >= total) return;
   if (i + 3 < total && (HoWo & 3) == 0) {
@@ -926,7 +926,11 @@
     }
     const int m = (int)((i / HoWo) % M);
     if (bias) { const float bm = bias[m]; v.x += bm; v.y += bm; v.z += bm; v.w += bm; }
-    if (addend) { const float4 t = *reinterpret_cast<const float4*>(addend + i); v.x += t.x; v.y += t.y; v.z += t.z; v.w += t.w; }
+    if (addend) {
+      float4 t = *reinterpret_cast<const float4*>(addend + i);
+      if (gate) prn_gate_apply(t, gate[i >> 2]);
+      v.x += t.x; v.y += t.y; v.z += t.z; v.w += t.w;
+    }
     if (epi == PRN_EPI_RELU) { v.x = fmaxf(v.x, 0.f); v.y = fmaxf(v.y, 0.f); v.z = fmaxf(v.z, 0.f); v.w = fmaxf(v.w, 0.f); }
     else if (epi == PRN_EPI_SIGMOID) { v.x = 1.f / (1.f + __expf(-v.x)); v.y = 1.f / (1.f + __expf(-v.y)); v.z = 1.f / (1.f + __expf(-v.z)); v.w = 1.f / (1.f + __expf(-v.w)); }
     *reinterpret_cast<float4*>(y + i) = v;
@@ -1404,8 +1408,9 @@
 }
 
 int prn_launch_reduce_epilogue(const float* ws, const float* bias, const float* addend, float* y, int64_t total, int M, int HoWo, int splits,
-                               int epi, hipStream_t st) {
-  hipLaunchKernelGGL(reduce_epilogue_kernel, dim3(cdiv(total, 1024)), dim3(256), 0, st, ws, bias, addend, y, total, M, HoWo, splits, epi);
+                               int epi, hipStream_t st, const unsigned char* gate) {
+  PRN_REQUIRE(gate == nullptr || (addend != nullptr && (HoWo & 3) == 0 && (total & 3) == 0), "reduce_epilogue: a gated addend needs HoWo %% 4 == 0");
+  hipLaunchKernelGGL(reduce_epilogue_kernel, dim3(cdiv(total, 1024)), dim3(256), 0, st, ws, bias, addend, y, total, M, HoWo, splits, epi, gate);
   PRN_CHECK_LAUNCH("reduce_epilogue");
   return 0;
 }
@@ -1501,6 +1506,22 @@
 extern "C" int prn_conv2d_fwd_counted(const prn_conv_desc* d, const float* x, const float* w, const void* w_images, const float* bias, const float* addend,
                                       float* y, void* ws, unsigned* counters, void* stream, int phase) {
   return conv_fwd_impl(d, nullptr, x, w, bias, addend, y, ws, stream, phase, counters, w_images);
+}
+
+int prn_conv2d_gated_addend_ok(const prn_conv_desc* d) {
+  if (check_desc(d, "prn_conv2d_gated_addend_ok")) return 0;
+  if (direct_small_m(d) || direct_one_c(d) || d->epilogue != PRN_EPI_NONE || ((d->H * d->W) & 3) != 0) return 0;
+  const int ss = split_plan_of(d);
+  return (ss > 1 || (ss == 1 && d->opts.split_kind == PRN_PIECES_F16)) ? 1 : 0;
+}
+int prn_conv2d_fwd_gated(const prn_conv_desc* d, const float* x, const float* w, const void* w_images, const float* addend, const unsigned char* gate, float* y,
+                         void* ws, void* stream) {
+  PRN_REQUIRE(prn_conv2d_gated_addend_ok(d), "prn_conv2d_fwd_gated: this descriptor's launch takes no gated addend");
+  PRN_REQUIRE(x && w && y && addend && gate && ws, "prn_conv2d_fwd_gated: null tensor / workspace");
+  const int ss = split_plan_of(d);
+  const int64_t ib = (prn_split_gemm_image_bytes(d->M, d->C, 1) + 255) & ~255LL;
+  return prn_split_gemm(w, w_images, x, nullptr, addend, y, ws, (float*)((char*)ws + ib), d->M, d->C, d->B, d->H * d->W, 1, 0, 0, 0, d->epilogue, ss, &d->opts,
+                        (hipStream_t)stream, 0, gate);
 }
 
 extern "C" int prn_conv2d_fwd_ragged(const prn_conv_desc* d, const prn_ragged* rg, const float* x, const float* w, const float* bias,
@@ -1606,7 +1627,7 @@
   if (p.splits > 1) {
     const int64_t total = (int64_t)a.B * a.M * a.HoWo;
     hipLaunchKernelGGL(reduce_epilogue_kernel, dim3(cdiv(total, 1024)), dim3(256), 0, st, (const float*)ws, bias, addend, y, total, a.M, a.HoWo,
-                       p.splits, a.epi);
+                       p.splits, a.epi, (const unsigned char*)nullptr);
     PRN_CHECK_LAUNCH("prn_conv2d_fwd/reduce");
   } else if (tail_pieces > 1 && (mode == PRN_IN_ZERO || mode == PRN_IN_REFLECT) && (d->KH == 1 || d->KH == 3)) {
     const int64_t total = (int64_t)a.B * a.M * a.HoWo;
diff --git a/planerecnet_amd/csrc/prn_gemm_split.hip b/planerecnet_amd/csrc/prn_gemm_split.hip
--- a/planerecnet_amd/csrc/prn_gemm_split.hip
+++ b/planerecnet_amd/csrc/prn_gemm_split.hip
@@ -253,6 +253,7 @@
   int store_policy;
   long long zx, zy, slice;
   int C, XH, XW, Wo, KW, stride, pad;
+  const unsigned char* gate;
 };
 
 template <int NP, int TAPS = 0>
@@ -432,7 +433,11 @@
         }
         if (fin) {
           if (a.bias) { const float bm = a.bias[row]; v.x += bm; v.y += bm; v.z += bm; v.w += bm; }
-          if (ab) { const float4 t4 = *reinterpret_cast<const float4*>(ab + idx); v.x += t4.x; v.y += t4.y; v.z += t4.z; v.w += t4.w; }
+          if (ab) {
+            float4 t4 = *reinterpret_cast<const float4*>(ab + idx);
+            if (a.gate) prn_gate_apply(t4, a.gate[((long long)b * M * HW + idx) >> 2]);
+            v.x += t4.x; v.y += t4.y; v.z += t4.z; v.w += t4.w;
+          }
           if (a.epi == PRN_EPI_RELU) { v.x = fmaxf(v.x, 0.f); v.y = fmaxf(v.y, 0.f); v.z = fmaxf(v.z, 0.f); v.w = fmaxf(v.w, 0.f); }
           else if (a.epi == PRN_EPI_SIGMOID) { v.x = 1.f / (1.f + expf(-v.x)); v.y = 1.f / (1.f + expf(-v.y)); v.z = 1.f / (1.f + expf(-v.z)); v.w = 1.f / (1.f + expf(-v.w)); }
           store4_policy(yb + idx, v, a.store_policy);
@@ -466,6 +471,7 @@
     for (int e = 0; e < 16; ++e) {
       const int ro = (e >> 2) * 8 + (e & 3), row = rbase + ro; const int rc = row < M ? row : M - 1;
       bv[e] = a.bias ? a.bias[rc] : 0.f; av[e] = ab ? ab[(long long)rc * HW + pxc] : 0.f; ev[e] = exm[rl0 + ro];
+      if (ab && a.gate && !((a.gate[((long long)b * M * HW + (long long)rc * HW + pxc) >> 2] >> (pxc & 3)) & 1)) av[e] = 0.f;
     }
 #pragma unroll
     for (int e = 0; e < 16; ++e) {
@@ -631,8 +637,11 @@
 int64_t prn_split_gemm_partial_bytes(int M, int B, int HW, int nz, int splits) { return splits > 1 ? (int64_t)splits * nz * B * M * HW * 4 : 0; }
 
 int prn_split_gemm(const float* w, const void* w_images, const float* x, const float* bias, const float* addend, float* y, void* images_ws, float* partial, int M,
-                   int K, int B, int HW, int nz, int64_t zw, int64_t zx, int64_t zy, int epi, int splits, const prn_gemm_opts* o, hipStream_t st, int phase) {
+                   int K, int B, int HW, int nz, int64_t zw, int64_t zx, int64_t zy, int epi, int splits, const prn_gemm_opts* o, hipStream_t st, int phase,
+                   const unsigned char* gate) {
   PRN_REQUIRE(o != nullptr && w && x && y && (splits == 1 || partial), "prn_split_gemm: null operand");
+  PRN_REQUIRE(gate == nullptr || (addend && nz == 1 && (HW & 3) == 0 && (splits > 1 || o->split_kind == PRN_PIECES_F16)),
+              "prn_split_gemm: a gated addend needs one dense output with HW %% 4 == 0, and fp16 pieces or a K split");
   const int mtiles = cdiv(M, 128), kslices = cdiv(K, 32), ptiles = cdiv(HW, 128);
   PRN_REQUIRE((int64_t)kslices * IMG_U4 * 16 < (1LL << 31) && (int64_t)K * HW < (1LL << 29), "prn_split_gemm: operand larger than a buffer descriptor");
   const int kind = o->split_kind;
@@ -655,7 +664,7 @@
       a.x = x; a.bias = bias; a.addend = addend; a.y = y; a.partial = partial;
       a.M = M; a.K = K; a.B = B; a.HW = HW; a.epi = epi; a.mtiles = mtiles; a.kslices = kslices; a.ptiles = ptiles;
       a.total = mtiles * ptiles * B * nz; a.splits = splits; a.zx = zx; a.zy = zy; a.slice = (long long)nz * B * M * HW;
-      a.C = K; a.XH = 1; a.XW = HW; a.Wo = HW; a.KW = 1; a.stride = 1; a.pad = 0;
+      a.C = K; a.XH = 1; a.XW = HW; a.Wo = HW; a.KW = 1; a.stride = 1; a.pad = 0; a.gate = gate;
       {
         auto al16 = [](const void* q) { return (reinterpret_cast<uintptr_t>(q) & 15) == 0; };
         static const int wide_on = prn_env_int("PRN_SPLIT_WIDE_STORE", 1);
@@ -677,7 +686,7 @@
   }
   if (splits > 1 && phase != 1) {
     PRN_REQUIRE(nz == 1 || (zy == (int64_t)B * M * HW), "prn_split_gemm: K splits need a dense output");
-    return prn_launch_reduce_epilogue(partial, bias, addend, y, (int64_t)nz * B * M * HW, M, HW, splits, epi, st);
+    return prn_launch_reduce_epilogue(partial, bias, addend, y, (int64_t)nz * B * M * HW, M, HW, splits, epi, st, gate);
   }
   return 0;
 }
@@ -697,7 +706,7 @@
     a.x = x; a.bias = bias; a.addend = addend; a.y = y; a.partial = partial;
     a.M = M; a.K = K; a.B = B; a.HW = HW; a.epi = epi; a.mtiles = mtiles; a.kslices = kslices; a.ptiles = ptiles;
     a.total = mtiles * ptiles * B; a.splits = splits; a.zx = 0; a.zy = 0; a.slice = (long long)B * M * HW;
-    a.C = C; a.XH = XH; a.XW = XW; a.Wo = Wo; a.KW = KW; a.stride = stride; a.pad = pad;
+    a.C = C; a.XH = XH; a.XW = XW; a.Wo = Wo; a.KW = KW; a.stride = stride; a.pad = pad; a.gate = nullptr;
     auto al16 = [](const void* q) { return (reinterpret_cast<uintptr_t>(q) & 15) == 0; };
     a.wide = (HW & 3) == 0 && ((int64_t)M * HW & 3) == 0 && al16(y) && al16(addend) && al16(partial);
     a.store_policy = 1;
@@ -722,7 +731,7 @@
   a.x = x; a.bias = bias; a.addend = nullptr; a.y = y; a.partial = nullptr;
   a.M = M; a.K = K; a.B = B; a.HW = HW; a.epi = epi; a.mtiles = mtiles; a.kslices = kslices; a.ptiles = ptiles;
   a.total = mtiles * ptiles * B * 4; a.splits = 1; a.zx = 0; a.zy = 0; a.slice = 0;
-  a.C = C; a.XH = H; a.XW = W; a.Wo = W; a.KW = 2; a.stride = 1; a.pad = 0;
+  a.C = C; a.XH = H; a.XW = W; a.Wo = W; a.KW = 2; a.stride = 1; a.pad = 0; a.gate = nullptr;
   a.wide = 1; a.store_policy = 1;
   if (o->split_products >= 4) hipLaunchKernelGGL((split16_gemm_kernel<4, 2>), dim3(a.total, 1), dim3(256), 0, st, a);
   else hipLaunchKernelGGL((split16_gemm_kernel<3, 2>), dim3(a.total, 1), dim3(256), 0, st, a);
diff --git a/planerecnet_amd/csrc/prn_norm.hip b/planerecnet_amd/csrc/prn_norm.hip
--- a/planerecnet_amd/csrc/prn_norm.hip
+++ b/planerecnet_amd/csrc/prn_norm.hip
@@ -65,7 +65,8 @@
                                                        const float* __restrict__ gamma, const float* __restrict__ beta,
                                                        const float* __restrict__ res, float* __restrict__ y, int C, int HW, int relu,
                                                        const double* __restrict__ ws, float* __restrict__ rmean, float* __restrict__ rvar,
-                                                       int S, double count, float eps, float momentum, int64_t ybs) {
+                                                       int S, double count, float eps, float momentum, int64_t ybs,
+                                                       unsigned char* __restrict__ gate) {
   const int bc = blockIdx.y, c = bc % C;
   float mean_f, istd_f;
   if (FIN) {
@@ -103,6 +104,7 @@
       if (rp) { const float4 r = rp[i]; v.x += r.x; v.y += r.y; v.z += r.z; v.w += r.w; }
       if (relu) { v.x = fmaxf(v.x, 0.f); v.y = fmaxf(v.y, 0.f); v.z = fmaxf(v.z, 0.f); v.w = fmaxf(v.w, 0.f); }
       yp[i] = v;
+      if (gate) gate[(base >> 2) + i] = (unsigned char)prn_gate_bits(v);
     }
   } else {
     for (int i = blockIdx.x * 256 + threadIdx.x; i < HW; i += gridDim.x * 256) {
@@ -117,7 +119,8 @@
 __global__ __launch_bounds__(256) void bn_bwd_partial_kernel(const float* __restrict__ dy, const float* __restrict__ x,
                                                              const float* __restrict__ y, const float* __restrict__ stats,
                                                              double* __restrict__ ws, int B, int C, int HW, int relu, const float* __restrict__ gamma,
-                                                             const float* __restrict__ beta, int64_t dbs) {
+                                                             const float* __restrict__ beta, int64_t dbs,
+                                                             const unsigned char* __restrict__ gate) {
   const int c = blockIdx.x, s = blockIdx.y, S = gridDim.y;
   const bool vec = (HW & 3) == 0;
   int beg, end;
@@ -138,6 +141,8 @@
         } else if (relu == 2) {
           g.x = fmaf(xv.x, sc, sh) > 0.f ? g.x : 0.f; g.y = fmaf(xv.y, sc, sh) > 0.f ? g.y : 0.f;
           g.z = fmaf(xv.z, sc, sh) > 0.f ? g.z : 0.f; g.w = fmaf(xv.w, sc, sh) > 0.f ? g.w : 0.f;
+        } else if (relu == 3) {
+          prn_gate_apply(g, gate[(base + p) >> 2]);
         }
         s1 += (g.x + g.y) + (g.z + g.w);
         s2 += (g.x * (xv.x - mean) + g.y * (xv.y - mean)) + (g.z * (xv.z - mean) + g.w * (xv.w - mean));
@@ -164,7 +169,8 @@
                                                            float* __restrict__ dx, float* __restrict__ dres, int C, int HW,
                                                            int S, float inv_count, int relu, int frozen, int have_partials,
                                                            float* __restrict__ dgamma, float* __restrict__ dbeta,
-                                                           const float* __restrict__ beta, int64_t dbs) {
+                                                           const float* __restrict__ beta, int64_t dbs,
+                                                           const unsigned char* __restrict__ gate) {
   const int bc = blockIdx.y, c = bc % C;
   const float mean = stats[c], istd = stats[C + c], gi = gamma[c] * istd;
   const float sc = relu == 2 ? gi : 0.f, sh = relu == 2 ? beta[c] - mean * sc : 0.f;
@@ -190,6 +196,8 @@
       } else if (relu == 2) {
         g.x = fmaf(xv.x, sc, sh) > 0.f ? g.x : 0.f; g.y = fmaf(xv.y, sc, sh) > 0.f ? g.y : 0.f;
         g.z = fmaf(xv.z, sc, sh) > 0.f ? g.z : 0.f; g.w = fmaf(xv.w, sc, sh) > 0.f ? g.w : 0.f;
+      } else if (relu == 3) {
+        prn_gate_apply(g, gate[(base >> 2) + i]);
       }
       if (dres) reinterpret_cast<float4*>(dres + base)[i] = g;
       float4 o;
@@ -257,7 +265,8 @@
                                                            const float* __restrict__ beta, const float* __restrict__ res, float* __restrict__ y,
                                                            float* __restrict__ rmean, float* __restrict__ rvar, int B, int C, int HW, float eps,
                                                            float momentum, int relu, int64_t ybs, int nparts, int64_t pstride, float* __restrict__ xsum,
-                                                           float* __restrict__ V = nullptr, int H = 0, int W = 0) {
+                                                           float* __restrict__ V = nullptr, int H = 0, int W = 0,
+                                                           unsigned char* __restrict__ gate = nullptr) {
   __shared__ float wino_plane[WINO ? BN_SMALL_MAX : 4];
   const int c = blockIdx.x, n4 = (B * HW) >> 2;
   const int64_t ydelta = ybs - (int64_t)C * HW;
@@ -327,6 +336,7 @@
     size_t oy = off[i];
     if (ydelta) oy += (size_t)(((threadIdx.x + i * 256) * 4) / HW) * ydelta;
     *reinterpret_cast<float4*>(y + oy) = o;
+    if (gate) gate[off[i] >> 2] = (unsigned char)prn_gate_bits(o);
     if constexpr (WINO) *reinterpret_cast<float4*>(&wino_plane[(threadIdx.x + i * 256) * 4]) = o;
   }
   if constexpr (WINO) {
@@ -341,7 +351,7 @@
                                                            const float* __restrict__ beta, float* __restrict__ dx, float* __restrict__ dres,
                                                            float* __restrict__ dgamma, float* __restrict__ dbeta, int B, int C, int HW, int relu,
                                                            int frozen, int64_t dbs, int nparts, int64_t pstride, float* __restrict__ V = nullptr, int H = 0,
-                                                           int W = 0) {
+                                                           int W = 0, const unsigned char* __restrict__ gate = nullptr) {
   __shared__ float wino_plane[WINO ? BN_SMALL_MAX : 4];
   const int c = blockIdx.x, n4 = (B * HW) >> 2;
   const int64_t ddelta = dbs - (int64_t)C * HW;
@@ -381,6 +391,13 @@
       g[i].x = yv[i].x > 0.f ? g[i].x : 0.f; g[i].y = yv[i].y > 0.f ? g[i].y : 0.f;
       g[i].z = yv[i].z > 0.f ? g[i].z : 0.f; g[i].w = yv[i].w > 0.f ? g[i].w : 0.f;
     }
+  } else if (relu == 3) {
+    unsigned gb[NV];
+#pragma unroll
+    for (int i = 0; i < NV; ++i) gb[i] = gate[off[i] >> 2];
+    __builtin_amdgcn_sched_barrier(0);
+#pragma unroll
+    for (int i = 0; i < NV; ++i) prn_gate_apply(g[i], gb[i]);
   } else if (relu == 2) {
 #pragma unroll
     for (int i = 0; i < NV; ++i) {
@@ -606,7 +623,8 @@
   if (gx < 1) gx = 1;
   PRN_REQUIRE((int64_t)B * C <= 65535, "prn_bn_apply: B*C too large for grid.y");
   hipLaunchKernelGGL((bn_apply_kernel<false>), dim3(gx, B * C), dim3(256), 0, (hipStream_t)stream, x, const_cast<float*>(stats), gamma, beta,
-                     residual, y, C, HW, relu, (const double*)nullptr, (float*)nullptr, (float*)nullptr, 0, 0.0, 0.f, 0.f, (int64_t)C * HW);
+                     residual, y, C, HW, relu, (const double*)nullptr, (float*)nullptr, (float*)nullptr, 0, 0.0, 0.f, 0.f, (int64_t)C * HW,
+                     (unsigned char*)nullptr);
   PRN_CHECK_LAUNCH("prn_bn_apply");
   return 0;
 }
@@ -617,9 +635,25 @@
   return prn_bn_train_fwd_into(x, stats, gamma, beta, residual, y, (int64_t)C * HW, running_mean, running_var, ws, B, C, HW, eps, momentum, relu, stream);
 }
 
+static int bn_train_fwd_impl(const float* x, float* stats, const float* gamma, const float* beta, const float* residual, float* y,
+                             int64_t y_batch_stride, float* running_mean, float* running_var, double* ws, int B, int C, int HW, float eps,
+                             float momentum, int relu, void* stream, unsigned char* gate);
+
 extern "C" int prn_bn_train_fwd_into(const float* x, float* stats, const float* gamma, const float* beta, const float* residual, float* y,
                                      int64_t y_batch_stride, float* running_mean, float* running_var, double* ws, int B, int C, int HW, float eps,
                                      float momentum, int relu, void* stream) {
+  return bn_train_fwd_impl(x, stats, gamma, beta, residual, y, y_batch_stride, running_mean, running_var, ws, B, C, HW, eps, momentum, relu, stream, nullptr);
+}
+
+int prn_bn_train_fwd_gate(const float* x, float* stats, const float* gamma, const float* beta, const float* residual, float* y, unsigned char* gate,
+                          float* running_mean, float* running_var, double* ws, int B, int C, int HW, float eps, float momentum, int relu, void* stream) {
+  PRN_REQUIRE(gate != nullptr && (HW & 3) == 0, "prn_bn_train_fwd_gate: the gate needs HW %% 4 == 0");
+  return bn_train_fwd_impl(x, stats, gamma, beta, residual, y, (int64_t)C * HW, running_mean, running_var, ws, B, C, HW, eps, momentum, relu, stream, gate);
+}
+
+static int bn_train_fwd_impl(const float* x, float* stats, const float* gamma, const float* beta, const float* residual, float* y,
+                             int64_t y_batch_stride, float* running_mean, float* running_var, double* ws, int B, int C, int HW, float eps,
+                             float momentum, int relu, void* stream, unsigned char* gate) {
   PRN_REQUIRE(x && stats && gamma && beta && y && B > 0 && C > 0 && HW > 0, "prn_bn_train_fwd: bad arguments");
   PRN_REQUIRE(ws || bn_small_ok(B, HW), "prn_bn_train_fwd: the two-launch path needs its workspace (prn_bn_kernel_kind(B, HW) == 0)");
   PRN_REQUIRE(y_batch_stride >= (int64_t)C * HW && ((HW & 3) || ((y_batch_stride & 3) == 0 && (reinterpret_cast<uintptr_t>(y) & 15) == 0)),
@@ -630,7 +664,8 @@
   if (bn_small_ok(B, HW)) {
     const int nv = cdiv(B * HW / 4, 256);
 #define PRN_BN_SMALL_FWD(NV_) hipLaunchKernelGGL((bn_small_fwd_kernel<NV_>), dim3(C), dim3(256), 0, st, x, stats, gamma, beta, residual, y, \
-                                                 running_mean, running_var, B, C, HW, eps, momentum, relu, ybs, 1, (int64_t)0, (float*)nullptr)
+                                                 running_mean, running_var, B, C, HW, eps, momentum, relu, ybs, 1, (int64_t)0, (float*)nullptr, \
+                                                 (float*)nullptr, 0, 0, gate)
     if (nv <= 3) PRN_BN_SMALL_FWD(3); else if (nv <= 6) PRN_BN_SMALL_FWD(6); else if (nv <= 10) PRN_BN_SMALL_FWD(10); else PRN_BN_SMALL_FWD(12);
 #undef PRN_BN_SMALL_FWD
     PRN_CHECK_LAUNCH("prn_bn_train_fwd/small");
@@ -642,7 +677,7 @@
   int gx = cdiv(HW, 256 * 8);
   if (gx < 1) gx = 1;
   hipLaunchKernelGGL((bn_apply_kernel<true>), dim3(gx, B * C), dim3(256), 0, st, x, stats, gamma, beta, residual, y, C, HW, relu,
-                     (const double*)ws, running_mean, running_var, S, (double)B * HW, eps, momentum, ybs);
+                     (const double*)ws, running_mean, running_var, S, (double)B * HW, eps, momentum, ybs, gate);
   PRN_CHECK_LAUNCH("prn_bn_train_fwd/apply");
   return 0;
 }
@@ -653,22 +688,38 @@
   return prn_bn_bwd_from(dy, (int64_t)C * HW, x, y, stats, gamma, beta, dx, dres, dgamma, dbeta, ws, B, C, HW, relu, frozen, stream);
 }
 
+static int bn_bwd_impl(const float* dy, int64_t dy_batch_stride, const float* x, const float* y, const float* stats, const float* gamma,
+                       const float* beta, float* dx, float* dres, float* dgamma, float* dbeta, double* ws,
+                       int B, int C, int HW, int relu, int frozen, void* stream, const unsigned char* gate);
+
 extern "C" int prn_bn_bwd_from(const float* dy, int64_t dy_batch_stride, const float* x, const float* y, const float* stats, const float* gamma,
                                const float* beta, float* dx, float* dres, float* dgamma, float* dbeta, double* ws,
                                int B, int C, int HW, int relu, int frozen, void* stream) {
+  return bn_bwd_impl(dy, dy_batch_stride, x, y, stats, gamma, beta, dx, dres, dgamma, dbeta, ws, B, C, HW, relu, frozen, stream, nullptr);
+}
+
+int prn_bn_bwd_gate(const float* dy, const float* x, const unsigned char* gate, const float* stats, const float* gamma, const float* beta, float* dx, float* dres,
+                    float* dgamma, float* dbeta, double* ws, int B, int C, int HW, int frozen, void* stream) {
+  PRN_REQUIRE(gate != nullptr && (HW & 3) == 0, "prn_bn_bwd_gate: the gate needs HW %% 4 == 0");
+  return bn_bwd_impl(dy, (int64_t)C * HW, x, nullptr, stats, gamma, beta, dx, dres, dgamma, dbeta, ws, B, C, HW, 1, frozen, stream, gate);
+}
+
+static int bn_bwd_impl(const float* dy, int64_t dy_batch_stride, const float* x, const float* y, const float* stats, const float* gamma,
+                       const float* beta, float* dx, float* dres, float* dgamma, float* dbeta, double* ws,
+                       int B, int C, int HW, int relu, int frozen, void* stream, const unsigned char* gate) {
   PRN_REQUIRE(dy && x && stats && gamma && dx && B > 0 && C > 0 && HW > 0, "prn_bn_bwd: bad arguments");
   PRN_REQUIRE(ws || bn_small_ok(B, HW), "prn_bn_bwd: the two-launch path needs its workspace (prn_bn_kernel_kind(B, HW) == 0)");
   PRN_REQUIRE(dy_batch_stride >= (int64_t)C * HW && ((HW & 3) || ((dy_batch_stride & 3) == 0 && (reinterpret_cast<uintptr_t>(dy) & 15) == 0)),
               "prn_bn_bwd_from: bad gradient batch stride / alignment");
   const int64_t dbs = dy_batch_stride;
-  PRN_REQUIRE(!relu || y || (beta && !dres), "prn_bn_bwd: relu needs the forward output, or beta (and no residual) to recompute its sign");
-  if (relu) relu = y ? 1 : 2;
+  PRN_REQUIRE(!relu || y || gate || (beta && !dres), "prn_bn_bwd: relu needs the forward output, or beta (and no residual) to recompute its sign");
+  if (relu) relu = gate ? 3 : (y ? 1 : 2);
   PRN_REQUIRE((int64_t)B * C <= 65535, "prn_bn_bwd: B*C too large for grid.y");
   hipStream_t st = (hipStream_t)stream;
   if (bn_small_ok(B, HW)) {
     const int nv = cdiv(B * HW / 4, 256);
 #define PRN_BN_SMALL_BWD(NV_) hipLaunchKernelGGL((bn_small_bwd_kernel<NV_>), dim3(C), dim3(256), 0, st, dy, x, y, stats, gamma, beta, dx, dres, dgamma, \
-                                                 dbeta, B, C, HW, relu, frozen, dbs, 1, (int64_t)0)
+                                                 dbeta, B, C, HW, relu, frozen, dbs, 1, (int64_t)0, (float*)nullptr, 0, 0, gate)
     if (nv <= 3) PRN_BN_SMALL_BWD(3); else if (nv <= 6) PRN_BN_SMALL_BWD(6); else if (nv <= 10) PRN_BN_SMALL_BWD(10); else PRN_BN_SMALL_BWD(12);
 #undef PRN_BN_SMALL_BWD
     PRN_CHECK_LAUNCH("prn_bn_bwd/small");
@@ -677,13 +728,13 @@
   const int S = bn_splits(B, HW);
   const int have = (!frozen || dgamma || dbeta) ? 1 : 0;
   if (have) {
-    for (int r = PRN_REPS(2); r > 0; --r) hipLaunchKernelGGL(bn_bwd_partial_kernel, dim3(C, S), dim3(256), 0, st, dy, x, y, stats, ws, B, C, HW, relu, gamma, beta, dbs);
+    for (int r = PRN_REPS(2); r > 0; --r) hipLaunchKernelGGL(bn_bwd_partial_kernel, dim3(C, S), dim3(256), 0, st, dy, x, y, stats, ws, B, C, HW, relu, gamma, beta, dbs, gate);
     PRN_CHECK_LAUNCH("prn_bn_bwd/partial");
   }
   int gx = cdiv(HW, 256 * 8);
   if (gx < 1) gx = 1;
   hipLaunchKernelGGL(bn_bwd_apply_kernel, dim3(gx, B * C), dim3(256), 0, st, dy, x, y, stats, gamma, (const double*)ws, dx, dres, C, HW,
-                     S, 1.f / ((float)B * HW), relu, frozen, have, dgamma, dbeta, beta, dbs);
+                     S, 1.f / ((float)B * HW), relu, frozen, have, dgamma, dbeta, beta, dbs, gate);
   PRN_CHECK_LAUNCH("prn_bn_bwd/apply");
   return 0;
 }
```

Result: no change. 191.9 (median of 6 runs) (+0.9%).
